# yellow-binary-tree/MMDuet

Measured on AMD Instinct MI355X. Metric: video frames/sec (stream decode, 1fps 336px), higher is better.
Workload: dtype bf16

## Files before the change

include/mmduet.h:

```cpp
#ifndef MMDUET_H
#define MMDUET_H
#include <stdint.h>
#ifdef __cplusplus
extern "C" {
#endif

#define MMD_OK 0
#define MMD_EINVAL (-22)
#define MMD_ENOMEM (-12)
#define MMD_ENOENT (-2)
#define MMD_ERANGE (-34)
#define MMD_EHIP (-5)

typedef enum { MMD_F32 = 0, MMD_BF16 = 1 } mmd_dtype;
typedef enum { MMD_W_DTYPE = 0, MMD_W_FP8_E4M3 = 1 } mmd_weight_dtype;
typedef enum { MMD_POOL_BILINEAR = 0, MMD_POOL_AVERAGE = 1, MMD_POOL_MAX = 2, MMD_POOL_ADAPTIVE_AVG = 3 } mmd_pool_mode;

typedef struct mmd_config {
    int32_t struct_size;
    int32_t dtype;
    int32_t vocab_size, hidden_size, intermediate_size, num_layers, num_heads, num_kv_heads, head_dim;
    float rope_theta, rms_norm_eps;
    int32_t vit_hidden, vit_intermediate, vit_layers, vit_heads, vit_image, vit_patch;
    float vit_ln_eps;
// ... 32 lines not shown
int mmd_vit_encode_frames(mmd_ctx* ctx, const uint8_t* frames, int B, int R, void* out);
int mmd_connector_pool(mmd_ctx* ctx, const void* tower_features, int B, void* out);
int mmd_normalize_frames(mmd_ctx* ctx, const void* frames, int src_kind, int B, int R, const float* mean3_host, const float* std3_host, float rescale, void* out);
int mmd_vision_tower(mmd_ctx* ctx, const void* pixel_values, int B, void* out);
int mmd_vision_pool_tokens(mmd_ctx* ctx, const void* feats, int B, int out_h, int out_w, void* out);
int mmd_vision_pool_head(mmd_ctx* ctx, const void* feats, int B, void* out);
int mmd_vit_set_full_tower(mmd_ctx* ctx, int on);
int mmd_vit_get_full_tower(const mmd_ctx* ctx);
int mmd_vit_debug_tap(mmd_ctx* ctx, int stage, void* out, int64_t out_elems);
int mmd_preprocess_frames(mmd_ctx* ctx, const uint8_t* frames, int T, int R, void* pixel_values);
int mmd_letterbox_geometry(int W, int H, int R, int* new_w, int* new_h, int* top, int* bottom, int* left, int* right);
int mmd_letterbox_frames(mmd_ctx* ctx, const uint8_t* frames, int T, int H, int W, int R, const uint8_t* pad_color,
                         int flip_channels, uint8_t* out);

int mmd_embed_tokens(mmd_ctx* ctx, const int64_t* ids, int k, void* out);

int mmd_stream_create(mmd_ctx* ctx, int64_t initial_tokens, mmd_stream** out);
void mmd_stream_destroy(mmd_stream* s);
int64_t mmd_kv_len(const mmd_stream* s);
int64_t mmd_kv_capacity(const mmd_stream* s);
int64_t mmd_kv_stride(const mmd_stream* s);
int mmd_kv_truncate(mmd_stream* s, int64_t new_len);
int mmd_kv_stash(mmd_stream* s, int64_t from, int64_t to);
int mmd_kv_unstash(mmd_stream* s);
int mmd_stream_reset(mmd_stream* s);
int mmd_kv_debug_set_len(mmd_stream* s, int64_t n);

int mmd_llm_step(mmd_ctx* ctx, mmd_stream* s, const void* embeds, int S, void* hidden_out);
int mmd_video_heads(mmd_ctx* ctx, const void* hidden, int M, float* out);
int mmd_lm_head(mmd_ctx* ctx, const void* hidden, int M, float* logits);
int mmd_frame_step(mmd_ctx* ctx, mmd_stream* s, const void* embeds, int S, const int32_t* head_rows_host, int n_rows,
                   float* head_logits_host);

int mmd_llm_step_multi(mmd_ctx* ctx, mmd_stream* const* streams, const int32_t* seg_rows, int n_segs, const void* embeds, void* hidden_out);
int mmd_frame_step_multi(mmd_ctx* ctx, mmd_stream* const* streams, const int32_t* seg_rows, int n_segs, const void* embeds,
                         const int32_t* head_rows, int n_head_rows, float* heads_out_host,
                         const int32_t* hidden_rows, int n_hidden_rows, void* hidden_rows_out, float* logits_out);

typedef struct mmd_sampler mmd_sampler;
#define MMD_SEG_FEED 1
#define MMD_SEG_SAMPLE 2
int mmd_sampler_create(mmd_ctx* ctx, mmd_sampler** out);
void mmd_sampler_destroy(mmd_sampler* sp);
int mmd_sampler_begin(mmd_sampler* sp, int64_t eos_id, float rep_penalty, const int64_t* prev_ids_host, int n_prev, int max_new);
int mmd_sampler_prev_len(const mmd_sampler* sp);
int mmd_round_multi(mmd_ctx* ctx, mmd_stream* const* streams, const int32_t* seg_rows, int n_segs, const void* const* seg_embeds, mmd_sampler* const* samplers,
                    const int32_t* seg_flags, const int32_t* head_rows, int n_head_rows, float* heads_out_host, int64_t* tokens_out_host);

int mmd_greedy_generate(mmd_ctx* ctx, mmd_stream* s, const void* prompt_embeds, int S, int64_t eos_id, float rep_penalty,
                        int64_t* prev_ids_host, int* n_prev, int prev_cap, int64_t* out_ids_host, int max_new, int* n_out);

#define MMD_COMM_ID_BYTES 128
typedef struct mmd_comm mmd_comm;
int mmd_comm_unique_id(uint8_t* id_out_host);
int mmd_comm_create(const uint8_t* id_host, int rank, int world, int device, void* hip_stream, mmd_comm** out);
void mmd_comm_destroy(mmd_comm* comm);
int mmd_comm_world(const mmd_comm* comm);
const char* mmd_comm_last_error(const mmd_comm* comm);
int mmd_gather_scores(mmd_comm* comm, const float* local, int T, int t_max, float* all);
int mmd_comm_probe(void);
int mmd_comm_set_stream(mmd_comm* comm, void* hip_stream);
int mmd_gather_block(mmd_comm* comm, const float* block, int64_t n_floats, float* all);

enum { MMD_K_GEMM_SKINNY = 0, MMD_K_GEMM_TILE = 1, MMD_K_ATTN_LLM = 2, MMD_K_ATTN_VIT = 3, MMD_K_NORM_ROPE = 4,
       MMD_K_OTHER = 5, MMD_K_COUNT = 6 };
int mmd_prof_enable(mmd_ctx* ctx, int class_mask);
int mmd_prof_set_stride(mmd_ctx* ctx, int stride);
int mmd_prof_read(mmd_ctx* ctx, double* ms_out , int64_t* launches_out ,
                  double* bytes_out , double* flops_out );
int mmd_prof_reset(mmd_ctx* ctx);

int mmd_op_gemm(mmd_ctx* ctx, const void* X, const void* W, const void* bias, const void* R, void* Y, int M, int N, int K,
                int epi, int out_f32, int variant);
int mmd_op_gemm_last_plan(mmd_ctx* ctx, int* out4);
int mmd_op_gemm_pair(mmd_ctx* ctx, const void* X, const void* W1, const void* b1, int epi1, const void* W2, const void* R, void* Y, int M, int N1, int K1, int N2,
                     int piece_major, int* used_pm_out);
int mmd_op_gemm_slabs(mmd_ctx* ctx, const void* X, const void* W, int M, int N, int K, int variant, float* slabs_out, int max_splits, int* splits_out);
int mmd_op_quantize_fp8(mmd_ctx* ctx, void* W, int N, int K, uint8_t* q8_out, float* scale_out);
int mmd_op_gemm_w8(mmd_ctx* ctx, const void* X, const void* Wq, const uint8_t* q8, const float* scale, const void* bias, const void* R, void* Y,
                   int M, int N, int K, int epi, int out_f32, int variant);
int mmd_op_gemm_bench(mmd_ctx* ctx, int M, int N, int K, int epi, int variant, int iters, float* avg_ms_out, const void* X, const void* W);
int mmd_op_rmsnorm(mmd_ctx* ctx, const void* x, const void* w, void* y, int M, int H, float eps);
int mmd_op_layernorm(mmd_ctx* ctx, const void* x, const void* w, const void* b, void* y, int M, int H, float eps);
int mmd_op_resid32_layernorm(mmd_ctx* ctx, const void* y16, float* h32, const void* pos16, int period, const void* w16, const void* b16, void* out16, void* outbf,
                             int M, int H, float eps);
int mmd_op_rope_append(mmd_ctx* ctx, void* qkv, int S, int nh, int nkv, int d, float theta, int64_t pos0, void* q_out,
                       void* Kc, void* Vc, int64_t cap);
int mmd_op_attention(mmd_ctx* ctx, const void* q, const void* Kc, const void* Vc, void* out, int S, int nh, int nkv, int d,
                     int64_t n_ctx, int64_t cap, int causal, int variant);
int mmd_op_attention_bench(mmd_ctx* ctx, int S, int nh, int nkv, int d, int64_t n_ctx, int variant, int iters, float* avg_ms_out);
int mmd_op_attention_last_form(mmd_ctx* ctx, int* out2);
int mmd_op_pool(mmd_ctx* ctx, const void* x, void* y, int B, int grid, int H, int mode, int stride);

#ifdef __cplusplus
}
#endif
#endif
```

mmduet_amd/_lib.py:

```python
import ctypes as C
import os

_HERE = os.path.dirname(os.path.abspath(__file__))
LIB_PATH = os.path.join(_HERE, 'csrc', 'libmmduet_hip.so')

MMD_F32, MMD_BF16 = 0, 1
POOL_MODES = {'bilinear': 0, 'average': 1, 'max': 2, 'adaptive_avg': 3}
K_NAMES = ('gemm_skinny', 'gemm_tile', 'attn_llm', 'attn_vit', 'norm_rope', 'other')
EPI = {'none': 0, 'gelu_tanh': 1, 'gelu_erf': 2, 'resid': 3, 'swiglu': 4}


class MmdConfig(C.Structure):
    _fields_ = [('struct_size', C.c_int32), ('dtype', C.c_int32),
                ('vocab_size', C.c_int32), ('hidden_size', C.c_int32), ('intermediate_size', C.c_int32),
                ('num_layers', C.c_int32), ('num_heads', C.c_int32), ('num_kv_heads', C.c_int32), ('head_dim', C.c_int32),
                ('rope_theta', C.c_float), ('rms_norm_eps', C.c_float),
                ('vit_hidden', C.c_int32), ('vit_intermediate', C.c_int32), ('vit_layers', C.c_int32), ('vit_heads', C.c_int32),
                ('vit_image', C.c_int32), ('vit_patch', C.c_int32), ('vit_ln_eps', C.c_float), ('vit_post_layernorm', C.c_int32),
                ('pool_mode', C.c_int32), ('pool_stride', C.c_int32), ('frame_num_tokens', C.c_int32),
                ('max_vit_batch', C.c_int32), ('max_step_tokens', C.c_int32), ('weight_dtype', C.c_int32),
                ('vision_only', C.c_int32), ('vit_class_token', C.c_int32), ('vit_pre_layernorm', C.c_int32), ('vit_act', C.c_int32), ('vit_pool_head', C.c_int32), ('tower_f16', C.c_int32)]


class MmduetError(RuntimeError):
    pass


_lib = None

_VP, _I, _I64, _F = C.c_void_p, C.c_int, C.c_int64, C.c_float
_SIGS = {
    'mmd_create': (_I, [C.POINTER(MmdConfig), _I, C.POINTER(_VP)]),
    'mmd_destroy': (None, [_VP]),
    'mmd_last_error': (C.c_char_p, [_VP]),
    'mmd_set_stream': (_I, [_VP, _VP]),
    'mmd_get_stream': (_VP, [_VP]),
    'mmd_synchronize': (_I, [_VP]),
    'mmd_load_tensor': (_I, [_VP, C.c_char_p, _VP, _I, C.POINTER(_I64), _I, _I]),
    'mmd_merge_lora': (_I, [_VP, C.c_char_p, _VP, _VP, _I, _F]),
    'mmd_set_rope_inv_freq': (_I, [_VP, _VP, _I]),
    'mmd_set_tower_share': (_I, [_VP, _I]),
    'mmd_finalize_weights': (_I, [_VP]),
    'mmd_weight_bytes': (_I64, [_VP]),
    'mmd_vit_encode': (_I, [_VP, _VP, _I, _VP]),
    'mmd_vit_set_full_tower': (_I, [_VP, _I]),
    'mmd_vit_get_full_tower': (_I, [_VP]),
    'mmd_vit_debug_tap': (_I, [_VP, _I, _VP, _I64]),
    'mmd_connector_pool': (_I, [_VP, _VP, _I, _VP]),
    'mmd_vit_encode_frames': (_I, [_VP, _VP, _I, _I, _VP]),
    'mmd_normalize_frames': (_I, [_VP, _VP, _I, _I, _I, C.POINTER(_F), C.POINTER(_F), _F, _VP]),
    'mmd_vision_tower': (_I, [_VP, _VP, _I, _VP]),
    'mmd_vision_pool_tokens': (_I, [_VP, _VP, _I, _I, _I, _VP]),
    'mmd_vision_pool_head': (_I, [_VP, _VP, _I, _VP]),
    'mmd_preprocess_frames': (_I, [_VP, _VP, _I, _I, _VP]),
    'mmd_letterbox_geometry': (_I, [_I, _I, _I] + [C.POINTER(_I)] * 6),
    'mmd_letterbox_frames': (_I, [_VP, _VP, _I, _I, _I, _I, _VP, _I, _VP]),
    'mmd_embed_tokens': (_I, [_VP, _VP, _I, _VP]),
    'mmd_stream_create': (_I, [_VP, _I64, C.POINTER(_VP)]),
    'mmd_stream_destroy': (None, [_VP]),
    'mmd_kv_len': (_I64, [_VP]),
    'mmd_kv_capacity': (_I64, [_VP]),
    'mmd_kv_stride': (_I64, [_VP]),
    'mmd_kv_truncate': (_I, [_VP, _I64]),
    'mmd_kv_debug_set_len': (_I, [_VP, _I64]),
    'mmd_stream_reset': (_I, [_VP]),
    'mmd_kv_stash': (_I, [_VP, _I64, _I64]),
    'mmd_kv_unstash': (_I, [_VP]),
    'mmd_comm_unique_id': (_I, [_VP]),
    'mmd_comm_create': (_I, [_VP, _I, _I, _I, _VP, C.POINTER(_VP)]),
    'mmd_comm_destroy': (None, [_VP]),
    'mmd_comm_world': (_I, [_VP]),
    'mmd_comm_last_error': (C.c_char_p, [_VP]),
    'mmd_gather_scores': (_I, [_VP, _VP, _I, _I, _VP]),
    'mmd_comm_probe': (_I, []),
    'mmd_comm_set_stream': (_I, [_VP, _VP]),
    'mmd_gather_block': (_I, [_VP, _VP, C.c_int64, _VP]),
    'mmd_llm_step': (_I, [_VP, _VP, _VP, _I, _VP]),
    'mmd_video_heads': (_I, [_VP, _VP, _I, _VP]),
    'mmd_lm_head': (_I, [_VP, _VP, _I, _VP]),
    'mmd_frame_step': (_I, [_VP, _VP, _VP, _I, _VP, _I, _VP]),
    'mmd_llm_step_multi': (_I, [_VP, C.POINTER(_VP), C.POINTER(C.c_int32), _I, _VP, _VP]),
    'mmd_frame_step_multi': (_I, [_VP, C.POINTER(_VP), C.POINTER(C.c_int32), _I, _VP, C.POINTER(C.c_int32), _I, C.POINTER(_F), C.POINTER(C.c_int32), _I, _VP, _VP]),
    'mmd_sampler_create': (_I, [_VP, C.POINTER(_VP)]),
    'mmd_sampler_destroy': (None, [_VP]),
    'mmd_sampler_begin': (_I, [_VP, _I64, _F, _VP, _I, _I]),
    'mmd_sampler_prev_len': (_I, [_VP]),
    'mmd_round_multi': (_I, [_VP, C.POINTER(_VP), C.POINTER(C.c_int32), _I, C.POINTER(_VP), C.POINTER(_VP), C.POINTER(C.c_int32), C.POINTER(C.c_int32), _I, C.POINTER(_F), C.POINTER(_I64)]),
    'mmd_greedy_generate': (_I, [_VP, _VP, _VP, _I, _I64, _F, _VP, C.POINTER(_I), _I, _VP, _I, C.POINTER(_I)]),
    'mmd_prof_enable': (_I, [_VP, _I]),
    'mmd_prof_set_stride': (_I, [_VP, _I]),
    'mmd_prof_read': (_I, [_VP, _VP, _VP, _VP, _VP]),
    'mmd_prof_reset': (_I, [_VP]),
    'mmd_op_gemm': (_I, [_VP, _VP, _VP, _VP, _VP, _VP, _I, _I, _I, _I, _I, _I]),
    'mmd_op_gemm_bench': (_I, [_VP, _I, _I, _I, _I, _I, _I, C.POINTER(_F), _VP, _VP]),
    'mmd_op_gemm_last_plan': (_I, [_VP, C.POINTER(_I)]),
    'mmd_op_gemm_pair': (_I, [_VP, _VP, _VP, _VP, _I, _VP, _VP, _VP, _I, _I, _I, _I, _I, C.POINTER(_I)]),
    'mmd_op_gemm_slabs': (_I, [_VP, _VP, _VP, _I, _I, _I, _I, _VP, _I, C.POINTER(_I)]),
    'mmd_op_quantize_fp8': (_I, [_VP, _VP, _I, _I, _VP, _VP]),
    'mmd_op_gemm_w8': (_I, [_VP, _VP, _VP, _VP, _VP, _VP, _VP, _VP, _I, _I, _I, _I, _I, _I]),
    'mmd_op_rmsnorm': (_I, [_VP, _VP, _VP, _VP, _I, _I, _F]),
    'mmd_op_layernorm': (_I, [_VP, _VP, _VP, _VP, _VP, _I, _I, _F]),
    'mmd_op_resid32_layernorm': (_I, [_VP, _VP, _VP, _VP, _I, _VP, _VP, _VP, _VP, _I, _I, _F]),
    'mmd_op_rope_append': (_I, [_VP, _VP, _I, _I, _I, _I, _F, _I64, _VP, _VP, _VP, _I64]),
    'mmd_op_attention': (_I, [_VP, _VP, _VP, _VP, _VP, _I, _I, _I, _I, _I64, _I64, _I, _I]),
    'mmd_op_attention_bench': (_I, [_VP, _I, _I, _I, _I, _I64, _I, _I, C.POINTER(_F)]),
    'mmd_op_attention_last_form': (_I, [_VP, C.POINTER(_I)]),
    'mmd_op_pool': (_I, [_VP, _VP, _VP, _I, _I, _I, _I, _I]),
}
EXPORTED_SYMBOLS = tuple(_SIGS)


def lib():
    global _lib
    if _lib is not None:
        return _lib
    if not os.path.exists(LIB_PATH):
        raise MmduetError(f'{LIB_PATH} not found: the MI355X HIP library is required (no CPU fallback). '
                          f'Build it with `make -C {os.path.dirname(LIB_PATH)}` or __graft_entry__.build().')
    try:
        L = C.CDLL(LIB_PATH, mode=C.RTLD_GLOBAL)
    except OSError as e:
        raise MmduetError(f'cannot load {LIB_PATH}: {e}') from e
    for name, (res, args) in _SIGS.items():
        try:
            fn = getattr(L, name)
        except AttributeError as e:
            raise MmduetError(f'{LIB_PATH} does not export {name}') from e
        fn.restype, fn.argtypes = res, args
    _lib = L
    return L


def check(rc, ctx=None, what=''):
    if rc == 0:
        return
    msg = lib().mmd_last_error(ctx)
    raise MmduetError(f'{what or "libmmduet_hip"} failed ({rc}): {msg.decode() if msg else "?"}')
```

mmduet_amd/csrc/gemm.hip:

```cpp
#include "common.h"
#include <type_traits>

#include "gemm_ring.h"

template <typename T> struct Frag;
template <> struct Frag<bf16_t> { using type = bf16x8_t; static constexpr int KSTEP = 32; };
template <> struct Frag<float> { using type = float; static constexpr int KSTEP = 4; };

template <typename T, int BM, int BN> struct TileCfg {
    static constexpr int BK = 32;
    static constexpr int PAD = sizeof(T) == 2 ? 8 : 1;
    static constexpr int LD = BK + PAD;
    static constexpr int WM = BM / 2, WN = BN / 2;
    static constexpr int TM = WM / 16, TN = WN / 16;
};

template <typename T, int ROWS, int LD>
__device__ __forceinline__ void stage_tile(T* __restrict__ lds, const T* __restrict__ g, long long ld, int r0, int nrows, int k0, int kend,
                                           int vec, int tid) {
    if constexpr (sizeof(T) == 2) {
        for (int i = tid; i < ROWS * 4; i += 256) {
            int r = i >> 2, c = (i & 3) * 8;
            s16x8_t v = {0, 0, 0, 0, 0, 0, 0, 0};
            int gr = r0 + r, gk = k0 + c;
// ... 841 lines not shown
        const int k0 = step * BK;
#pragma unroll
        for (int j = 0; j < BM / 32; ++j) {
            const int pi = wave + 4 * j;
            int row = m0 + pi * 8 + (lane >> 3);
            row = row < p.M ? row : p.M - 1;
            const int chunk = (lane & 7) ^ (lane >> 3);
            const bf16_t* src = X + (long long)row * p.ldx + k0 + chunk * 8;
            __builtin_amdgcn_global_load_lds((const __attribute__((address_space(1))) void*)src,
                                             (__attribute__((address_space(3))) void*)(xs + pi * 512), 16, 0, 0);
        }
#pragma unroll
        for (int j = 0; j < BN / 32; ++j) {
            const int wi = wave + 4 * j;
            const bf16_t* src = Wp + (((long long)(n0 / 16 + (wi >> 1)) * KT + (k0 >> 5) + (wi & 1)) * 64 + lane) * 8;
            __builtin_amdgcn_global_load_lds((const __attribute__((address_space(1))) void*)src,
                                             (__attribute__((address_space(3))) void*)(ws + wi * 512), 16, 0, 0);
        }
    };

    f32x4_t acc[TM][TN];
#pragma unroll
    for (int i = 0; i < TM; ++i)
#pragma unroll
        for (int j = 0; j < TN; ++j) acc[i][j] = f32x4_t{0, 0, 0, 0};

    const int zsteps = (nsteps + gridDim.z - 1) / gridDim.z;
    const int t0 = blockIdx.z * zsteps, t1 = min(nsteps, t0 + zsteps);
    if (t0 < t1) stage(0, t0);
    int cur = 0;
    for (int t = t0; t < t1; ++t) {
        __syncthreads();
        if (t + 1 < t1) stage(cur ^ 1, t + 1);
        const bf16_t* xs = lds + cur * (XE + WE);
        const bf16_t* ws = xs + XE;
#pragma unroll
        for (int kt = 0; kt < 2; ++kt) {
            bf16x8_t xf[TM], wf[TN];
#pragma unroll
            for (int i = 0; i < TM; ++i) {
                const int mt = (wm >> 4) + i;
                const int c = kt * 4 + lq;
                xf[i] = *reinterpret_cast<const bf16x8_t*>(xs + (mt * 2 + (lr >> 3)) * 512 + (lr & 7) * 64 + ((c ^ (lr & 7)) * 8));
            }
#pragma unroll
            for (int j = 0; j < TN; ++j) wf[j] = *reinterpret_cast<const bf16x8_t*>(ws + (((wn >> 4) + j) * 2 + kt) * 512 + lane * 8);
#pragma unroll
            for (int i = 0; i < TM; ++i)
#pragma unroll
                for (int j = 0; j < TN; ++j) acc[i][j] = mfma16<F16>(wf[j], xf[i], acc[i][j]);
        }
        cur ^= 1;
    }

    if (gridDim.z > 1) {
        float* ws = p.ws + (long long)blockIdx.z * p.M * p.N;
#pragma unroll
        for (int i = 0; i < TM; ++i) {
            const int m = m0 + wm + i * 16 + lr;
            if (m < p.M) {
#pragma unroll
                for (int j = 0; j < TN; ++j) *reinterpret_cast<f32x4_t*>(ws + (long long)m * p.N + n0 + wn + j * 16 + lq * 4) = acc[i][j];
            }
        }
        return;
    }
    [[maybe_unused]] f32x4_t scq[TN]; [[maybe_unused]] s16x4_t biq[TN]; [[maybe_unused]] s16x4_t rq[TM][TN];
    const bool has_sc = p.wscale != nullptr, has_bi = p.bias != nullptr;
    if constexpr (EPI != EPI_SWIGLU) {
#pragma unroll
        for (int j = 0; j < TN; ++j) {
            const int n = n0 + wn + j * 16 + lq * 4;
            scq[j] = has_sc ? *reinterpret_cast<const f32x4_t*>(p.wscale + n) : f32x4_t{1, 1, 1, 1};
            biq[j] = has_bi ? *reinterpret_cast<const s16x4_t*>((const bf16_t*)p.bias + n) : s16x4_t{0, 0, 0, 0};
        }
#pragma unroll
        for (int i = 0; i < TM; ++i)
#pragma unroll
            for (int j = 0; j < TN; ++j) {
                rq[i][j] = s16x4_t{0, 0, 0, 0};
                if constexpr (EPI == EPI_RESID) rq[i][j] = *reinterpret_cast<const s16x4_t*>((const bf16_t*)p.R + (long long)min(m0 + wm + i * 16 + lr, p.M - 1) * p.ldr + n0 + wn + j * 16 + lq * 4);
            }
    }
#pragma unroll
    for (int i = 0; i < TM; ++i) {
        const int m = m0 + wm + i * 16 + lr;
        [[maybe_unused]] const int mc = m < p.M ? m : p.M - 1;
        if constexpr (EPI == EPI_SWIGLU) {
            if constexpr (TN == 4) {
                const int nb = n0 + wn, ob = (nb >> 5) * 16;
                const s16x8_t v = pair_to_row8(big_value_swiglu(acc[i][0], acc[i][1], p.wscale, nb + lq * 4), big_value_swiglu(acc[i][2], acc[i][3], p.wscale, nb + 32 + lq * 4));
                if (m < p.M) *reinterpret_cast<s16x8_t*>((bf16_t*)p.Y + (long long)m * p.ldy + ob + (lq & 1) * 16 + (lq >> 1) * 8) = v;
            } else {
#pragma unroll
                for (int j = 0; j < TN; j += 2) big_store_swiglu(p, m, n0 + wn + j * 16 + lq * 4, acc[i][j], acc[i][j + 1]);
            }
        } else {
#pragma unroll
            for (int j = 0; j < TN; j += 2) {
                const int nb = n0 + wn + j * 16;
                const s16x8_t v = pair_to_row8(big_value_pre<EPI, F16>(acc[i][j], has_sc, scq[j], has_bi, biq[j], rq[i][j]), big_value_pre<EPI, F16>(acc[i][j + 1], has_sc, scq[j + 1], has_bi, biq[j + 1], rq[i][j + 1]));
                if (m < p.M) *reinterpret_cast<s16x8_t*>((bf16_t*)p.Y + (long long)m * p.ldy + nb + (lq & 1) * 16 + (lq >> 1) * 8) = v;
            }
        }
    }
}

template <int BN>
static void launch_big(const GemmP& p, const GemmPlan& pl, hipStream_t st) {
    const int KT = p.K >> 5;
    const dim3 grid(pl.gx, pl.gy, pl.splits);
    if (pl.bm == 160) {
        if constexpr (BN == 64) {
            if (p.epi == EPI_RESID) hipLaunchKernelGGL((gemm_big_kernel<64, EPI_RESID, false, 160>), grid, dim3(256), 0, st, p, KT);
            else hipLaunchKernelGGL((gemm_big_kernel<64, EPI_NONE, false, 160>), grid, dim3(256), 0, st, p, KT);
        }
        return;
    }
    if (pl.f16) {
        switch (p.epi) {
            case EPI_GELU_TANH: hipLaunchKernelGGL((gemm_big_kernel<BN, EPI_GELU_TANH, true>), grid, dim3(256), 0, st, p, KT); break;
            case EPI_RESID: hipLaunchKernelGGL((gemm_big_kernel<BN, EPI_RESID, true>), grid, dim3(256), 0, st, p, KT); break;
            default: hipLaunchKernelGGL((gemm_big_kernel<BN, EPI_NONE, true>), grid, dim3(256), 0, st, p, KT); break;
        }
        return;
    }
    switch (p.epi) {
        case EPI_GELU_TANH: hipLaunchKernelGGL((gemm_big_kernel<BN, EPI_GELU_TANH>), grid, dim3(256), 0, st, p, KT); break;
        case EPI_GELU_ERF: hipLaunchKernelGGL((gemm_big_kernel<BN, EPI_GELU_ERF>), grid, dim3(256), 0, st, p, KT); break;
        case EPI_RESID: hipLaunchKernelGGL((gemm_big_kernel<BN, EPI_RESID>), grid, dim3(256), 0, st, p, KT); break;
        case EPI_SWIGLU: hipLaunchKernelGGL((gemm_big_kernel<BN, EPI_SWIGLU>), grid, dim3(256), 0, st, p, KT); break;
        default: hipLaunchKernelGGL((gemm_big_kernel<BN, EPI_NONE>), grid, dim3(256), 0, st, p, KT); break;
    }
    if (pl.reduce) launch_reduce(splitk_reduce_kernel<bf16_t>, p, pl.splits, st);
}


static void* ring_dump_slot() {
    static void* dump_slot[64] = {};
    int dev = 0; hipGetDevice(&dev);
    if (dev < 0 || dev >= 64) return nullptr;
    if (!dump_slot[dev] && hipMalloc(&dump_slot[dev], 8192) != hipSuccess) return nullptr;
    return dump_slot[dev];
}

template <int WN, bool M32, int NS, bool EARLY, bool F16 = false>
static hipError_t launch_ringx_t(const GemmP& p, const GemmPlan& pl, hipStream_t st) {
    constexpr int BN = 64 * WN;
    const dim3 grid(pl.gx, 1, pl.splits);
    const int KT = p.K >> 5;
    const size_t smem = NS * (256 * 32 + BN * 32) * sizeof(bf16_t);
    static bool attr_set[64] = {};
    int adev = 0; hipGetDevice(&adev);
    if (adev >= 0 && adev < 64 && !attr_set[adev]) {
#define RX_ATTR(E) hipFuncSetAttribute((const void*)gemm_ringx_kernel<E, WN, M32, NS, EARLY, 0, F16>, hipFuncAttributeMaxDynamicSharedMemorySize, (int)smem);
        RX_ATTR(EPI_NONE) RX_ATTR(EPI_GELU_TANH) RX_ATTR(EPI_RESID)
        if constexpr (!F16) { RX_ATTR(EPI_GELU_ERF) RX_ATTR(EPI_SWIGLU) }
#undef RX_ATTR
        attr_set[adev] = true;
    }
    const dim3 block(WN * 128);
    GemmP q = p;
    q.dump = ring_dump_slot();
    if (!q.dump) return hipErrorOutOfMemory;
#define RX_GO(E) hipLaunchKernelGGL((gemm_ringx_kernel<E, WN, M32, NS, EARLY, 0, F16>), grid, block, smem, st, q, KT)
    switch (p.epi) {
        case EPI_GELU_TANH: RX_GO(EPI_GELU_TANH); break;
        case EPI_GELU_ERF: if constexpr (!F16) RX_GO(EPI_GELU_ERF); break;
        case EPI_RESID: RX_GO(EPI_RESID); break;
        case EPI_SWIGLU: if constexpr (!F16) RX_GO(EPI_SWIGLU); break;
        default: RX_GO(EPI_NONE); break;
    }
#undef RX_GO
    if (pl.reduce) launch_reduce(splitk_reduce_kernel<bf16_t>, p, pl.splits, st);
    return hipSuccess;
}
static hipError_t launch_ringx(const GemmP& p, const GemmPlan& pl, hipStream_t st) {
    if (pl.f16) return launch_ringx_t<4, false, 3, true, true>(p, pl, st);
    return pl.wn == 4 ? launch_ringx_t<4, false, 3, true>(p, pl, st) : launch_ringx_t<2, false, 3, true>(p, pl, st);
}

static inline void set_plan(const GemmArgs& a, const GemmPlan& pl) {
    if (a.plan_out) { a.plan_out[0] = pl.kernel; a.plan_out[1] = pl.tiles; a.plan_out[2] = pl.splits; a.plan_out[3] = pl.blocks; }
}

#ifdef MMDUET_DEBUG_VARIANTS
template <int DBG, int NS = 3>
static hipError_t launch_ringx_dbg(const GemmP& p, const GemmArgs& a, hipStream_t st) {
    GemmPlan pl;
    pl.kernel = GEMM_K_RING256; pl.tiles = cdiv(a.N, 256) * cdiv(a.M, 256); pl.blocks = pl.tiles <= 256 ? pl.tiles : 256;
    set_plan(a, pl);
    const size_t smem = NS * (256 * 32 + 256 * 32) * sizeof(bf16_t);
    hipFuncSetAttribute((const void*)gemm_ringx_kernel<EPI_NONE, 4, false, NS, true, DBG>, hipFuncAttributeMaxDynamicSharedMemorySize, (int)smem);
    hipLaunchKernelGGL((gemm_ringx_kernel<EPI_NONE, 4, false, NS, true, DBG>), dim3(pl.blocks), dim3(512), smem, st, p, a.K >> 5);
    return hipGetLastError();
}
static bool launch_debug_variant(GemmP p, const GemmArgs& a, hipStream_t st, hipError_t* err) {
    const int variant = a.variant;
    p.W = a.Wp;
    if (variant >= 92 && variant <= 99) {
        if (!big_packed_ok(MMD_BF16, a, 16) || (a.N % 32) != 0) { *err = hipErrorInvalidValue; return true; }
        switch (variant) {
            case 92: *err = launch_ringx_dbg<8, 4>(p, a, st); break;
            case 93: *err = launch_ringx_dbg<7>(p, a, st); break;
            case 94: *err = launch_ringx_dbg<6>(p, a, st); break;
            case 95: *err = launch_ringx_dbg<5>(p, a, st); break;
            case 99: *err = launch_ringx_dbg<4>(p, a, st); break;
            case 96: *err = launch_ringx_dbg<1>(p, a, st); break;
            case 97: *err = launch_ringx_dbg<2>(p, a, st); break;
            default: *err = launch_ringx_dbg<3>(p, a, st); break;
        }
        return true;
    }
    if (variant >= 300 && variant < 340 && a.M <= 64 && a.Wp) {
        p.slabs = a.epi == EPI_SWIGLU ? 0 : 1;
        GemmArgs b = a; int dummy = 0; if (a.epi != EPI_SWIGLU) { b.slabs_out = &dummy; b.epi = EPI_NONE; p.epi = EPI_NONE; }
        const bool two = a.epi == EPI_SWIGLU;
        GemmPlan pl;
#define SGO(NT_, WK_, KS_, NB_, DBG_, WN_, SPLIT_) (stream_geometry(pl, b, 4, NT_, WK_ * KS_, WN_, SPLIT_), set_plan(a, pl), launch_stream_t<4, NT_, WK_, KS_, NB_, DBG_, WN_>(p, pl, st))
#define SCFG(id, WK_, KS_, NB_, DBG_) case id: if (two) SGO(2, WK_, KS_, NB_, DBG_, 4, 0); else SGO(1, WK_, KS_, NB_, DBG_, 4, 0); break;
        switch (variant - 300) {
            SCFG(0, 2, 2, 4, 0) SCFG(1, 1, 4, 3, 0) SCFG(2, 4, 1, 4, 0) SCFG(3, 2, 4, 3, 0) SCFG(4, 1, 4, 4, 0) SCFG(5, 4, 2, 3, 0) SCFG(7, 2, 2, 6, 0)
            SCFG(10, 2, 2, 4, 1) SCFG(11, 1, 4, 3, 1) SCFG(12, 2, 2, 4, 2) SCFG(13, 1, 4, 3, 2)
            case 20: if (two) SGO(2, 2, 2, 4, 0, 5, 0); else SGO(1, 2, 2, 4, 0, 7, 8); break;
            case 21: if (two) SGO(2, 3, 2, 3, 0, 5, 0); else SGO(1, 2, 2, 4, 0, 7, 4); break;
            case 22: if (two) SGO(2, 2, 2, 4, 1, 5, 0); else SGO(1, 2, 2, 4, 1, 7, 8); break;
            case 23: if (two) SGO(2, 1, 4, 3, 0, 5, 0); else SGO(1, 1, 4, 3, 0, 7, 8); break;
            case 24: if (two) SGO(2, 2, 2, 4, 0, 8, 0); else SGO(1, 2, 2, 4, 0, 7, 16); break;
            default: *err = hipErrorInvalidValue; return true;
        }
#undef SCFG
#undef SGO
        *err = hipGetLastError();
        return true;
    }
    return false;
}
#endif

template <typename T>
static hipError_t launch_t(const GemmArgs& a, const GemmPlan& pl, hipStream_t st) {
    GemmP p;
    p.X = a.X; p.W = pl.w_from == GEMM_W_PACKED8 ? a.Wp8 : (pl.w_from == GEMM_W_PACKED ? a.Wp : a.W); p.bias = a.bias; p.R = a.R; p.Y = a.Y; p.ws = a.splitk_ws; p.wscale = a.wscale;
    p.ldx = a.ldx; p.ldw = a.ldw; p.ldr = a.ldr; p.ldy = a.ldy;
    p.M = a.M; p.N = a.N; p.K = a.K; p.epi = a.epi; p.out_f32 = a.out_f32; p.slabs = a.slabs_out ? 1 : 0; p.dump = nullptr; p.flags = 0; p.kper = pl.kper; p.x_pm = a.x_pm; p.y_pm = a.y_pm;
    p.vec = (sizeof(T) == 2 && (a.ldx % 8) == 0 && (a.ldw % 8) == 0 && ((uintptr_t)a.X % 16) == 0 && ((uintptr_t)a.W % 16) == 0) ? 1 : 0;
    if (a.ring_slabs_out) *a.ring_slabs_out = pl.ring_slabs;
    if (pl.kernel == GEMM_PLAN_EMPTY) return hipSuccess;
#ifdef MMDUET_DEBUG_VARIANTS
    if (hipError_t e = hipSuccess; sizeof(T) == 2 && launch_debug_variant(p, a, st, &e)) return e;
#endif
    if (!pl.valid()) return hipErrorInvalidValue;
    if (a.slabs_out && (pl.kernel == GEMM_K_GEMV16 || pl.kernel == GEMM_K_SKINNY || pl.kernel == GEMM_K_STREAM)) *a.slabs_out = pl.slabs;
    set_plan(a, pl);
    switch (pl.kernel) {
        case GEMM_K_GEMV16: launch_gemv16(p, pl, a.chain, st); break;
        case GEMM_K_STREAM: launch_stream(p, pl, st); break;
        case GEMM_K_RING256: case GEMM_K_RING128X2: if (hipError_t e = launch_ringx(p, pl, st); e != hipSuccess) return e; break;
        case GEMM_K_BIG128: launch_big<128>(p, pl, st); break;
        case GEMM_K_BIG64: launch_big<64>(p, pl, st); break;
        case GEMM_K_SKINNY: if (pl.mt == 1) launch_skinny_mt<1>(p, pl, st); else if (pl.mt == 2) launch_skinny_mt<2>(p, pl, st); else launch_skinny_mt<4>(p, pl, st); break;
        case GEMM_K_TILE128: hipLaunchKernelGGL((gemm_tile_kernel<T, 128, 128>), dim3(pl.gx, pl.gy, 1), dim3(256), 0, st, p); break;
        default:
            hipLaunchKernelGGL((gemm_tile_kernel<T, 64, 64>), dim3(pl.gx, pl.gy, pl.splits), dim3(256), 0, st, p);
            if (pl.reduce) launch_reduce(splitk_reduce_kernel<T>, p, pl.splits, st);
    }
    return hipGetLastError();
}

GemmPlan gemm_plan_for(int dtype, const GemmArgs& a) {
    static const GemmTuning tune = [] { GemmTuning t; if (const char* s = getenv("MMDUET_GEMV_KSPLIT_SHORT")) t.gemv_ksplit_short = atoi(s); return t; }();
    return gemm_plan(dtype, a, tune);
}
bool gemm_can_slab(int dtype, const GemmArgs& a) {
    int dummy = 0; GemmArgs b = a; b.slabs_out = &dummy; b.epi = EPI_NONE;
    const int k = gemm_plan_for(dtype, b).kernel;
    return k == GEMM_K_GEMV16 || k == GEMM_K_SKINNY || k == GEMM_K_STREAM;
}
bool gemm_ring_auto(int dtype, const GemmArgs& a, bool plain_only) {
    const int ring = gemm_plan_for(dtype, a).ring_auto;
    return !a.wscale && (plain_only ? ring == RING_AUTO_PLAIN : ring != RING_AUTO_NONE);
}
hipError_t launch_gemm(int dtype, const GemmArgs& a, hipStream_t st, const GemmPlan* planned) {
    const GemmPlan pl = planned ? *planned : gemm_plan_for(dtype, a);
    return dtype != MMD_F32 ? launch_t<bf16_t>(a, pl, st) : launch_t<float>(a, pl, st);
}
```

mmduet_amd/csrc/gemm_plan.h:

```cpp
#pragma once
#include <stddef.h>
#include <stdint.h>
#include "../../include/mmduet.h"

constexpr int MMD_F16 = 2;

static inline int cdiv(int64_t a, int64_t b) { return (int)((a + b - 1) / b); }
static inline int64_t round_up(int64_t a, int64_t b) { return (a + b - 1) / b * b; }

enum { EPI_NONE = 0, EPI_GELU_TANH = 1, EPI_GELU_ERF = 2, EPI_RESID = 3, EPI_SWIGLU = 4 };
enum { GEMM_AUTO = 0, GEMM_GENERIC = 1, GEMM_SKINNY = 2, GEMM_LARGE = 3, GEMM_BIG = 4, GEMM_SLAB = 5, GEMM_RING256 = 6, GEMM_RING256_SPLIT = 7,
       GEMM_RINGX = 16 ,
       GEMM_STREAM = 8  };

constexpr int GEMV_SSQ_STRIDE = 256;
constexpr int GEMV_CHAIN_ROWS = 4;
struct GemvChain {
    const void* xn_h = nullptr; const void* xn_gamma = nullptr; const float* xn_ssq = nullptr; float xn_eps = 0.f;
    void* fin_h = nullptr; float* fin_ssq = nullptr;
};
struct GemmArgs {
    const void* X; int64_t ldx;
    const void* W; int64_t ldw;
    const void* Wp = nullptr;
    const void* Wp8 = nullptr;
    const float* wscale = nullptr;
    const void* bias;
    const void* R; int64_t ldr;
    void* Y; int64_t ldy;
    int M, N, K;
    int epi; int out_f32;
    int variant;
    float* splitk_ws; size_t splitk_ws_bytes;
    int no_gemv = 0;
    int* ring_slabs_out = nullptr;
    int* slabs_out = nullptr;
    int ring_flags = 16;
    int ring_max_blocks = 0;
    const GemvChain* chain = nullptr;
    int* plan_out = nullptr;
    int x_pm = 0, y_pm = 0;
    int f16 = 0;
};
enum { GEMM_K_TILE64 = 0, GEMM_K_TILE128 = 1, GEMM_K_SKINNY = 2, GEMM_K_GEMV16 = 3, GEMM_K_BIG64 = 4, GEMM_K_BIG128 = 5, GEMM_K_RING256 = 6, GEMM_K_RING128X2 = 7, GEMM_K_STREAM = 8 };

struct GemmTuning {
    int gemv_ksplit_short = 2;
};

enum { GEMM_PLAN_INVALID = -1,
       GEMM_PLAN_EMPTY = -2 };
enum { GEMM_W_ROWMAJOR = 0, GEMM_W_PACKED = 1, GEMM_W_PACKED8 = 2 };
enum { GEMV_PLAIN = 0, GEMV_CONSUMER = 1, GEMV_PRODUCER = 2 };
enum { RING_AUTO_NONE = 0, RING_AUTO_PLAIN = 1, RING_AUTO_SPLIT = 2 };

struct GemmPlan {
    int kernel = GEMM_PLAN_INVALID;
    int tiles = 0, splits = 1, blocks = 0;
    int gx = 0, gy = 1;
    int prof_class = MMD_K_GEMM_TILE;
    int w_from = GEMM_W_ROWMAJOR;
    int mt = 0, nt = 0, wn = 0;
    int kt_per_block = 0;
    int kper = 0;
    int bn = 0, bm = 0;
    int chain = GEMV_PLAIN;
    int f16 = 0;
    int ring_auto = RING_AUTO_NONE;
    bool reduce = false;
    int slabs = 0;
    int ring_slabs = 0;
    bool valid() const { return kernel >= 0; }
};

static inline bool stream_ok(int dtype, const GemmArgs& a) {
    if (dtype != MMD_BF16 || a.f16 || !a.Wp || a.M <= 32 || a.M > 256 || (a.N % 16) != 0 || (a.ldx % 8) != 0 || ((uintptr_t)a.X % 16) != 0 || a.out_f32) return false;
    if (a.Wp8 && a.M <= 64) return false;
    if ((long long)a.M * a.ldx * 2 >= (1ll << 32)) return false;
    const int ksb = a.M <= 128 ? 4 : 2;
    if ((a.K % (ksb * 32)) != 0) return false;
    if (a.epi == EPI_SWIGLU) return (a.N % 32) == 0 && !a.slabs_out;
    if (a.slabs_out) return a.splitk_ws != nullptr && a.epi == EPI_NONE && (size_t)a.M * a.N * sizeof(float) <= a.splitk_ws_bytes;
    return a.splitk_ws != nullptr && (a.N % 4) == 0 && (a.ldy % 4) == 0 && (a.epi != EPI_RESID || (a.ldr % 4) == 0);
}
static inline void stream_geometry(GemmPlan& pl, const GemmArgs& a, int MT, int NT, int KSB, int WN, int want_split) {
    const int KT = a.K >> 5, ntiles = a.N >> 4;
    const int bx = cdiv(ntiles, WN * NT);
    int ksplit = 1;
    if (a.slabs_out || (a.epi != EPI_SWIGLU && a.splitk_ws)) {
        ksplit = want_split > 0 ? want_split : cdiv(288, bx);
        const int maxs = KT / (KSB * 6); if (ksplit > maxs) ksplit = maxs;
        if (ksplit > 16) ksplit = 16;
        if (ksplit < 1) ksplit = 1;
        while (ksplit > 1 && (size_t)ksplit * a.M * a.N * sizeof(float) > a.splitk_ws_bytes) --ksplit;
    }
    const int ktper = (int)round_up(cdiv(KT, ksplit), KSB);
    ksplit = cdiv(KT, ktper);
    pl.kernel = GEMM_K_STREAM; pl.tiles = ntiles; pl.splits = ksplit; pl.blocks = bx * ksplit; pl.gx = bx; pl.gy = 1;
    pl.w_from = GEMM_W_PACKED; pl.mt = MT; pl.nt = NT; pl.wn = WN; pl.kt_per_block = ktper;
    pl.slabs = ksplit;
    pl.reduce = !a.slabs_out && ksplit > 1;
}
struct StreamPlan { int wn, ksplit; };
static inline StreamPlan stream_plan(const GemmArgs& a, int NT, int MT, int KSB, bool can_split) {
    const int KT = a.K >> 5, ntiles = a.N >> 4;
    StreamPlan best{4, 1}; double best_cost = 1e30;
    for (int wn = 4; wn <= 8; ++wn) {
        const int bx = cdiv(ntiles, wn * NT);
        for (int ks = 1; ks <= (can_split ? 16 : 1); ++ks) {
            const int ktper = (int)round_up(cdiv(KT, ks), KSB);
            if (cdiv(KT, ktper) != ks) continue;
// ... 55 lines not shown
        if (splits > 8) splits = 8;
        while (splits > 1 && (size_t)splits * a.M * a.N * sizeof(float) > a.splitk_ws_bytes) --splits;
    }
    int ktper = (int)round_up(cdiv(KT, splits), 4);
    splits = cdiv(KT, ktper);
    GemmPlan pl;
    pl.kernel = GEMM_K_SKINNY; pl.tiles = ntiles; pl.splits = splits; pl.blocks = nblocks * splits; pl.gx = nblocks;
    pl.w_from = a.Wp8 ? GEMM_W_PACKED8 : GEMM_W_PACKED; pl.mt = MT; pl.nt = NT; pl.kt_per_block = ktper;
    pl.slabs = splits;
    pl.reduce = !a.slabs_out && splits > 1;
    return pl;
}

static inline bool big_bm160(const GemmArgs& a, int BN) {
    if (BN != 64 || a.f16 || (a.epi != EPI_NONE && a.epi != EPI_RESID) || a.M < 512) return false;
    const long long t128 = (long long)(a.N / 64) * cdiv(a.M, 128), t160 = (long long)(a.N / 64) * cdiv(a.M, 160);
    if (t160 > 512) return false;
    return (double)cdiv(t160, 256) * 160.0 < (double)cdiv(t128, 256) * 128.0 * 0.97;
}
static inline GemmPlan plan_big(const GemmArgs& a, int BN) {
    GemmPlan pl;
    pl.kernel = BN == 128 ? GEMM_K_BIG128 : GEMM_K_BIG64; pl.w_from = GEMM_W_PACKED; pl.bn = BN; pl.f16 = a.f16;
    if (big_bm160(a, BN)) {
        const int tiles = (a.N / 64) * cdiv(a.M, 160);
        pl.tiles = tiles; pl.splits = 1; pl.blocks = tiles; pl.gx = a.N / 64; pl.gy = cdiv(a.M, 160); pl.bm = 160;
        return pl;
    }
    const int tiles = (a.N / BN) * cdiv(a.M, 128);
    int splits = 1;
    if (tiles < 320 && a.K >= 8192 && a.epi != EPI_SWIGLU && a.splitk_ws && !a.f16) {
        splits = 3;
        if (tiles <= 64) splits = 4;
        while (splits > 1 && (size_t)splits * a.M * a.N * sizeof(float) > a.splitk_ws_bytes) --splits;
    } else if (tiles < 128 && a.K >= 2048 && a.epi != EPI_SWIGLU && a.splitk_ws && !a.f16) {
        splits = 256 / tiles; if (splits > 4) splits = 4; if (splits < 1) splits = 1;
        while (splits > 1 && (size_t)splits * a.M * a.N * sizeof(float) > a.splitk_ws_bytes) --splits;
    }
    pl.tiles = tiles; pl.splits = splits; pl.blocks = tiles * splits; pl.gx = a.N / BN; pl.gy = cdiv(a.M, 128); pl.bm = 128;
    if (splits > 1) {
        if (a.ring_slabs_out) pl.ring_slabs = splits;
        else pl.reduce = true;
    }
    return pl;
}

static inline bool ring_size_ok(const GemmArgs& a) { return (long long)a.M * a.ldx * 2 < (1ll << 32) && (long long)a.N * a.K * 2 < (1ll << 32); }
static inline bool ring_tiles_ok(long long t) { return t >= 400 || (t >= 192 && (double)t / (double)(cdiv((int)t, 256) * 256) >= 0.9); }
static inline bool big_packed_ok(int dtype, const GemmArgs& a, int BN) {
    return dtype == MMD_BF16 && a.Wp != nullptr && a.M > 64 && (a.N % BN) == 0 && (a.K % 64) == 0 && (a.ldx % 8) == 0 &&
           ((uintptr_t)a.X % 16) == 0 && !a.out_f32 && (a.ldy % 4) == 0 && ((uintptr_t)a.Y % 8) == 0 &&
           (a.epi != EPI_RESID || ((a.ldr % 4) == 0 && ((uintptr_t)a.R % 8) == 0)) && (a.bias == nullptr || ((uintptr_t)a.bias % 8) == 0);
}

static inline bool skinny_packed_ok(int dtype, const GemmArgs& a) {
    return dtype == MMD_BF16 && a.Wp != nullptr && a.M <= 64 && (a.N % 16) == 0 && (a.K % 32) == 0 && (a.ldx % 8) == 0 &&
           ((uintptr_t)a.X % 16) == 0 && (a.epi != EPI_SWIGLU || (a.N % 32) == 0);
}

static inline int ring_split_choice(const GemmArgs& a) {
    const int t256 = cdiv(a.M, 256) * cdiv(a.N, 256);
    int sp = 256 / t256; if (sp < 1) sp = 1;
    if (t256 > 128) {
        double best = 1e30; int bsp = 1;
        for (int s = 1; s <= 8; ++s) {
            if (s > 1 && (a.K / s < 1024 || (size_t)s * a.M * a.N * sizeof(float) > a.splitk_ws_bytes)) break;
            const double rounds = (double)cdiv(t256 * s, 256);
            const double cost = rounds * ((double)a.K / s) * 0.025 + (s > 1 ? (double)s * a.M * a.N * 8.0 / 5e6 : 0.0);
            if (cost < best * 0.97) { best = cost; bsp = s; }
        }
        return bsp;
    }
    while (sp > 1 && a.K / sp < 1024) --sp;
    while (sp > 1 && (size_t)sp * a.M * a.N * sizeof(float) > a.splitk_ws_bytes) --sp;
    return sp;
}
static inline GemmPlan plan_ring(const GemmArgs& a, int flags, int splits) {
    GemmPlan pl;
    int WN = 4;
    if (!a.f16) switch (flags & 27) {
        case 16: WN = 4; break;
        case 17: WN = 2; break;
        default: return pl;
    }
    if (a.f16 && a.epi != EPI_NONE && a.epi != EPI_GELU_TANH && a.epi != EPI_RESID) return pl;
    if (a.f16) splits = 1;
    while (splits > 1 && (a.epi == EPI_SWIGLU || !a.splitk_ws || (size_t)splits * a.M * a.N * sizeof(float) > a.splitk_ws_bytes)) --splits;
    const int BN = 64 * WN;
    const int tiles = cdiv(a.N, BN) * cdiv(a.M, 256);
    const int slots = WN == 2 ? 512 : 256;
    const int cap = a.ring_max_blocks < 0 ? tiles : (a.ring_max_blocks > 0 && a.ring_max_blocks < slots ? a.ring_max_blocks : slots);
    pl.kernel = WN == 2 ? GEMM_K_RING128X2 : GEMM_K_RING256; pl.w_from = GEMM_W_PACKED; pl.wn = WN; pl.f16 = a.f16;
    pl.gx = splits > 1 || tiles <= cap ? tiles : cap;
    pl.tiles = tiles; pl.splits = splits; pl.blocks = pl.gx * splits;
    pl.kper = splits > 1 ? 0 : ((a.K / 32) * 10) / 100 + 1;
    if (splits > 1) {
        if (a.ring_slabs_out) pl.ring_slabs = splits;
        else pl.reduce = true;
    }
    return pl;
}

static inline GemmPlan plan_tile(const GemmArgs& a, bool skinny, bool large) {
    int splits = 1;
    if (skinny) {
        int blocks = cdiv(a.N, 64) * cdiv(a.M, 64);
        int want = cdiv(512, blocks);
        int maxs = a.K / 256; if (maxs < 1) maxs = 1;
        splits = want < maxs ? want : maxs;
        if (splits > 16) splits = 16;
        if (a.splitk_ws == nullptr) splits = 1;
        while (splits > 1 && (size_t)splits * a.M * a.N * sizeof(float) > a.splitk_ws_bytes) --splits;
    }
    int kper = (int)round_up(cdiv(a.K, splits), 32);
    splits = cdiv(a.K, kper);
    GemmPlan pl;
    pl.kper = kper;
    const int B = large ? 128 : 64;
    pl.kernel = large ? GEMM_K_TILE128 : GEMM_K_TILE64; pl.gx = cdiv(a.N, B); pl.gy = cdiv(a.M, B);
    pl.tiles = pl.gx * pl.gy; pl.splits = large ? 1 : splits; pl.blocks = pl.tiles * pl.splits;
    pl.reduce = !large && splits > 1;
    return pl;
}

static inline GemmPlan plan_kernel(bool two_byte, const GemmArgs& a, const GemmTuning& tune) {
    const GemmPlan invalid;
    const int variant = a.variant;
    const bool skinny = (variant == GEMM_SKINNY) || (variant == GEMM_AUTO && a.M <= 64);
    const bool large = (variant == GEMM_LARGE) || (variant == GEMM_AUTO && a.M >= 256 && a.N >= 128);
    if (two_byte) {
        if ((variant == GEMM_AUTO || variant == GEMM_SKINNY || variant == GEMM_STREAM) && stream_ok(MMD_BF16, a)) return plan_stream(a);
        if (variant == GEMM_STREAM) return invalid;
        const bool ring_ok = big_packed_ok(MMD_BF16, a, 16) && (a.N % 32) == 0 && ring_size_ok(a);
        if (variant == GEMM_RING256 || (variant == GEMM_AUTO && a.M >= 512 && ring_ok && ring_tiles_ok((long long)cdiv(a.M, 256) * cdiv(a.N, 256)))) {
            if (!ring_ok) return invalid;
            GemmPlan pl = plan_ring(a, a.ring_flags, 1);
            if (variant == GEMM_AUTO) pl.ring_auto = RING_AUTO_PLAIN;
            return pl;
        }
        const bool ring_split_ok = ring_ok && a.epi != EPI_SWIGLU && a.splitk_ws != nullptr;
        if (!a.f16 && (variant == GEMM_RING256_SPLIT || (variant == GEMM_AUTO && a.M >= 512 && a.K >= 8192 && ring_split_ok))) {
            if (variant == GEMM_RING256_SPLIT && !ring_ok) return invalid;
            const int sp = ring_split_choice(a);
            if (variant == GEMM_RING256_SPLIT || sp >= 2) {
                GemmPlan pl = plan_ring(a, 16, sp);
                if (variant == GEMM_AUTO) pl.ring_auto = RING_AUTO_SPLIT;
                return pl;
            }
        }
        if (variant >= GEMM_RINGX && variant < GEMM_RINGX + 128) {
            if (!ring_ok) return invalid;
            const int flags = variant - GEMM_RINGX;
            int sp = 1;
            if (flags & 4) {
                const int slots = (flags & 1) ? 512 : 256, tl = cdiv(a.M, 256) * cdiv(a.N, (flags & 1) ? 128 : 256);
                sp = slots / tl; if (sp < 1) sp = 1;
                while (sp > 1 && a.K / sp < 1024) --sp;
                if (sp < 2) sp = 2;
            }
            return plan_ring(a, flags, sp);
        }
        const bool want_big = variant == GEMM_BIG || (variant == GEMM_AUTO && a.M > 64);
        if (want_big) {
            int bn = 0;
            const long long t128 = (long long)cdiv(a.M, 128) * (a.N / 128);
            if (big_packed_ok(MMD_BF16, a, 128) && (t128 >= 400 || (a.K >= 8192 && t128 >= 224))) bn = 128;
            else if (big_packed_ok(MMD_BF16, a, 64)) bn = 64;
            if (bn && variant == GEMM_AUTO && !a.f16 && a.M >= 512 && a.K >= 1024 && (a.N % 128) == 0 && big_packed_ok(MMD_BF16, a, 16) && ring_size_ok(a)) {
                const long long mt128 = cdiv(a.M, 128);
                const double nb = bn == 64 ? (double)cdiv(mt128 * (a.N / 64), 256) : (double)cdiv(t128, 256);
                const double cbig = bn == 64 ? (nb > 1.83 ? nb : 1.83) : (1.77 * nb > 2.29 ? 1.77 * nb : 2.29);
                const double cr4 = 2.95 * (double)cdiv((long long)cdiv(a.M, 256) * (a.N / 128), 256);
                if (cr4 < 0.8 * cbig)
                    return plan_ring(a, 17, 1);
            }
            if (bn) return plan_big(a, bn);
            if (variant == GEMM_BIG) return invalid;
        }
        if (a.f16) return invalid;
        if (skinny && skinny_packed_ok(MMD_BF16, a)) {
            if (a.slabs_out && !a.splitk_ws) return invalid;
            if (a.M <= 16 && !a.no_gemv) return plan_gemv16(a, tune);
            if (a.chain) return invalid;
            return plan_skinny(a, a.M <= 16 ? 1 : (a.M <= 32 ? 2 : 4));
        }
    }
    if (a.slabs_out) return invalid;
    if (a.chain) return invalid;
    if (a.W == nullptr) return invalid;
    return plan_tile(a, skinny, large);
}

static inline GemmPlan gemm_plan(int dtype, const GemmArgs& a, const GemmTuning& tune) {
    if (dtype == MMD_F16 && !a.f16) { GemmArgs h = a; h.f16 = 1; return gemm_plan(dtype, h, tune); }
    GemmPlan pl;
    if (a.M <= 0 || a.N <= 0) { pl.kernel = GEMM_PLAN_EMPTY; return pl; }
    pl = plan_kernel(dtype != MMD_F32, a, tune);
    if (!pl.valid()) return pl;
    if ((a.x_pm || a.y_pm) && (pl.ring_auto == RING_AUTO_NONE || a.wscale || (a.x_pm && (a.K % 32)) || (a.y_pm && ((a.epi == EPI_SWIGLU ? a.N / 2 : a.N) % 32)))) return GemmPlan();
    if (a.y_pm && pl.ring_auto != RING_AUTO_PLAIN) return GemmPlan();
    const bool streaming = pl.kernel == GEMM_K_GEMV16 || pl.kernel == GEMM_K_SKINNY || pl.kernel == GEMM_K_STREAM;
    pl.prof_class = streaming || (pl.kernel == GEMM_K_TILE64 && a.M <= 64) ? MMD_K_GEMM_SKINNY : MMD_K_GEMM_TILE;
    return pl;
}
```

mmduet_amd/csrc/gemm_ring.h:

```cpp
#pragma once
#include "common.h"
#include <type_traits>

#define MMD_BAR() do { asm volatile("" ::: "memory"); __builtin_amdgcn_s_barrier(); asm volatile("" ::: "memory"); } while (0)

struct GemmP {
    const void* X; const void* W; const void* bias; const void* R; void* Y; float* ws;
    const float* wscale;
    long long ldx, ldw, ldr, ldy;
    int M, N, K, epi, out_f32, kper, vec;
    int slabs;
    void* dump;
    int flags;
    int x_pm, y_pm;
};

template <int EPI>
__device__ __forceinline__ s16x4_t big_value(const GemmP& p, int m, int n, const f32x4_t& a) {
    float v[4] = {a[0], a[1], a[2], a[3]};
    if (p.wscale) {
        const f32x4_t sc = *reinterpret_cast<const f32x4_t*>(p.wscale + n);
#pragma unroll
        for (int r = 0; r < 4; ++r) v[r] *= sc[r];
    }
    if (p.bias) {
        s16x4_t b = *reinterpret_cast<const s16x4_t*>((const bf16_t*)p.bias + n);
#pragma unroll
        for (int r = 0; r < 4; ++r) v[r] += bf2f((bf16_t)b[r]);
    }
    if constexpr (EPI == EPI_GELU_TANH) {
#pragma unroll
        for (int r = 0; r < 4; ++r) v[r] = gelu_tanh_fast(bf2f(f2bf(v[r])));
    } else if constexpr (EPI == EPI_GELU_ERF) {
#pragma unroll
        for (int r = 0; r < 4; ++r) v[r] = gelu_erf_fast(bf2f(f2bf(v[r])));
    } else if constexpr (EPI == EPI_RESID) {
        s16x4_t rr = *reinterpret_cast<const s16x4_t*>((const bf16_t*)p.R + (long long)m * p.ldr + n);
#pragma unroll
        for (int r = 0; r < 4; ++r) v[r] = bf2f(f2bf(v[r])) + bf2f((bf16_t)rr[r]);
    }
    return s16x4_t{(short)f2bf(v[0]), (short)f2bf(v[1]), (short)f2bf(v[2]), (short)f2bf(v[3])};
}
template <int EPI, bool F16 = false>
__device__ __forceinline__ s16x4_t big_value_pre(const f32x4_t& a, bool has_scale, const f32x4_t& sc, bool has_bias, const s16x4_t& b, const s16x4_t& rr) {
    float v[4] = {a[0], a[1], a[2], a[3]};
    if (has_scale) {
#pragma unroll
        for (int r = 0; r < 4; ++r) v[r] *= sc[r];
    }
    if (has_bias) {
#pragma unroll
        for (int r = 0; r < 4; ++r) v[r] += raw2f<F16>((uint16_t)b[r]);
    }
    if constexpr (EPI == EPI_GELU_TANH) {
#pragma unroll
        for (int r = 0; r < 4; ++r) v[r] = gelu_tanh_fast(raw2f<F16>(f2raw<F16>(v[r])));
    } else if constexpr (EPI == EPI_GELU_ERF) {
#pragma unroll
        for (int r = 0; r < 4; ++r) v[r] = gelu_erf_fast(raw2f<F16>(f2raw<F16>(v[r])));
    } else if constexpr (EPI == EPI_RESID) {
#pragma unroll
        for (int r = 0; r < 4; ++r) v[r] = raw2f<F16>(f2raw<F16>(v[r])) + raw2f<F16>((uint16_t)rr[r]);
    }
    return s16x4_t{(short)f2raw<F16>(v[0]), (short)f2raw<F16>(v[1]), (short)f2raw<F16>(v[2]), (short)f2raw<F16>(v[3])};
}
template <int EPI>
__device__ __forceinline__ void big_store(const GemmP& p, int m, int n, const f32x4_t& a) {
    if (m >= p.M) return;
    *reinterpret_cast<s16x4_t*>((bf16_t*)p.Y + (long long)m * p.ldy + n) = big_value<EPI>(p, m, n, a);
}
__device__ __forceinline__ s16x4_t big_value_swiglu(const f32x4_t& g_in, const f32x4_t& u_in, const float* ws = nullptr, int n_gate = 0) {
    f32x4_t g = g_in, u = u_in;
    if (ws) { g *= *reinterpret_cast<const f32x4_t*>(ws + n_gate); u *= *reinterpret_cast<const f32x4_t*>(ws + n_gate + 16); }
    s16x4_t o;
#pragma unroll
    for (int r = 0; r < 4; ++r) {
        float gg = bf2f(f2bf(g[r])), uu = bf2f(f2bf(u[r]));
        float sl = bf2f(f2bf(gg * __builtin_amdgcn_rcpf(1.0f + __builtin_amdgcn_exp2f(-gg * 1.4426950408889634f))));
        o[r] = (short)f2bf(sl * uu);
    }
    return o;
}
__device__ __forceinline__ s16x8_t pair_to_row8(const s16x4_t& ta, const s16x4_t& tb) {
    const uint2 a = __builtin_bit_cast(uint2, ta), b = __builtin_bit_cast(uint2, tb);
    const auto x = __builtin_amdgcn_permlane16_swap(a.x, b.x, false, false);
    const auto y = __builtin_amdgcn_permlane16_swap(a.y, b.y, false, false);
    const uint4 o = {x[0], y[0], x[1], y[1]};
    return __builtin_bit_cast(s16x8_t, o);
}
__device__ __forceinline__ void big_store_swiglu(const GemmP& p, int m, int n_gate, const f32x4_t& g, const f32x4_t& u) {
    if (m >= p.M) return;
    const int oc = (n_gate >> 5) * 16 + (n_gate & 15);
    *reinterpret_cast<s16x4_t*>((bf16_t*)p.Y + (long long)m * p.ldy + oc) = big_value_swiglu(g, u, p.wscale, n_gate);
}


__device__ __forceinline__ f32x4_t quad_of(const f32x16_t& v, int q) { return f32x4_t{v[4 * q], v[4 * q + 1], v[4 * q + 2], v[4 * q + 3]}; }
__device__ __forceinline__ s16x8_t halves_to_row8(const s16x4_t& q0, const s16x4_t& q1) {
    const uint2 a = __builtin_bit_cast(uint2, q0), b = __builtin_bit_cast(uint2, q1);
    const auto x = __builtin_amdgcn_permlane32_swap(a.x, b.x, false, false);
    const auto y = __builtin_amdgcn_permlane32_swap(a.y, b.y, false, false);
    const uint4 o = {x[0], y[0], x[1], y[1]};
    return __builtin_bit_cast(s16x8_t, o);
}

template <int EPI, int WN, bool M32, int NS, bool EARLY, int DBG = 0, bool F16 = false>
__global__ __launch_bounds__(WN * 128, 2) void gemm_ringx_kernel(GemmP p, int KT) {
    static_assert(!F16 || (!M32 && EPI != EPI_SWIGLU), "the fp16 form exists for the 16x16x32 schedule and the tower's epilogues");
    constexpr int BM = 256, BN = 64 * WN, BK = 32, NW = 2 * WN;
    constexpr int XE = BM * BK, WE = BN * BK, SE = XE + WE;
    constexpr int XP = (BM / 16) / NW, WP = (BN / 16) / NW;
    constexpr int NDMA = DBG == 3 ? 0 : (DBG == 2 ? WP : XP + WP);
    extern __shared__ __attribute__((aligned(16))) bf16_t lds[];
    const int tid = threadIdx.x, lane = tid & 63, wave = __builtin_amdgcn_readfirstlane(tid >> 6);
    const int lr = lane & 15, lq = lane >> 4, lh = lane >> 5;
    const int wr = wave / WN, wc = wave % WN;
    const int nbx = (p.N + BN - 1) / BN, nby = (p.M + BM - 1) / BM;
    const int nblk = nbx * nby;
    int m0 = 0, n0 = 0;
    auto tile_origin = [&](int bid) {
        const int xcd = bid & 7, q = nblk >> 3, r = nblk & 7;
        bid = (xcd < r ? xcd * (q + 1) : r * (q + 1) + (xcd - r) * q) + (bid >> 3);
        const int TB = nby < 8 ? nby : 8;
        const int band = bid / (TB * nbx), rem = bid - band * (TB * nbx);
        const int tb = min(TB, nby - band * TB);
        const int nt = rem / tb, mt = band * TB + rem - nt * tb;
        m0 = mt * BM; n0 = nt * BN;
    };
    const int ntiles = p.N >> 4;
    const bf16_t* X = (const bf16_t*)p.X;
    const bf16_t* Wp = (const bf16_t*)p.W;
    const int nsteps_all = p.K / BK;
    const int zsteps = (nsteps_all + gridDim.z - 1) / gridDim.z;
    const int t0 = blockIdx.z * zsteps;
    const int nsteps = min(nsteps_all, t0 + zsteps) - t0;

    const int srow = lane >> 2, spos = lane & 3;
    const int sswz = (0x1230 >> (((srow >> 2) & 3) * 4)) & 3;
    unsigned xo[XP]; long long wo[WP];
    const unsigned wlane = lane * 16;
    const int xstep = p.x_pm ? 1024 : BK * 2;
    auto tile_sources = [&]() {
#pragma unroll
        for (int j = 0; j < XP; ++j) {
            const int pi = wave + NW * j;
            if (p.x_pm) {
                int grp = (m0 >> 4) + pi; const int gmax = (p.M - 1) >> 4; grp = grp < gmax ? grp : gmax;
                xo[j] = (unsigned)(grp * (p.K >> 5)) * 1024u + (unsigned)(srow * 64 + ((spos ^ sswz) * 16));
                continue;
            }
            int row = m0 + pi * 16 + srow; row = row < p.M ? row : p.M - 1;
            xo[j] = (unsigned)(row * (int)p.ldx + ((spos ^ sswz) * 8)) * 2u;
        }
#pragma unroll
        for (int j = 0; j < WP; ++j) {
            const int pi = wave + NW * j;
            int ntile = n0 / 16 + pi; ntile = ntile < ntiles ? ntile : ntiles - 1;
            wo[j] = ((long long)ntile * KT * 512 + (long long)t0 * 512) * 2;
        }
    };
    auto dma_x = [&](int slot, int step, int j) {
        if constexpr (DBG == 2 || DBG == 3) return;
        if constexpr (DBG == 1) {
            __builtin_amdgcn_global_load_lds((const __attribute__((address_space(1))) void*)(X + (long long)min(m0 + (wave + NW * j) * 16, p.M - 16) * p.ldx + (long long)step * 512 + lane * 8),
                                             (__attribute__((address_space(3))) void*)(lds + slot * SE + (wave + NW * j) * 512), 16, 0, 0);
            return;
        }
        const char* ub = (const char*)X + (long long)(t0 + step) * xstep;
        asm volatile("" : "+s"(ub));
        __builtin_amdgcn_global_load_lds((const __attribute__((address_space(1))) void*)(ub + xo[j]),
                                         (__attribute__((address_space(3))) void*)(lds + slot * SE + (wave + NW * j) * 512), 16, 0, 0);
    };
    auto dma_w = [&](int slot, int step, int j) {
        if constexpr (DBG == 3) return;
        const char* ub = (const char*)Wp + wo[j] + (long long)step * 1024;
        asm volatile("" : "+s"(ub));
        __builtin_amdgcn_global_load_lds((const __attribute__((address_space(1))) void*)(ub + wlane),
                                         (__attribute__((address_space(3))) void*)(lds + slot * SE + XE + (wave + NW * j) * 512), 16, 0, 0);
    };
    auto stage = [&](int slot, int step) {
#pragma unroll
        for (int j = 0; j < XP; ++j) dma_x(slot, step, j);
#pragma unroll
        for (int j = 0; j < WP; ++j) dma_w(slot, step, j);
    };
    auto dma_k = [&](int slot, int step, int k) { if (k < XP) dma_x(slot, step, k); else if (k < XP + WP) dma_w(slot, step, k - XP); };

    constexpr int VM_ONE = NDMA, VM_TWO = 2 * NDMA;
    constexpr int NST = EPI == EPI_SWIGLU ? 8 : 16;
#ifdef MMDUET_NO_PST
    constexpr bool PST = false;
#else
    constexpr bool PST = !M32 && NS == 3 && DBG == 0;
#endif
#define RINGX_WAIT(n) asm volatile("s_waitcnt vmcnt(%0) lgkmcnt(0)" :: "i"(n) : "memory")
    const int G = gridDim.x;
    const int rswz = (0x1230 >> (((lr >> 2) & 3) * 4)) & 3;
    if constexpr (WN == 2 && NS == 3) {
        if (G > 256 && (int)blockIdx.x >= 256 && p.kper > 0) {
            for (int i = 0; i < p.kper; ++i) __builtin_amdgcn_s_sleep(127);
        }
    }

    if constexpr (!M32) {
        f32x4_t acc[8][4];
#pragma unroll
        for (int i = 0; i < 8; ++i)
#pragma unroll
            for (int j = 0; j < 4; ++j) acc[i][j] = f32x4_t{0, 0, 0, 0};
        const int aoff = (wr * 8) * 512 + lr * 32 + ((lq ^ rswz) * 8);
        const int boff = XE + (wc * 4) * 512 + lane * 8;
        bf16x8_t a[8], b0[4], b1[4];
        auto step = [&](auto steady, int s, int slot, const bf16x8_t (&b)[4], bf16x8_t (&bn)[4], auto pending) {
            constexpr bool STEADY = decltype(steady)::value;
            constexpr bool PEND = decltype(pending)::value;
            if (DBG == 5 && s < 2) RINGX_WAIT((NS - 2) * NDMA + 16);
            else if (PEND) RINGX_WAIT((NS - 2) * NDMA + NST);
            else if (STEADY || s + NS - 1 < nsteps) RINGX_WAIT((NS - 2) * NDMA);
            else if (NS == 4 && s + 2 < nsteps) RINGX_WAIT(NDMA);
            else RINGX_WAIT(0);
            if (!(DBG == 8 && (s & 1))) MMD_BAR();
            const bool refill = STEADY || s + NS < nsteps;
            const bool more = STEADY || s + 1 < nsteps;
            const bf16_t* nbase = lds + (slot == NS - 1 ? 0 : slot + 1) * SE;
            bf16x8_t a6n, a7n;
            __builtin_amdgcn_s_setprio(1);
            if constexpr (DBG == 7) {
#pragma unroll
                for (int i = 0; i < 8; ++i) {
                    acc[i][0] = mfma16<F16>(b[0], a[i], acc[i][0]);
                    __builtin_amdgcn_sched_barrier(0);
                    if (more) { if (i == 0) a7n = *reinterpret_cast<const bf16x8_t*>(nbase + aoff + 7 * 512); else a[i - 1] = *reinterpret_cast<const bf16x8_t*>(nbase + aoff + (i - 1) * 512); }
                    __builtin_amdgcn_sched_barrier(0);
                    acc[i][1] = mfma16<F16>(b[1], a[i], acc[i][1]);
                    __builtin_amdgcn_sched_barrier(0);
                    if (more && i < 4) bn[i] = *reinterpret_cast<const bf16x8_t*>(nbase + boff + i * 512);
                    __builtin_amdgcn_sched_barrier(0);
                    acc[i][2] = mfma16<F16>(b[2], a[i], acc[i][2]);
                    __builtin_amdgcn_sched_barrier(0);
                    if (refill && i < XP + WP) dma_k(slot, s + NS, i);
                    __builtin_amdgcn_sched_barrier(0);
                    acc[i][3] = mfma16<F16>(b[3], a[i], acc[i][3]);
                    __builtin_amdgcn_sched_barrier(0);
                }
                if (more) a[7] = a7n;
                __builtin_amdgcn_s_setprio(0);
                return;
            }
#pragma unroll
            for (int i = 0; i < 8; ++i) {
#pragma unroll
                for (int j = 0; j < 4; ++j) acc[i][j] = mfma16<F16>(b[j], a[i], acc[i][j]);
                __builtin_amdgcn_sched_barrier(0);
                if (more) {
                    if (i < 6) a[i] = *reinterpret_cast<const bf16x8_t*>(nbase + aoff + i * 512);
                    if (i < 4) bn[i] = *reinterpret_cast<const bf16x8_t*>(nbase + boff + i * 512);
                    if (i == 0) a6n = *reinterpret_cast<const bf16x8_t*>(nbase + aoff + 6 * 512);
                    if (i == 1) a7n = *reinterpret_cast<const bf16x8_t*>(nbase + aoff + 7 * 512);
                }
                if (refill) {
                    if (EARLY ? i < XP + WP : i >= 8 - (XP + WP)) dma_k(slot, s + NS, i - (EARLY ? 0 : 8 - (XP + WP)));
                }
                __builtin_amdgcn_sched_barrier(0);
            }
            if (more) { a[6] = a6n; a[7] = a7n; }
            __builtin_amdgcn_s_setprio(0);
        };
        auto prologue = [&]() { stage(0, 0); if (nsteps > 1) stage(1, 1); if (nsteps > 2) stage(2, 2); if (NS > 3 && nsteps > 3) stage(3, 3); };
        int tile = blockIdx.x;
        tile_origin(tile); tile_sources(); prologue();
        for (; tile < nblk; tile += G) {
            const bool pend = PST && tile != (int)blockIdx.x && nsteps >= NS + 3 && gridDim.z == 1;
            if (DBG == 5) asm volatile("s_waitcnt vmcnt(%0)" :: "i"(VM_TWO + 16) : "memory");
            else if (pend) asm volatile("s_waitcnt vmcnt(%0)" :: "i"(VM_TWO + NST) : "memory");
            else if (NS > 3 && nsteps > 3) asm volatile("s_waitcnt vmcnt(%0)" :: "i"(3 * NDMA) : "memory");
            else if (nsteps > 2) asm volatile("s_waitcnt vmcnt(%0)" :: "i"(VM_TWO) : "memory");
            else if (nsteps > 1) asm volatile("s_waitcnt vmcnt(%0)" :: "i"(VM_ONE) : "memory");
            else asm volatile("s_waitcnt vmcnt(0)" ::: "memory");
            MMD_BAR();
#pragma unroll
            for (int i = 0; i < 8; ++i) a[i] = *reinterpret_cast<const bf16x8_t*>(lds + aoff + i * 512);
#pragma unroll
            for (int j = 0; j < 4; ++j) b0[j] = *reinterpret_cast<const bf16x8_t*>(lds + boff + j * 512);
            int slot = 0, s = 0;
            if (pend) {
                step(std::true_type{}, 0, 0, b0, b1, std::true_type{});
                step(std::true_type{}, 1, 1, b1, b0, std::true_type{});
                slot = 2 % NS; s = 2;
            }
            for (; s + NS + 1 < nsteps; s += 2) {
                step(std::true_type{}, s, slot, b0, b1, std::false_type{});
                slot = slot == NS - 1 ? 0 : slot + 1;
                step(std::true_type{}, s + 1, slot, b1, b0, std::false_type{});
                slot = slot == NS - 1 ? 0 : slot + 1;
            }
            for (; s < nsteps; s += 2) {
                step(std::false_type{}, s, slot, b0, b1, std::false_type{});
                slot = slot == NS - 1 ? 0 : slot + 1;
                if (s + 1 < nsteps) {
                    step(std::false_type{}, s + 1, slot, b1, b0, std::false_type{});
                    slot = slot == NS - 1 ? 0 : slot + 1;
                }
            }
            const int em0 = m0, en0 = n0;
            bf16_t* const dump = (bf16_t*)p.dump + tid * 8;
            if (tile + G < nblk) { tile_origin(tile + G); tile_sources(); prologue(); }
            __builtin_amdgcn_sched_barrier(0);
            if (gridDim.z > 1) {
                float* wsl = p.ws + (long long)blockIdx.z * p.M * p.N;
#pragma unroll
                for (int i = 0; i < 8; ++i) {
                    const int m = em0 + wr * 128 + i * 16 + lr;
                    if (m < p.M) {
#pragma unroll
                        for (int j = 0; j < 4; ++j) { const int nb = en0 + wc * 64 + j * 16; if (nb + 16 <= p.N) *reinterpret_cast<f32x4_t*>(wsl + (long long)m * p.N + nb + lq * 4) = acc[i][j]; }
                    }
                }
                return;
            }
            f32x4_t scq[4]; s16x4_t biq[4], rq[4], rnext[4];
            int ncol[4];
            const bool has_sc = p.wscale != nullptr, has_bi = p.bias != nullptr;
            if constexpr (EPI != EPI_SWIGLU) {
#pragma unroll
                for (int j = 0; j < 4; ++j) {
                    const int nb = en0 + wc * 64 + (j & ~1) * 16;
                    ncol[j] = ((j & 1) ? (nb + 32 <= p.N ? nb + 16 : p.N - 16) : (nb + 16 <= p.N ? nb : p.N - 16)) + lq * 4;
                    scq[j] = has_sc ? *reinterpret_cast<const f32x4_t*>(p.wscale + ncol[j]) : f32x4_t{1, 1, 1, 1};
                    biq[j] = has_bi ? *reinterpret_cast<const s16x4_t*>((const bf16_t*)p.bias + ncol[j]) : s16x4_t{0, 0, 0, 0};
                    rq[j] = rnext[j] = s16x4_t{0, 0, 0, 0};
                }
                if constexpr (EPI == EPI_RESID) {
                    const int m = min(em0 + wr * 128 + lr, p.M - 1);
#pragma unroll
                    for (int j = 0; j < 4; ++j) rnext[j] = *reinterpret_cast<const s16x4_t*>((const bf16_t*)p.R + (long long)m * p.ldr + ncol[j]);
                }
            }
            if constexpr (DBG == 4) {
#pragma unroll
                for (int i = 0; i < 8; ++i)
#pragma unroll
                    for (int j = 0; j < 4; ++j) asm volatile("" :: "v"(acc[i][j][0]), "v"(acc[i][j][1]), "v"(acc[i][j][2]), "v"(acc[i][j][3]));
            } else
#pragma unroll
            for (int i = 0; i < 8; ++i) {
                const int m = em0 + wr * 128 + i * 16 + lr;
                const int mc = m < p.M ? m : p.M - 1;
                if constexpr (EPI == EPI_RESID) {
#pragma unroll
                    for (int j = 0; j < 4; ++j) rq[j] = rnext[j];
                    if (i < 7) {
                        const int mn = min(m + 16, p.M - 1);
#pragma unroll
                        for (int j = 0; j < 4; ++j) rnext[j] = *reinterpret_cast<const s16x4_t*>((const bf16_t*)p.R + (long long)mn * p.ldr + ncol[j]);
                    }
                    __builtin_amdgcn_sched_barrier(0);
                }
                if constexpr (EPI == EPI_SWIGLU) {
                    const int nb = en0 + wc * 64;
                    const int ob = (nb >> 5) * 16;
                    const int ns0 = min(nb, p.N - 32) + lq * 4, ns1 = min(nb + 32, p.N - 32) + lq * 4;
                    const s16x8_t v = pair_to_row8(big_value_swiglu(acc[i][0], acc[i][1], p.wscale, ns0), big_value_swiglu(acc[i][2], acc[i][3], p.wscale, ns1));
                    const bool ok = m < p.M && nb + 32 * (lq & 1) + 32 <= p.N;
                    bf16_t* const yd = p.y_pm ? (bf16_t*)p.Y + ((long long)(m >> 4) * (p.N >> 6) + (ob >> 5)) * 512 + lr * 32 + (lq & 1) * 16 + (lq >> 1) * 8
                                              : (bf16_t*)p.Y + (long long)m * p.ldy + ob + (lq & 1) * 16 + (lq >> 1) * 8;
                    if constexpr (PST) *reinterpret_cast<s16x8_t*>(ok ? yd : dump) = v;
                    else if (ok) *reinterpret_cast<s16x8_t*>(yd) = v;
                } else {
#pragma unroll
                    for (int j = 0; j < 4; j += 2) {
                        const int nb = en0 + wc * 64 + j * 16;
                        const s16x8_t v = pair_to_row8(big_value_pre<EPI, F16>(acc[i][j], has_sc, scq[j], has_bi, biq[j], rq[j]), big_value_pre<EPI, F16>(acc[i][j + 1], has_sc, scq[j + 1], has_bi, biq[j + 1], rq[j + 1]));
                        if constexpr (DBG == 6) { const u32x4_t w = __builtin_bit_cast(u32x4_t, v); asm volatile("" :: "v"(w[0]), "v"(w[1]), "v"(w[2]), "v"(w[3])); }
                        else {
                            const bool ok = m < p.M && nb + 16 * (lq & 1) + 16 <= p.N;
                            bf16_t* const yd = p.y_pm ? (bf16_t*)p.Y + ((long long)(m >> 4) * (p.N >> 5) + (nb >> 5)) * 512 + lr * 32 + (lq & 1) * 16 + (lq >> 1) * 8
                                                      : (bf16_t*)p.Y + (long long)m * p.ldy + nb + (lq & 1) * 16 + (lq >> 1) * 8;
                            if constexpr (PST) *reinterpret_cast<s16x8_t*>(ok ? yd : dump) = v;
                            else if (ok) *reinterpret_cast<s16x8_t*>(yd) = v;
                        }
                    }
                }
            }
#pragma unroll
            for (int i = 0; i < 8; ++i)
#pragma unroll
                for (int j = 0; j < 4; ++j) acc[i][j] = f32x4_t{0, 0, 0, 0};
        }
    } else {
        f32x16_t acc[4][2];
#pragma unroll
        for (int i = 0; i < 4; ++i)
#pragma unroll
            for (int j = 0; j < 2; ++j)
#pragma unroll
                for (int r = 0; r < 16; ++r) acc[i][j][r] = 0.f;
        const int lt = (lane >> 4) & 1;
        const int xoff0 = (wr * 8 + lt) * 512 + lr * 32 + (((0 + lh) ^ rswz) * 8);
        const int xoff1 = (wr * 8 + lt) * 512 + lr * 32 + (((2 + lh) ^ rswz) * 8);
        const int woff0 = XE + (wc * 4 + lt) * 512 + ((0 + lh) * 16 + lr) * 8;
        const int woff1 = XE + (wc * 4 + lt) * 512 + ((2 + lh) * 16 + lr) * 8;
        bf16x8_t xf[4][2], w0[2][2], w1[2][2];
        auto ldx = [&](const bf16_t* base, int i, int kk) { return *reinterpret_cast<const bf16x8_t*>(base + (kk ? xoff1 : xoff0) + i * 1024); };
        auto ldw = [&](const bf16_t* base, int j, int kk) { return *reinterpret_cast<const bf16x8_t*>(base + (kk ? woff1 : woff0) + j * 1024); };
        auto step = [&](auto steady, int s, int slot, const bf16x8_t (&w)[2][2], bf16x8_t (&wn)[2][2]) {
            constexpr bool STEADY = decltype(steady)::value;
            if (STEADY || s + NS - 1 < nsteps) RINGX_WAIT((NS - 2) * NDMA);
            else if (NS == 4 && s + 2 < nsteps) RINGX_WAIT(NDMA);
            else RINGX_WAIT(0);
            MMD_BAR();
            const bool refill = STEADY || s + NS < nsteps;
            const bool more = STEADY || s + 1 < nsteps;
            const bf16_t* nbase = lds + (slot == NS - 1 ? 0 : slot + 1) * SE;
            bf16x8_t x3n0, x3n1;
            __builtin_amdgcn_s_setprio(1);
#pragma unroll
            for (int i = 0; i < 4; ++i) {
#pragma unroll
                for (int kk = 0; kk < 2; ++kk)
#pragma unroll
                    for (int j = 0; j < 2; ++j) acc[i][j] = __builtin_amdgcn_mfma_f32_32x32x16_bf16(w[j][kk], xf[i][kk], acc[i][j], 0, 0, 0);
                __builtin_amdgcn_sched_barrier(0);
                if (more) {
                    if (i < 3) { xf[i][0] = ldx(nbase, i, 0); xf[i][1] = ldx(nbase, i, 1); }
                    if (i == 0) { x3n0 = ldx(nbase, 3, 0); wn[0][0] = ldw(nbase, 0, 0); }
                    if (i == 1) { x3n1 = ldx(nbase, 3, 1); wn[0][1] = ldw(nbase, 0, 1); }
                    if (i == 2) { wn[1][0] = ldw(nbase, 1, 0); wn[1][1] = ldw(nbase, 1, 1); }
                }
                if (refill) {
                    constexpr int first = EARLY ? 0 : 4 - (XP + WP) / 2;
                    if (i >= first && i < first + (XP + WP) / 2) { dma_k(slot, s + NS, 2 * (i - first)); dma_k(slot, s + NS, 2 * (i - first) + 1); }
                }
                __builtin_amdgcn_sched_barrier(0);
            }
            if (more) { xf[3][0] = x3n0; xf[3][1] = x3n1; }
            __builtin_amdgcn_s_setprio(0);
        };
        auto prologue = [&]() { stage(0, 0); if (nsteps > 1) stage(1, 1); if (nsteps > 2) stage(2, 2); if (NS > 3 && nsteps > 3) stage(3, 3); };
        int tile = blockIdx.x;
        tile_origin(tile); tile_sources(); prologue();
        for (; tile < nblk; tile += G) {
// ... 77 lines not shown
```

mmduet_amd/csrc/model.hip:

```cpp
#include "common.h"
#include <algorithm>
#include <cfloat>
#include <cmath>
#include <cstdio>
#include <cstring>
#include <cstdlib>
#include <map>
#include <string>
#include <unordered_map>
#include <vector>

static thread_local std::string g_create_error;

struct RawTensor { void* p = nullptr; std::vector<int64_t> shape; int64_t numel = 0; };

struct Prof {
    unsigned on = 0;
    int stride = 1;
    int64_t seen[MMD_K_COUNT] = {0};
    std::vector<hipEvent_t> pool;
    struct Pending { hipEvent_t a, b; int kind; };
    std::vector<Pending> pending;
    double ms[MMD_K_COUNT] = {0}; int64_t n[MMD_K_COUNT] = {0}; double bytes[MMD_K_COUNT] = {0}; double flops[MMD_K_COUNT] = {0};
};

struct LlmLayer { void *ln1 = 0, *ln2 = 0, *wqkv = 0, *bqkv = 0, *wo = 0, *wgu = 0, *wdown = 0;
                  void *wqkv_p = 0, *wo_p = 0, *wgu_p = 0, *wdown_p = 0;
                  void *wqkv_8 = 0, *wo_8 = 0, *wgu_8 = 0, *wdown_8 = 0;
                  float *sqkv = 0, *so = 0, *sgu = 0, *sdown = 0; };
struct VitLayer { void *ln1w = 0, *ln1b = 0, *wqkv = 0, *bqkv = 0, *wo = 0, *bo = 0, *ln2w = 0, *ln2b = 0, *w1 = 0, *b1 = 0, *w2 = 0, *b2 = 0;
                  void *wqkv_p = 0, *wo_p = 0, *w1_p = 0, *w2_p = 0; };

struct mmd_ctx {
    mmd_config cfg;
    int device = 0;
    hipStream_t own_stream = nullptr, stream = nullptr;
    std::string err;
    std::unordered_map<std::string, RawTensor> raw;
    std::vector<void*> allocs;
    int64_t weight_bytes = 0;
    bool finalized = false;
    std::vector<LlmLayer> L;
    std::vector<VitLayer> VL;
    void *embed = 0, *fnorm = 0, *lm_head = 0, *heads4 = 0, *lm_head_p = 0;
    void *patch_w = 0, *patch_b = 0, *pos_emb = 0, *post_w = 0, *post_b = 0, *p0w = 0, *p0b = 0, *p2w = 0, *p2b = 0;
    void *patch_w_p = 0, *p0w_p = 0, *p2w_p = 0;
    int vit_kpad = 0, vit_ipad = 0, vit_tokens = 0, vit_grid = 0, qkv_w = 0;
    int vit_seq = 0;
    void *cls_emb = 0, *pre_w = 0, *pre_b = 0, *v_patch = 0;
    void *hd_probe = 0, *hd_wq = 0, *hd_bq = 0, *hd_wkv = 0, *hd_bkv = 0, *hd_wo = 0, *hd_bo = 0, *hd_lnw = 0, *hd_lnb = 0, *hd_w1 = 0, *hd_b1 = 0, *hd_w2 = 0, *hd_b2 = 0;
    void *hd_q = 0, *hd_kv = 0, *hd_a = 0, *hd_h = 0, *hd_n = 0, *hd_m = 0;
    float* inv_freq = nullptr; bool inv_freq_user = false;
    void *v_col = 0, *v_h = 0, *v_xn = 0, *v_qkv = 0, *v_attn = 0, *v_mlp = 0, *v_p1 = 0, *v_p2 = 0;
    float* v_h32 = 0; int64_t v_h32_rows = 0;
    void *l_h = 0, *l_xn = 0, *l_qkv = 0, *l_q = 0, *l_attn = 0, *l_act = 0, *l_hid = 0;
    float* splitk_ws = 0; size_t splitk_bytes = 0;
    float* attn_ws = 0; size_t attn_bytes = 0;
    float* v_splitk_ws = 0; size_t v_splitk_bytes = 0;
    float* v_attn_ws = 0; size_t v_attn_bytes = 0;
    float* logits_ws = 0;
    float* heads_dev = 0;
    int32_t* rows_dev = 0;
    int64_t* tok_dev = 0;
    void* argmax_scratch = 0;
    int64_t* prev_dev = 0; int prev_cap = 0;
    void* gen_embed = 0;
    float* heads_host = 0; int32_t* rows_host = 0; int64_t* tok_host = 0;
    int lb_W = 0, lb_H = 0, lb_R = 0; int32_t* lb_xtab = 0; int32_t* lb_ytab = 0;
    int pp_R = 0; int32_t* pp_coef = 0; int32_t* pp_bounds = 0; int pp_ksize = 0; uint8_t* pp_tmp = 0; size_t pp_tmp_bytes = 0;
    int last_vit_B = 0;
    StepState* step_dev = nullptr; StepState* step_host = nullptr;
    hipGraphExec_t dec_graph = nullptr; hipGraph_t dec_graph_src = nullptr;
    float dec_pen = 0.f; int64_t dec_eos = 0; bool no_graph = false;
    int last_form[2] = {0, 0};
    int last_plan[4] = {-1, 0, 0, 0};
    bool no_fuse = false;
    bool no_pm = false;
    bool gemm_half = false;
    int tower_ring_flags = -1, tower_ring_blocks = 0;
    int hid_compact = 0;
    bool full_tower = false;
    bool last_sparse = false;
    bool tower_compact = false;
    bool full_projector = false;
    bool no_slab_norm = false;
    bool full_last_layer = false;
    bool no_chain = false;
    void* rope_tab = 0;
    bool no_rope_fuse = false;
    float* chain_ssq = 0;
    StepState* seg_dev = nullptr; StepState* seg_host = nullptr; int seg_slot = 0;
    hipEvent_t seg_event[8] = {};
    float* round_logits = 0; void* round_hidden = 0; void* round_scratch = 0; int64_t* round_toks_dev = 0; int64_t* round_toks_host = 0;
    Prof prof;
};

struct mmd_stream {
    mmd_ctx* ctx;
    void* K = nullptr; void* V = nullptr;
    int64_t cap = 0, len = 0;
    bool vmm = false;
    int64_t mapped = 0, chunk_tokens = 0;
    size_t va_bytes = 0;
    std::vector<hipMemGenericAllocationHandle_t> handles;
    std::vector<std::pair<void*, size_t>> maps;
    void* stash_k = nullptr; void* stash_v = nullptr; size_t stash_bytes = 0; int64_t stash_from = -1, stash_to = -1;
};

#define FAIL(ctx, code, ...) do { char _b[512]; snprintf(_b, sizeof(_b), __VA_ARGS__); (ctx)->err = _b; return (code); } while (0)
#define HIPCHK(ctx, expr) do { hipError_t _e = (expr); if (_e != hipSuccess) { FAIL(ctx, MMD_EHIP, "%s failed: %s (%s:%d)", #expr, hipGetErrorString(_e), __FILE__, __LINE__); } } while (0)

static size_t es(const mmd_ctx* c) { return dtype_size(c->cfg.dtype); }

static int dev_alloc(mmd_ctx* c, void** out, size_t bytes, bool zero = true) {
    if (bytes == 0) bytes = 16;
    void* p = nullptr;
    hipError_t e = hipMalloc(&p, bytes);
    if (e != hipSuccess) FAIL(c, MMD_ENOMEM, "hipMalloc(%zu) failed: %s", bytes, hipGetErrorString(e));
    if (zero) { e = hipMemsetAsync(p, 0, bytes, c->stream); if (e != hipSuccess) FAIL(c, MMD_EHIP, "memset failed"); }
    c->allocs.push_back(p);
    *out = p;
    return MMD_OK;
}
static void dev_free(mmd_ctx* c, void* p) {
    if (!p) return;
    for (size_t i = 0; i < c->allocs.size(); ++i) if (c->allocs[i] == p) { c->allocs[i] = c->allocs.back(); c->allocs.pop_back(); break; }
    hipFree(p);
}

struct ProfScope {
    mmd_ctx* c; int kind; hipEvent_t a = nullptr, b = nullptr;
    ProfScope(mmd_ctx* c_, int kind_, double bytes, double flops) : c(c_), kind(kind_) {
        if (!((c->prof.on >> kind_) & 1u)) return;
        if ((c->prof.seen[kind_]++ % c->prof.stride) != 0) return;
        auto get = [&]() { hipEvent_t e; if (!c->prof.pool.empty()) { e = c->prof.pool.back(); c->prof.pool.pop_back(); } else hipEventCreate(&e); return e; };
        a = get(); b = get();
        c->prof.bytes[kind] += bytes; c->prof.flops[kind] += flops; c->prof.n[kind] += 1;
        hipEventRecord(a, c->stream);
    }
    ~ProfScope() {
        if (!a) return;
        hipEventRecord(b, c->stream);
        c->prof.pending.push_back({a, b, kind});
        if (c->prof.pending.size() >= 32) {
            size_t done = 0;
            while (done + 8 < c->prof.pending.size() && hipEventQuery(c->prof.pending[done].b) == hipSuccess) {
                Prof::Pending& p = c->prof.pending[done];
                float ms = 0; hipEventElapsedTime(&ms, p.a, p.b);
                c->prof.ms[p.kind] += ms;
                c->prof.pool.push_back(p.a); c->prof.pool.push_back(p.b);
                ++done;
            }
            if (done) c->prof.pending.erase(c->prof.pending.begin(), c->prof.pending.begin() + done);
        }
    }
};
static void prof_drain(mmd_ctx* c) {
    if (c->prof.pending.empty()) return;
    hipStreamSynchronize(c->stream);
    for (auto& p : c->prof.pending) {
        float ms = 0; hipEventElapsedTime(&ms, p.a, p.b);
        c->prof.ms[p.kind] += ms;
        c->prof.pool.push_back(p.a); c->prof.pool.push_back(p.b);
    }
    c->prof.pending.clear();
}

static GemmArgs gemm_args(mmd_ctx* c, const void* X, int64_t ldx, const void* W, int64_t ldw, const void* bias, const void* R, int64_t ldr, void* Y, int64_t ldy, int M, int N, int K,
                          int epi, int out_f32, int variant, const void* Wp, bool tower, const void* Wp8 = nullptr, const float* wscale = nullptr) {
    GemmArgs a;
    a.X = X; a.ldx = ldx; a.W = W; a.ldw = ldw; a.Wp = Wp; a.bias = bias; a.R = R; a.ldr = ldr; a.Y = Y; a.ldy = ldy;
    a.M = M; a.N = N; a.K = K; a.epi = epi; a.out_f32 = out_f32; a.variant = variant; a.Wp8 = Wp8; a.wscale = wscale;
    a.splitk_ws = tower ? c->v_splitk_ws : c->splitk_ws; a.splitk_ws_bytes = tower ? c->v_splitk_bytes : c->splitk_bytes;
    a.plan_out = c->last_plan;
    if (tower && c->tower_ring_flags >= 0) { a.ring_flags = c->tower_ring_flags; a.ring_max_blocks = c->tower_ring_blocks; }
    return a;
}
static int gemm(mmd_ctx* c, const void* X, int64_t ldx, const void* W, int64_t ldw, const void* bias, const void* R, int64_t ldr, void* Y,
                int64_t ldy, int M, int N, int K, int epi, int out_f32 = 0, int variant = GEMM_AUTO, const void* Wp = nullptr, bool tower = false,
                const void* Wp8 = nullptr, const float* wscale = nullptr, const GemvChain* chain = nullptr, int* ring_slabs_out = nullptr, int pm = 0) {
    GemmArgs a = gemm_args(c, X, ldx, W, ldw, bias, R, ldr, Y, ldy, M, N, K, epi, out_f32, variant, Wp, tower, Wp8, wscale);
    a.chain = chain; a.ring_slabs_out = ring_slabs_out; a.x_pm = pm & 1; a.y_pm = (pm >> 1) & 1;
    const int dt = c->gemm_half ? MMD_F16 : c->cfg.dtype;
    const GemmPlan pl = gemm_plan_for(dt, a);
    double e = (double)es(c);
    double bytes = (double)M * K * e + (double)N * K * ((Wp8 && M <= 64) ? 1.0 : e) + (double)M * (epi == EPI_SWIGLU ? N / 2 : N) * (out_f32 ? 4.0 : e);
    ProfScope ps(c, pl.prof_class, bytes, 2.0 * M * N * K);
    HIPCHK(c, launch_gemm(dt, a, c->stream, &pl));
    return MMD_OK;
}

static bool gemm_pair_pm(mmd_ctx* c, bool tower, const void* X1, int64_t ldx1, const void* W1p, const void* b1, int N1w, int K1, int epi1, void* T, int64_t ldt,
                         const void* W2p, int N2, const void* R2, int64_t ldr2, void* Y2, int64_t ldy2, int epi2, int M) {
    if (c->no_pm) return false;
    const int dt = c->gemm_half ? MMD_F16 : c->cfg.dtype;
    const GemmArgs a = gemm_args(c, X1, ldx1, nullptr, 0, b1, nullptr, 0, T, ldt, M, N1w, K1, epi1, 0, GEMM_AUTO, W1p, tower);
    const GemmArgs b = gemm_args(c, T, ldt, nullptr, 0, nullptr, R2, ldr2, Y2, ldy2, M, N2, (int)ldt, epi2, 0, GEMM_AUTO, W2p, tower);
    return gemm_ring_auto(dt, a, true) && gemm_ring_auto(dt, b);
}

extern "C" int mmd_create(const mmd_config* cfg, int device, mmd_ctx** out) {
    if (!cfg || !out) { g_create_error = "null argument"; return MMD_EINVAL; }
    if (cfg->struct_size != (int32_t)sizeof(mmd_config)) { g_create_error = "mmd_config size mismatch (ABI)"; return MMD_EINVAL; }
    if (cfg->dtype != MMD_F32 && cfg->dtype != MMD_BF16) { g_create_error = "unsupported dtype"; return MMD_EINVAL; }
    if (cfg->weight_dtype != MMD_W_DTYPE && (cfg->weight_dtype != MMD_W_FP8_E4M3 || cfg->dtype != MMD_BF16)) { g_create_error = "weight_dtype fp8_e4m3 needs a bf16 context"; return MMD_EINVAL; }
    if (!cfg->vision_only && (cfg->num_heads % cfg->num_kv_heads != 0 || cfg->head_dim % 2 != 0 || cfg->head_dim > 128)) { g_create_error = "unsupported head configuration"; return MMD_EINVAL; }
    if (cfg->vit_hidden % cfg->vit_heads != 0 || cfg->vit_hidden / cfg->vit_heads > 128) { g_create_error = "unsupported ViT head configuration"; return MMD_EINVAL; }
    if (cfg->tower_f16 && (cfg->dtype != MMD_BF16 || cfg->vision_only || cfg->vit_class_token || cfg->vit_pre_layernorm || cfg->vit_act != 0 || cfg->vit_pool_head ||
                           (cfg->vit_hidden % 64) != 0 || ((cfg->vit_hidden / cfg->vit_heads) % 8) != 0)) {
        g_create_error = "tower_f16 needs a bf16 context and the LLaVA SigLIP tower form (no class token / pre-LN / pooling head, hidden % 64 == 0, head_dim % 8 == 0)"; return MMD_EINVAL; }
    if (cfg->tower_f16 < 0 || cfg->tower_f16 > 2 || (cfg->tower_f16 == 1 && (cfg->vit_post_layernorm || cfg->vit_hidden > 2048))) {
        g_create_error = "tower_f16: 0 | 1 (autocast: fp32 residual stream; no post_layernorm, hidden <= 2048) | 2 (fp16 residual stream)"; return MMD_EINVAL; }
    hipError_t e = hipSetDevice(device);
    if (e != hipSuccess) { g_create_error = std::string("hipSetDevice: ") + hipGetErrorString(e); return MMD_EHIP; }
    mmd_ctx* c = new mmd_ctx();
    c->cfg = *cfg; c->device = device;
    e = hipStreamCreateWithFlags(&c->own_stream, hipStreamNonBlocking);
    if (e != hipSuccess) { g_create_error = std::string("hipStreamCreate: ") + hipGetErrorString(e); delete c; return MMD_EHIP; }
    c->stream = c->own_stream;
    c->vit_grid = cfg->vit_image / cfg->vit_patch;
    c->vit_tokens = c->vit_grid * c->vit_grid;
    c->vit_seq = c->vit_tokens + (cfg->vit_class_token ? 1 : 0);
    c->vit_kpad = (int)round_up(3 * cfg->vit_patch * cfg->vit_patch, 64);
    c->vit_ipad = (int)round_up(cfg->vit_intermediate, 64);
    c->qkv_w = cfg->vision_only ? 0 : (cfg->num_heads + 2 * cfg->num_kv_heads) * cfg->head_dim;
    { const char* nf = getenv("MMDUET_NO_FUSE"); c->no_fuse = nf && nf[0] == '1'; c->no_pm = nf && (nf[0] == '1' || nf[0] == '2'); }
    { const char* nf = getenv("MMDUET_NO_CHAIN"); c->no_chain = nf && nf[0] == '1'; }
    { const char* nf = getenv("MMDUET_NO_SLAB_NORM"); c->no_slab_norm = nf && nf[0] == '1'; }
    { const char* nf = getenv("MMDUET_FULL_LAST_LAYER"); c->full_last_layer = nf && nf[0] == '1'; }
    { const char* nf = getenv("MMDUET_NO_ROPE_FUSE"); c->no_rope_fuse = nf && nf[0] == '1'; }
    { const char* ng = getenv("MMDUET_GRAPH"); c->no_graph = !(ng && ng[0] == '1'); }
    *out = c;
    return MMD_OK;
}

extern "C" void mmd_destroy(mmd_ctx* c) {
    if (!c) return;
    hipSetDevice(c->device);
    hipStreamSynchronize(c->stream);
    prof_drain(c);
    for (auto e : c->prof.pool) hipEventDestroy(e);
    for (void* p : c->allocs) hipFree(p);
    if (c->heads_host) hipHostFree(c->heads_host);
    if (c->rows_host) hipHostFree(c->rows_host);
    if (c->tok_host) hipHostFree(c->tok_host);
    if (c->step_host) hipHostFree(c->step_host);
    if (c->seg_host) hipHostFree(c->seg_host);
    if (c->round_toks_host) hipHostFree(c->round_toks_host);
    for (auto& ev : c->seg_event) if (ev) hipEventDestroy(ev);
    if (c->dec_graph) hipGraphExecDestroy(c->dec_graph);
    if (c->dec_graph_src) hipGraphDestroy(c->dec_graph_src);
    hipStreamDestroy(c->own_stream);
    delete c;
}

extern "C" const char* mmd_last_error(const mmd_ctx* c) { return c ? c->err.c_str() : g_create_error.c_str(); }
extern "C" int mmd_set_tower_share(mmd_ctx* c, int max_blocks) {
    if (!c || max_blocks < 0) return MMD_EINVAL;
    c->tower_ring_blocks = max_blocks; if (c->tower_ring_flags < 0) c->tower_ring_flags = 16;
    return MMD_OK;
}
extern "C" int mmd_set_stream(mmd_ctx* c, void* s) { if (!c) return MMD_EINVAL; c->stream = (hipStream_t)s; return MMD_OK; }
extern "C" void* mmd_get_stream(mmd_ctx* c) { return c ? (void*)c->stream : nullptr; }
extern "C" int mmd_synchronize(mmd_ctx* c) { if (!c) return MMD_EINVAL; HIPCHK(c, hipStreamSynchronize(c->stream)); return MMD_OK; }
extern "C" int64_t mmd_weight_bytes(const mmd_ctx* c) { return c ? c->weight_bytes : 0; }

static std::string canon_name(const char* name) {
    std::string n(name);
    const std::string a = "model.vision_tower.vision_tower.vision_model.", b = "model.vision_tower.vision_tower.";
    if (n.compare(0, a.size(), a) == 0) return "vit." + n.substr(a.size());
    if (n.compare(0, b.size(), b) == 0) return "vit." + n.substr(b.size());
    return n;
}

extern "C" int mmd_load_tensor(mmd_ctx* c, const char* name, const void* data, int src_dtype, const int64_t* shape, int rank, int on_device) {
    if (!c || !name || !data || rank < 1 || rank > 4) return MMD_EINVAL;
    if (c->finalized) FAIL(c, MMD_EINVAL, "weights already finalized");
    if (src_dtype != MMD_F32 && src_dtype != MMD_BF16) FAIL(c, MMD_EINVAL, "unsupported source dtype %d for %s", src_dtype, name);
    hipSetDevice(c->device);
    RawTensor t;
    t.numel = 1;
    for (int i = 0; i < rank; ++i) { t.shape.push_back(shape[i]); t.numel *= shape[i]; }
    int rc = dev_alloc(c, &t.p, (size_t)t.numel * es(c), false);
    if (rc) return rc;
    const void* src = data;
    void* staging = nullptr;
    if (!on_device) {
        size_t sb = (size_t)t.numel * dtype_size(src_dtype);
        if (src_dtype == c->cfg.dtype) {
            HIPCHK(c, hipMemcpyAsync(t.p, data, sb, hipMemcpyHostToDevice, c->stream));
            HIPCHK(c, hipStreamSynchronize(c->stream));
            src = nullptr;
        } else {
            HIPCHK(c, hipMalloc(&staging, sb));
            HIPCHK(c, hipMemcpyAsync(staging, data, sb, hipMemcpyHostToDevice, c->stream));
            src = staging;
        }
    }
    if (src) {
        HIPCHK(c, launch_convert(src, src_dtype, t.p, c->cfg.dtype, t.numel, c->stream));
        if (staging) { HIPCHK(c, hipStreamSynchronize(c->stream)); hipFree(staging); }
    }
    std::string key = canon_name(name);
    auto it = c->raw.find(key);
    if (it != c->raw.end()) dev_free(c, it->second.p);
    c->raw[key] = t;
    return MMD_OK;
}

// ... 195 lines not shown
        { TAKE(t, "vit.head.mlp.fc1.weight", {CI, C}); c->hd_w1 = t.p; } { TAKE(t, "vit.head.mlp.fc1.bias", {CI}); c->hd_b1 = t.p; }
        { TAKE(t, "vit.head.mlp.fc2.weight", {C, CI}); c->hd_w2 = t.p; } { TAKE(t, "vit.head.mlp.fc2.bias", {C}); c->hd_b2 = t.p; }
    }
    for (auto& kv : c->raw) dev_free(c, kv.second.p);
    c->raw.clear();
    if (!c->inv_freq_user && !g.vision_only) {
        int n = d / 2;
        std::vector<float> t(n);
        for (int i = 0; i < n; ++i) t[i] = (float)(1.0 / std::pow((double)g.rope_theta, (double)(2 * i) / (double)d));
        if (!c->inv_freq) { int rc = dev_alloc(c, (void**)&c->inv_freq, sizeof(float) * n); if (rc) return rc; }
        HIPCHK(c, hipMemcpyAsync(c->inv_freq, t.data(), sizeof(float) * n, hipMemcpyHostToDevice, st));
        HIPCHK(c, hipStreamSynchronize(st));
    }
    size_t wb = 0; { size_t fr = 0, tot = 0; (void)fr; (void)tot; }
    wb = ((size_t)2 * V * H + (size_t)g.num_layers * ((size_t)c->qkv_w * H + (size_t)H * nh * d + (size_t)3 * I * H) +
          (size_t)g.vit_layers * ((size_t)4 * C * C + (size_t)2 * c->vit_ipad * C) + (size_t)C * c->vit_kpad + (size_t)H * C + (size_t)H * H) * e;
    if (g.weight_dtype == MMD_W_FP8_E4M3) wb += (size_t)g.num_layers * ((size_t)c->qkv_w * H + (size_t)H * nh * d + (size_t)3 * I * H);
    c->weight_bytes = (int64_t)wb;
    int rc = alloc_workspaces(c);
    if (rc) return rc;
    HIPCHK(c, hipStreamSynchronize(st));
    c->finalized = true;
    return MMD_OK;
}

static size_t splitk_ws_size(const mmd_config& g) { return (size_t)(g.max_step_tokens > 2048 ? 192 : 64) << 20; }

static int alloc_workspaces(mmd_ctx* c) {
    const mmd_config& g = c->cfg; const size_t e = es(c);
    const int C = g.vit_hidden, H = g.hidden_size;
    int64_t Mv = round_up((int64_t)g.max_vit_batch * c->vit_seq, 128);
    int rc;
#define WS(ptr, bytes) rc = dev_alloc(c, (void**)&(ptr), (bytes)); if (rc) return rc;
    WS(c->v_col, (size_t)Mv * c->vit_kpad * e); WS(c->v_h, (size_t)Mv * C * e); WS(c->v_xn, (size_t)Mv * C * e);
    if (g.tower_f16 == 1) {
        const int pout_ = (c->vit_grid + g.pool_stride - 1) / g.pool_stride;
        c->v_h32_rows = Mv; WS(c->v_h32, (size_t)(Mv + (int64_t)g.max_vit_batch * 4 * pout_ * pout_) * C * sizeof(float));
    }
    WS(c->v_qkv, (size_t)Mv * 3 * C * e); WS(c->v_attn, (size_t)Mv * C * e); WS(c->v_mlp, (size_t)round_up(Mv, 16) * c->vit_ipad * e);
    if (g.vit_class_token) { WS(c->v_patch, (size_t)Mv * C * e); }
    c->v_splitk_bytes = (size_t)32 << 20; WS(c->v_splitk_ws, c->v_splitk_bytes);
    c->v_attn_bytes = (size_t)32 << 20; WS(c->v_attn_ws, c->v_attn_bytes);
    if (g.vit_pool_head) {
        const size_t Bm = (size_t)g.max_vit_batch;
        WS(c->hd_q, (size_t)C * e); WS(c->hd_kv, (size_t)Mv * 2 * C * e); WS(c->hd_a, Bm * C * e); WS(c->hd_h, Bm * C * e); WS(c->hd_n, Bm * C * e);
        WS(c->hd_m, Bm * g.vit_intermediate * e);
    }
    if (g.vision_only) return MMD_OK;
    WS(c->v_p1, (size_t)Mv * H * e); WS(c->v_p2, (size_t)Mv * H * e);
    int64_t S = round_up(g.max_step_tokens, 128);
    WS(c->l_h, (size_t)S * H * e); WS(c->l_xn, (size_t)S * H * e); WS(c->l_qkv, (size_t)S * c->qkv_w * e);
    WS(c->l_q, (size_t)S * g.num_heads * g.head_dim * e); WS(c->l_attn, (size_t)S * g.num_heads * g.head_dim * e);
    WS(c->l_act, (size_t)round_up(S, 16) * g.intermediate_size * e); WS(c->l_hid, (size_t)S * H * e);
    c->splitk_bytes = splitk_ws_size(g); WS(c->splitk_ws, c->splitk_bytes);
    WS(c->chain_ssq, (size_t)GEMV_CHAIN_ROWS * GEMV_SSQ_STRIDE * sizeof(float)); WS(c->rope_tab, (size_t)S * 64 * 2 * sizeof(float));
    c->attn_bytes = (size_t)128 << 20; WS(c->attn_ws, c->attn_bytes);
    WS(c->logits_ws, (size_t)g.vocab_size * sizeof(float));
    WS(c->heads_dev, (size_t)S * 4 * sizeof(float)); WS(c->rows_dev, (size_t)S * sizeof(int32_t));
    WS(c->tok_dev, 64); WS(c->argmax_scratch, 1024); c->prev_cap = 16384; WS(c->prev_dev, (size_t)c->prev_cap * sizeof(int64_t));
    WS(c->gen_embed, (size_t)H * e);
#undef WS
    HIPCHK(c, hipHostMalloc((void**)&c->heads_host, (size_t)S * 4 * sizeof(float)));
    HIPCHK(c, hipHostMalloc((void**)&c->rows_host, (size_t)S * sizeof(int32_t)));
    HIPCHK(c, hipHostMalloc((void**)&c->tok_host, 64));
    HIPCHK(c, hipHostMalloc((void**)&c->step_host, sizeof(StepState)));
    HIPCHK(c, hipHostMalloc((void**)&c->seg_host, 8 * 64 * sizeof(StepState)));
    rc = dev_alloc(c, (void**)&c->seg_dev, 8 * 64 * sizeof(StepState)); if (rc) return rc;
    rc = dev_alloc(c, (void**)&c->step_dev, sizeof(StepState)); if (rc) return rc;
    return MMD_OK;
}

#define NEED_FINAL(c) do { if (!(c)) return MMD_EINVAL; if (!(c)->finalized) FAIL(c, MMD_EINVAL, "weights not finalized"); hipSetDevice((c)->device); } while (0)

static int connector_pool(mmd_ctx* c, const void* feats, int B, void* out);
static int ensure_preprocess_tables(mmd_ctx* c, int T, int R);
static int vit_tower(mmd_ctx* c, const void* px, int B, bool col_ready = false, bool for_pool = false) {
    const mmd_config& g = c->cfg; hipStream_t st = c->stream;
    const int dt = g.tower_f16 ? MMD_F16 : g.dtype;
    struct HalfScope { mmd_ctx* c; HalfScope(mmd_ctx* c_, bool on) : c(c_) { c->gemm_half = on; } ~HalfScope() { c->gemm_half = false; } } half_scope(c, g.tower_f16 != 0);
    if (B > g.max_vit_batch) FAIL(c, MMD_ERANGE, "vit batch %d exceeds max_vit_batch %d", B, g.max_vit_batch);
    const int C = g.vit_hidden, T = c->vit_tokens, TS = c->vit_seq, M = B * TS, hd = C / g.vit_heads;
    if (!col_ready) { ProfScope ps(c, MMD_K_OTHER, 0, 0); HIPCHK(c, launch_im2col(g.tower_f16 ? MMD_F16 + 1 : dt, px, B, g.vit_image, g.vit_patch, c->vit_grid, c->vit_kpad, c->v_col, st)); }
    const bool r32 = g.tower_f16 == 1;
    void* patch_out = g.vit_class_token ? c->v_patch : (r32 ? c->v_xn : c->v_h);
    int rc = gemm(c, c->v_col, c->vit_kpad, c->patch_w, c->vit_kpad, c->patch_b, nullptr, 0, patch_out, C, B * T, C, c->vit_kpad, EPI_NONE, 0, GEMM_AUTO, c->patch_w_p, true); if (rc) return rc;
    if (r32) {
        ProfScope ps(c, MMD_K_NORM_ROPE, 12.0 * M * C, 0);
        if (g.vit_layers > 0) { HIPCHK(c, launch_resid32_layernorm(c->v_xn, c->v_h32, c->pos_emb, T, c->VL[0].ln1w, c->VL[0].ln1b, c->v_xn, nullptr, M, C, g.vit_ln_eps, st)); }
        else { HIPCHK(c, launch_resid32_layernorm(c->v_xn, c->v_h32, c->pos_emb, T, nullptr, nullptr, nullptr, c->v_h, M, C, g.vit_ln_eps, st)); }
    } else if (g.vit_class_token) {
        ProfScope ps(c, MMD_K_OTHER, 0, 0); HIPCHK(c, launch_assemble_cls(dt, c->v_patch, c->cls_emb, c->pos_emb, B, T, C, c->v_h, st));
    } else {
        ProfScope ps(c, MMD_K_OTHER, 0, 0); HIPCHK(c, launch_add_rows(dt, c->v_h, c->pos_emb, M, C, T, st));
    }
    if (g.vit_pre_layernorm) { HIPCHK(c, launch_layernorm(dt, c->v_h, c->pre_w, c->pre_b, c->v_h, M, C, g.vit_ln_eps, st)); }
    const int pout = (c->vit_grid + g.pool_stride - 1) / g.pool_stride, U = 4 * pout * pout;
    const bool sparse_last = for_pool && !c->full_tower && !c->full_projector && g.pool_mode == MMD_POOL_BILINEAR && U < T && TS == T && !g.vit_post_layernorm &&
                             g.vit_act != 1 && g.vit_layers > 0 && !g.vision_only && (!g.tower_f16 || (U >= 64 && B * U > 64));
    c->last_sparse = sparse_last;
    c->tower_compact = false;
    for (int i = 0; i < g.vit_layers; ++i) {
        VitLayer& L = c->VL[i];
        if (!r32) { ProfScope ps(c, MMD_K_NORM_ROPE, 2.0 * M * C * es(c), 0); HIPCHK(c, launch_layernorm(dt, c->v_h, L.ln1w, L.ln1b, c->v_xn, M, C, g.vit_ln_eps, st)); }
        rc = gemm(c, c->v_xn, C, L.wqkv, C, L.bqkv, nullptr, 0, c->v_qkv, 3 * C, M, 3 * C, C, EPI_NONE, 0, GEMM_AUTO, L.wqkv_p, true); if (rc) return rc;
        if (sparse_last && i + 1 == g.vit_layers) {
            const int Mc = B * U;
            void* qc = c->v_mlp; void* hc = c->v_col;
            { ProfScope ps(c, MMD_K_OTHER, 0, 0);
              HIPCHK(c, launch_gather_pool_rows(dt == MMD_F32 ? MMD_F32 : MMD_BF16, c->v_qkv, qc, B, c->vit_grid, C, pout, st, 3 * C));
              if (r32) { HIPCHK(c, launch_gather_pool_rows(MMD_F32, c->v_h32, c->v_h32 + c->v_h32_rows * C, B, c->vit_grid, C, pout, st, C)); }
              else { HIPCHK(c, launch_gather_pool_rows(dt == MMD_F32 ? MMD_F32 : MMD_BF16, c->v_h, hc, B, c->vit_grid, C, pout, st, C)); } }
            {
                AttnArgs a; memset(&a, 0, sizeof(a));
                a.q = qc; a.ldq = C; a.K = (char*)c->v_qkv + (size_t)C * es(c); a.V = (char*)c->v_qkv + (size_t)2 * C * es(c);
                a.k_hs = hd; a.k_ts = 3 * C; a.v_hs = hd; a.v_ts = 3 * C; a.out = c->v_attn; a.ldo = C;
                a.S = U; a.nh = g.vit_heads; a.nkv = g.vit_heads; a.d = hd; a.n_ctx = TS - U; a.causal = 0;
                a.batch = B; a.q_bstride = (int64_t)U * C; a.kv_bstride = (int64_t)TS * 3 * C; a.o_bstride = (int64_t)U * C;
                a.ws = c->v_attn_ws; a.ws_bytes = c->v_attn_bytes; a.variant = 0;
                ProfScope ps(c, MMD_K_ATTN_VIT, 2.0 * (M + Mc) * C * es(c), 4.0 * B * (double)U * TS * C);
                HIPCHK(c, launch_attention(dt, a, st));
            }
            if (r32) {
                float* hc32 = c->v_h32 + c->v_h32_rows * C;
                rc = gemm(c, c->v_attn, C, L.wo, C, L.bo, nullptr, 0, c->v_xn, C, Mc, C, C, EPI_NONE, 0, GEMM_AUTO, L.wo_p, true); if (rc) return rc;
                { ProfScope ps(c, MMD_K_NORM_ROPE, 12.0 * Mc * C, 0); HIPCHK(c, launch_resid32_layernorm(c->v_xn, hc32, nullptr, 1, L.ln2w, L.ln2b, c->v_xn, nullptr, Mc, C, g.vit_ln_eps, st)); }
                const bool pm = gemm_pair_pm(c, true, c->v_xn, C, L.w1_p, L.b1, c->vit_ipad, C, EPI_GELU_TANH, c->v_mlp, c->vit_ipad, L.w2_p, C, nullptr, 0, c->v_xn, C, EPI_NONE, Mc);
                rc = gemm(c, c->v_xn, C, L.w1, C, L.b1, nullptr, 0, c->v_mlp, c->vit_ipad, Mc, c->vit_ipad, C, EPI_GELU_TANH, 0, GEMM_AUTO, L.w1_p, true, nullptr, nullptr, nullptr, nullptr, pm ? 2 : 0); if (rc) return rc;
                rc = gemm(c, c->v_mlp, c->vit_ipad, L.w2, c->vit_ipad, L.b2, nullptr, 0, c->v_xn, C, Mc, C, c->vit_ipad, EPI_NONE, 0, GEMM_AUTO, L.w2_p, true, nullptr, nullptr, nullptr, nullptr, pm ? 1 : 0); if (rc) return rc;
                { ProfScope ps(c, MMD_K_NORM_ROPE, 8.0 * Mc * C, 0); HIPCHK(c, launch_resid32_layernorm(c->v_xn, hc32, nullptr, 1, nullptr, nullptr, nullptr, hc, Mc, C, g.vit_ln_eps, st)); }
                c->tower_compact = true;
                c->last_vit_B = B;
                return MMD_OK;
            }
            rc = gemm(c, c->v_attn, C, L.wo, C, L.bo, hc, C, hc, C, Mc, C, C, EPI_RESID, 0, GEMM_AUTO, L.wo_p, true); if (rc) return rc;
            { ProfScope ps(c, MMD_K_NORM_ROPE, 2.0 * Mc * C * es(c), 0); HIPCHK(c, launch_layernorm(dt, hc, L.ln2w, L.ln2b, c->v_xn, Mc, C, g.vit_ln_eps, st)); }
            const bool pm = gemm_pair_pm(c, true, c->v_xn, C, L.w1_p, L.b1, c->vit_ipad, C, EPI_GELU_TANH, c->v_mlp, c->vit_ipad, L.w2_p, C, hc, C, hc, C, EPI_RESID, Mc);
            rc = gemm(c, c->v_xn, C, L.w1, C, L.b1, nullptr, 0, c->v_mlp, c->vit_ipad, Mc, c->vit_ipad, C, EPI_GELU_TANH, 0, GEMM_AUTO, L.w1_p, true, nullptr, nullptr, nullptr, nullptr, pm ? 2 : 0); if (rc) return rc;
            rc = gemm(c, c->v_mlp, c->vit_ipad, L.w2, c->vit_ipad, L.b2, hc, C, hc, C, Mc, C, c->vit_ipad, EPI_RESID, 0, GEMM_AUTO, L.w2_p, true, nullptr, nullptr, nullptr, nullptr, pm ? 1 : 0); if (rc) return rc;
            if (g.tower_f16) { ProfScope ps(c, MMD_K_OTHER, 0, 0); HIPCHK(c, launch_convert(hc, MMD_F16, hc, MMD_BF16, (int64_t)Mc * C, st)); }
            c->tower_compact = true;
            c->last_vit_B = B;
            return MMD_OK;
        }
        {
            AttnArgs a; memset(&a, 0, sizeof(a));
            a.q = c->v_qkv; a.ldq = 3 * C; a.K = (char*)c->v_qkv + (size_t)C * es(c); a.V = (char*)c->v_qkv + (size_t)2 * C * es(c);
            a.k_hs = hd; a.k_ts = 3 * C; a.v_hs = hd; a.v_ts = 3 * C; a.out = c->v_attn; a.ldo = C;
            a.S = TS; a.nh = g.vit_heads; a.nkv = g.vit_heads; a.d = hd; a.n_ctx = 0; a.causal = 0;
            a.batch = B; a.q_bstride = (int64_t)TS * 3 * C; a.kv_bstride = (int64_t)TS * 3 * C; a.o_bstride = (int64_t)TS * C;
            a.ws = c->v_attn_ws; a.ws_bytes = c->v_attn_bytes; a.variant = 0;
            ProfScope ps(c, MMD_K_ATTN_VIT, 4.0 * M * C * es(c), 4.0 * B * (double)TS * TS * C);
            HIPCHK(c, launch_attention(dt, a, st));
        }
        if (r32) {
            rc = gemm(c, c->v_attn, C, L.wo, C, L.bo, nullptr, 0, c->v_xn, C, M, C, C, EPI_NONE, 0, GEMM_AUTO, L.wo_p, true); if (rc) return rc;
            { ProfScope ps(c, MMD_K_NORM_ROPE, 12.0 * M * C, 0); HIPCHK(c, launch_resid32_layernorm(c->v_xn, c->v_h32, nullptr, 1, L.ln2w, L.ln2b, c->v_xn, nullptr, M, C, g.vit_ln_eps, st)); }
            const bool pm = gemm_pair_pm(c, true, c->v_xn, C, L.w1_p, L.b1, c->vit_ipad, C, EPI_GELU_TANH, c->v_mlp, c->vit_ipad, L.w2_p, C, nullptr, 0, c->v_xn, C, EPI_NONE, M);
            rc = gemm(c, c->v_xn, C, L.w1, C, L.b1, nullptr, 0, c->v_mlp, c->vit_ipad, M, c->vit_ipad, C, EPI_GELU_TANH, 0, GEMM_AUTO, L.w1_p, true, nullptr, nullptr, nullptr, nullptr, pm ? 2 : 0); if (rc) return rc;
            rc = gemm(c, c->v_mlp, c->vit_ipad, L.w2, c->vit_ipad, L.b2, nullptr, 0, c->v_xn, C, M, C, c->vit_ipad, EPI_NONE, 0, GEMM_AUTO, L.w2_p, true, nullptr, nullptr, nullptr, nullptr, pm ? 1 : 0); if (rc) return rc;
            ProfScope ps(c, MMD_K_NORM_ROPE, 12.0 * M * C, 0);
            if (i + 1 < g.vit_layers) { HIPCHK(c, launch_resid32_layernorm(c->v_xn, c->v_h32, nullptr, 1, c->VL[i + 1].ln1w, c->VL[i + 1].ln1b, c->v_xn, nullptr, M, C, g.vit_ln_eps, st)); }
            else { HIPCHK(c, launch_resid32_layernorm(c->v_xn, c->v_h32, nullptr, 1, nullptr, nullptr, nullptr, c->v_h, M, C, g.vit_ln_eps, st)); }
            continue;
        }
        rc = gemm(c, c->v_attn, C, L.wo, C, L.bo, c->v_h, C, c->v_h, C, M, C, C, EPI_RESID, 0, GEMM_AUTO, L.wo_p, true); if (rc) return rc;
        { ProfScope ps(c, MMD_K_NORM_ROPE, 2.0 * M * C * es(c), 0); HIPCHK(c, launch_layernorm(dt, c->v_h, L.ln2w, L.ln2b, c->v_xn, M, C, g.vit_ln_eps, st)); }
        bool pm = false;
        if (g.vit_act == 1) {
            rc = gemm(c, c->v_xn, C, L.w1, C, L.b1, nullptr, 0, c->v_mlp, c->vit_ipad, M, c->vit_ipad, C, EPI_NONE, 0, GEMM_AUTO, L.w1_p, true); if (rc) return rc;
            HIPCHK(c, launch_quick_gelu(dt, c->v_mlp, (int64_t)M * c->vit_ipad, st));
        } else {
            pm = gemm_pair_pm(c, true, c->v_xn, C, L.w1_p, L.b1, c->vit_ipad, C, EPI_GELU_TANH, c->v_mlp, c->vit_ipad, L.w2_p, C, c->v_h, C, c->v_h, C, EPI_RESID, M);
            rc = gemm(c, c->v_xn, C, L.w1, C, L.b1, nullptr, 0, c->v_mlp, c->vit_ipad, M, c->vit_ipad, C, EPI_GELU_TANH, 0, GEMM_AUTO, L.w1_p, true, nullptr, nullptr, nullptr, nullptr, pm ? 2 : 0); if (rc) return rc;
        }
        rc = gemm(c, c->v_mlp, c->vit_ipad, L.w2, c->vit_ipad, L.b2, c->v_h, C, c->v_h, C, M, C, c->vit_ipad, EPI_RESID, 0, GEMM_AUTO, L.w2_p, true, nullptr, nullptr, nullptr, nullptr, pm ? 1 : 0); if (rc) return rc;
    }
    if (g.vit_post_layernorm) { HIPCHK(c, launch_layernorm(dt, c->v_h, c->post_w, c->post_b, c->v_h, M, C, g.vit_ln_eps, st)); }
    if (g.tower_f16 && !r32) { ProfScope ps(c, MMD_K_OTHER, 0, 0); HIPCHK(c, launch_convert(c->v_h, MMD_F16, c->v_h, MMD_BF16, (int64_t)M * C, st)); }
    c->last_vit_B = B;
    return MMD_OK;
}

extern "C" int mmd_vit_encode(mmd_ctx* c, const void* px, int B, void* out) {
    NEED_FINAL(c);
    if (B <= 0) return MMD_OK;
    if (c->cfg.vision_only) FAIL(c, MMD_EINVAL, "vision-only context: use mmd_vision_tower");
    int rc = vit_tower(c, px, B, false, true); if (rc) return rc;
    return connector_pool(c, c->tower_compact ? c->v_col : c->v_h, B, out);
}

extern "C" int mmd_vit_encode_frames(mmd_ctx* c, const uint8_t* frames, int B, int R, void* out) {
    NEED_FINAL(c);
    if (B <= 0) return MMD_OK;
    if (!frames || !out) return MMD_EINVAL;
    if (c->cfg.vision_only) FAIL(c, MMD_EINVAL, "vision-only context: use mmd_vision_tower");
    if (B > c->cfg.max_vit_batch) FAIL(c, MMD_ERANGE, "vit batch %d exceeds max_vit_batch %d", B, c->cfg.max_vit_batch);
    int rc = ensure_preprocess_tables(c, B, R); if (rc) return rc;
    { ProfScope ps(c, MMD_K_OTHER, 0, 0);
      HIPCHK(c, launch_preprocess_im2col(c->cfg.tower_f16 ? MMD_F16 : c->cfg.dtype, frames, B, R, c->cfg.vit_image, c->pp_coef, c->pp_bounds, c->pp_ksize, c->pp_tmp, c->cfg.vit_patch, c->vit_grid,
                                         c->vit_kpad, c->v_col, c->stream)); }
    rc = vit_tower(c, nullptr, B, true, true); if (rc) return rc;
    return connector_pool(c, c->tower_compact ? c->v_col : c->v_h, B, out);
}

extern "C" int mmd_normalize_frames(mmd_ctx* c, const void* frames, int src_kind, int B, int R, const float* mean, const float* sd, float rescale, void* out) {
    if (!c || !frames || !out || !mean || !sd || (src_kind != 0 && src_kind != 1)) return MMD_EINVAL;
    hipSetDevice(c->device);
    HIPCHK(c, launch_normalize_frames(c->cfg.dtype, frames, src_kind, B, R, rescale, mean, sd, out, c->stream));
    return MMD_OK;
}
extern "C" int mmd_vision_tower(mmd_ctx* c, const void* px, int B, void* out) {
    NEED_FINAL(c);
    if (B <= 0) return MMD_OK;
    if (!px || !out) return MMD_EINVAL;
    int rc = vit_tower(c, px, B); if (rc) return rc;
    HIPCHK(c, hipMemcpyAsync(out, c->v_h, (size_t)B * c->vit_seq * c->cfg.vit_hidden * es(c), hipMemcpyDeviceToDevice, c->stream));
    return MMD_OK;
}
extern "C" int mmd_vision_pool_tokens(mmd_ctx* c, const void* feats, int B, int out_h, int out_w, void* out) {
    NEED_FINAL(c);
    if (B <= 0) return MMD_OK;
    if (!feats || !out || out_h <= 0 || out_h != out_w) FAIL(c, MMD_EINVAL, "pool target must be square (frame_token_pooled = [%d, %d])", out_h, out_w);
    const int C = c->cfg.vit_hidden, T = c->vit_tokens, TS = c->vit_seq; const size_t e = es(c);
    for (int b = 0; b < B; ++b) {
        const char* src = (const char*)feats + ((size_t)b * TS + (TS - T)) * C * e;
        HIPCHK(c, launch_pool(c->cfg.dtype, src, (char*)out + (size_t)b * out_h * out_w * C * e, 1, c->vit_grid, C, MMD_POOL_ADAPTIVE_AVG, out_h, c->stream));
    }
    return MMD_OK;
}
extern "C" int mmd_vision_pool_head(mmd_ctx* c, const void* feats, int B, void* out) {
    NEED_FINAL(c);
    if (B <= 0) return MMD_OK;
    const mmd_config& g = c->cfg; const int dt = g.dtype; hipStream_t st = c->stream; const size_t e = es(c);
    if (!g.vit_pool_head) FAIL(c, MMD_EINVAL, "this tower has no pooling head");
    if (B > g.max_vit_batch) FAIL(c, MMD_ERANGE, "batch %d exceeds max_vit_batch %d", B, g.max_vit_batch);
    const int C = g.vit_hidden, CI = g.vit_intermediate, TS = c->vit_seq, hd = C / g.vit_heads;
    int rc = gemm(c, c->hd_probe, C, c->hd_wq, C, c->hd_bq, nullptr, 0, c->hd_q, C, 1, C, C, EPI_NONE, 0, GEMM_AUTO, nullptr, true); if (rc) return rc;
    rc = gemm(c, feats, C, c->hd_wkv, C, c->hd_bkv, nullptr, 0, c->hd_kv, 2 * C, B * TS, 2 * C, C, EPI_NONE, 0, GEMM_AUTO, nullptr, true); if (rc) return rc;
    {
        AttnArgs a; memset(&a, 0, sizeof(a));
        a.q = c->hd_q; a.ldq = C; a.K = c->hd_kv; a.V = (char*)c->hd_kv + (size_t)C * e;
        a.k_hs = hd; a.k_ts = 2 * C; a.v_hs = hd; a.v_ts = 2 * C; a.out = c->hd_a; a.ldo = C;
        a.S = 1; a.nh = g.vit_heads; a.nkv = g.vit_heads; a.d = hd; a.n_ctx = TS - 1; a.causal = 0;
        a.batch = B; a.q_bstride = 0; a.kv_bstride = (int64_t)TS * 2 * C; a.o_bstride = C;
        a.ws = c->v_attn_ws; a.ws_bytes = c->v_attn_bytes; a.variant = 1;
// ... 905 lines not shown
extern "C" int mmd_prof_reset(mmd_ctx* c) {
    if (!c) return MMD_EINVAL;
    prof_drain(c);
    for (int i = 0; i < MMD_K_COUNT; ++i) { c->prof.ms[i] = 0; c->prof.n[i] = 0; c->prof.bytes[i] = 0; c->prof.flops[i] = 0; c->prof.seen[i] = 0; }
    return MMD_OK;
}
extern "C" int mmd_prof_read(mmd_ctx* c, double* ms, int64_t* n, double* bytes, double* flops) {
    if (!c) return MMD_EINVAL;
    prof_drain(c);
    for (int i = 0; i < MMD_K_COUNT; ++i) { if (ms) ms[i] = c->prof.ms[i]; if (n) n[i] = c->prof.n[i]; if (bytes) bytes[i] = c->prof.bytes[i]; if (flops) flops[i] = c->prof.flops[i]; }
    return MMD_OK;
}

extern "C" int mmd_op_gemm(mmd_ctx* c, const void* X, const void* W, const void* bias, const void* R, void* Y, int M, int N, int K, int epi,
                           int out_f32, int variant) {
    if (!c) return MMD_EINVAL;
    hipSetDevice(c->device);
    if (!c->splitk_ws) { c->splitk_bytes = splitk_ws_size(c->cfg); int rc = dev_alloc(c, (void**)&c->splitk_ws, c->splitk_bytes); if (rc) return rc; }
    int NO = epi == EPI_SWIGLU ? N / 2 : N;
    void* Wp = nullptr;
    if (variant == GEMM_AUTO || variant == GEMM_SKINNY || variant == GEMM_BIG || variant == GEMM_RING256 || variant == GEMM_RING256_SPLIT || variant == GEMM_STREAM || variant >= GEMM_RINGX) { int rc = make_packed(c, W, N, K, &Wp); if (rc) return rc; }
    int rc = gemm(c, X, K, W, K, bias, R, NO, Y, NO, M, N, K, epi, out_f32, variant, Wp);
    if (Wp) { hipStreamSynchronize(c->stream); dev_free(c, Wp); }
    return rc;
}
extern "C" int mmd_op_gemm_slabs(mmd_ctx* c, const void* X, const void* W, int M, int N, int K, int variant, float* slabs_out, int max_splits, int* splits_out) {
    if (!c || !X || !W || !slabs_out || !splits_out || max_splits < 1) return MMD_EINVAL;
    if (M <= 0 || N <= 0 || K <= 0 || M > 256 || (N % 16) != 0 || (K % 32) != 0 || (variant != GEMM_SKINNY && variant != GEMM_STREAM)) FAIL(c, MMD_EINVAL, "gemm_slabs: 1 <= M <= 256, N %% 16 == 0, K %% 32 == 0, variant 2 or 8");
    hipSetDevice(c->device);
    void* Wp = nullptr;
    int rc = make_packed(c, W, N, K, &Wp); if (rc) return rc;
    GemmArgs g; memset(&g, 0, sizeof(g));
    int splits = 0;
    g.X = X; g.ldx = K; g.Wp = Wp; g.M = M; g.N = N; g.K = K; g.epi = EPI_NONE; g.variant = variant;
    g.splitk_ws = slabs_out; g.splitk_ws_bytes = (size_t)max_splits * M * N * sizeof(float); g.slabs_out = &splits; g.plan_out = c->last_plan;
    if (!Wp || !gemm_can_slab(c->cfg.dtype, g)) { if (Wp) dev_free(c, Wp); FAIL(c, MMD_EINVAL, "gemm_slabs: no slab kernel takes M = %d, N = %d, K = %d in this context's dtype", M, N, K); }
    hipError_t e = launch_gemm(c->cfg.dtype, g, c->stream);
    hipStreamSynchronize(c->stream);
    dev_free(c, Wp);
    if (e != hipSuccess) FAIL(c, MMD_EHIP, "slab GEMM launch failed: %s", hipGetErrorString(e));
    *splits_out = splits;
    return MMD_OK;
}
extern "C" int mmd_op_quantize_fp8(mmd_ctx* c, void* W, int N, int K, uint8_t* q8_out, float* scale_out) {
    if (!c || !W || !q8_out || !scale_out) return MMD_EINVAL;
    if (c->cfg.dtype != MMD_BF16) FAIL(c, MMD_EINVAL, "fp8 weights need a bf16 context");
    hipSetDevice(c->device);
    HIPCHK(c, launch_quantize_fp8_rows(W, N, K, q8_out, scale_out, c->stream));
    return MMD_OK;
}
extern "C" int mmd_op_gemm_w8(mmd_ctx* c, const void* X, const void* Wq, const uint8_t* q8, const float* scale, const void* bias, const void* R, void* Y,
                              int M, int N, int K, int epi, int out_f32, int variant) {
    if (!c || !X || !Wq || !q8 || !scale || !Y) return MMD_EINVAL;
    if (c->cfg.dtype != MMD_BF16 || (N % 16) != 0 || (K % 64) != 0) FAIL(c, MMD_EINVAL, "mmd_op_gemm_w8: bf16 context, N %% 16 == 0, K %% 64 == 0");
    hipSetDevice(c->device);
    if (!c->splitk_ws) { c->splitk_bytes = splitk_ws_size(c->cfg); int rc = dev_alloc(c, (void**)&c->splitk_ws, c->splitk_bytes); if (rc) return rc; }
    void *Wp = nullptr, *Wp8 = nullptr;
    int rc = make_packed(c, Wq, N, K, &Wp); if (rc) return rc;
    rc = dev_alloc(c, &Wp8, (size_t)N * K, false); if (rc) return rc;
    HIPCHK(c, launch_pack_w8(q8, N, K, Wp8, c->stream));
    const int NO = epi == EPI_SWIGLU ? N / 2 : N;
    rc = gemm(c, X, K, Wq, K, bias, R, NO, Y, NO, M, N, K, epi, out_f32, variant, Wp, false, Wp8, scale);
    hipStreamSynchronize(c->stream);
    dev_free(c, Wp); dev_free(c, Wp8);
    return rc;
}
extern "C" int mmd_op_gemm_pair(mmd_ctx* c, const void* X, const void* W1, const void* b1, int epi1, const void* W2, const void* R, void* Y, int M, int N1, int K1, int N2,
                                int piece_major, int* used_pm_out) {
    if (!c || !X || !W1 || !W2 || !Y) return MMD_EINVAL;
    hipSetDevice(c->device);
    if (!c->splitk_ws) { c->splitk_bytes = splitk_ws_size(c->cfg); int rc = dev_alloc(c, (void**)&c->splitk_ws, c->splitk_bytes); if (rc) return rc; }
    const int T = epi1 == EPI_SWIGLU ? N1 / 2 : N1;
    void *W1p = nullptr, *W2p = nullptr, *mid = nullptr; int rc;
    if ((rc = make_packed(c, W1, N1, K1, &W1p)) || (rc = make_packed(c, W2, N2, T, &W2p)) || (rc = dev_alloc(c, &mid, (size_t)round_up(M, 16) * T * es(c)))) return rc;
    const int epi2 = R ? EPI_RESID : EPI_NONE;
    const bool pm = piece_major && gemm_pair_pm(c, false, X, K1, W1p, b1, N1, K1, epi1, mid, T, W2p, N2, R, N2, Y, N2, epi2, M);
    if (used_pm_out) *used_pm_out = pm ? 1 : 0;
    rc = gemm(c, X, K1, W1, K1, b1, nullptr, 0, mid, T, M, N1, K1, epi1, 0, GEMM_AUTO, W1p, false, nullptr, nullptr, nullptr, nullptr, pm ? 2 : 0);
    if (!rc) rc = gemm(c, mid, T, W2, T, nullptr, R, N2, Y, N2, M, N2, T, epi2, 0, GEMM_AUTO, W2p, false, nullptr, nullptr, nullptr, nullptr, pm ? 1 : 0);
    hipStreamSynchronize(c->stream);
    dev_free(c, W1p); dev_free(c, W2p); dev_free(c, mid);
    return rc;
}
extern "C" int mmd_op_attention_last_form(mmd_ctx* c, int* out2) { if (!c || !out2) return MMD_EINVAL; out2[0] = c->last_form[0]; out2[1] = c->last_form[1]; return MMD_OK; }
extern "C" int mmd_op_gemm_last_plan(mmd_ctx* c, int* out4) {
    if (!c || !out4) return MMD_EINVAL;
    for (int i = 0; i < 4; ++i) out4[i] = c->last_plan[i];
    return MMD_OK;
}
extern "C" int mmd_op_gemm_bench(mmd_ctx* c, int M, int N, int K, int epi, int variant, int iters, float* avg_ms_out, const void* Xin, const void* Win) {
    if (!c || !avg_ms_out || iters <= 0) return MMD_EINVAL;
    hipSetDevice(c->device);
    if (!c->splitk_ws) { c->splitk_bytes = splitk_ws_size(c->cfg); int rc = dev_alloc(c, (void**)&c->splitk_ws, c->splitk_bytes); if (rc) return rc; }
    const size_t e = es(c);
    int NO = epi == EPI_SWIGLU ? N / 2 : N;
    void *X = nullptr, *W = nullptr, *Y = nullptr, *R = nullptr, *Wp = nullptr;
    int rc;
    if ((rc = dev_alloc(c, &X, (size_t)M * K * e)) || (rc = dev_alloc(c, &W, (size_t)N * K * e)) || (rc = dev_alloc(c, &Y, (size_t)M * NO * e)) ||
        (rc = dev_alloc(c, &R, (size_t)M * NO * e))) return rc;
    if (Xin) HIPCHK(c, hipMemcpyAsync(X, Xin, (size_t)M * K * e, hipMemcpyDeviceToDevice, c->stream)); else HIPCHK(c, hipMemsetAsync(X, 0x3c, (size_t)M * K * e, c->stream));
    if (Win) HIPCHK(c, hipMemcpyAsync(W, Win, (size_t)N * K * e, hipMemcpyDeviceToDevice, c->stream)); else HIPCHK(c, hipMemsetAsync(W, 0x3b, (size_t)N * K * e, c->stream));
    if (Xin) HIPCHK(c, hipMemcpyAsync(R, Xin, std::min((size_t)M * K, (size_t)M * NO) * e, hipMemcpyDeviceToDevice, c->stream));
    void* Wp8 = nullptr; float* wsc = nullptr;
    if (variant >= 1000) { variant -= 1000; rc = quantize_fp8(c, W, N, K, &Wp8, &wsc); if (rc) return rc; }
    if (variant != GEMM_GENERIC && variant != GEMM_LARGE) { rc = make_packed(c, W, N, K, &Wp); if (rc) return rc; }
    if (variant == 5 && !Wp) FAIL(c, MMD_EINVAL, "slab mode needs a packable shape");
    hipEvent_t a, b; hipEventCreate(&a); hipEventCreate(&b);
    unsigned was = c->prof.on; c->prof.on = 0;
    int slabs = 0;
    auto run = [&]() -> int {
        if (variant == 5) {
            GemmArgs g; memset(&g, 0, sizeof(g));
            g.X = X; g.ldx = K; g.Wp = Wp; g.Wp8 = Wp8; g.wscale = wsc; g.M = M; g.N = N; g.K = K; g.epi = EPI_NONE; g.variant = GEMM_SKINNY;
            g.splitk_ws = c->splitk_ws; g.splitk_ws_bytes = c->splitk_bytes; g.slabs_out = &slabs;
            return launch_gemm(c->cfg.dtype, g, c->stream) == hipSuccess ? MMD_OK : MMD_EHIP;
        }
        return gemm(c, X, K, W, K, nullptr, epi == EPI_RESID ? R : nullptr, NO, Y, NO, M, N, K, epi, 0, variant, Wp, false, Wp8, wsc);
    };
    for (int i = 0; i < 3; ++i) { rc = run(); if (rc) return rc; }
    hipEventRecord(a, c->stream);
    for (int i = 0; i < iters; ++i) run();
    hipEventRecord(b, c->stream);
    hipEventSynchronize(b);
    float ms = 0; hipEventElapsedTime(&ms, a, b);
    *avg_ms_out = ms / iters;
    c->prof.on = was;
    hipEventDestroy(a); hipEventDestroy(b);
    dev_free(c, X); dev_free(c, W); dev_free(c, Y); dev_free(c, R); if (Wp) dev_free(c, Wp); if (Wp8) dev_free(c, Wp8); if (wsc) dev_free(c, wsc);
    return MMD_OK;
}
extern "C" int mmd_op_rmsnorm(mmd_ctx* c, const void* x, const void* w, void* y, int M, int H, float eps) {
    if (!c) return MMD_EINVAL; hipSetDevice(c->device);
    HIPCHK(c, launch_rmsnorm(c->cfg.dtype, x, w, y, M, H, eps, c->stream)); return MMD_OK;
}
extern "C" int mmd_op_layernorm(mmd_ctx* c, const void* x, const void* w, const void* b, void* y, int M, int H, float eps) {
    if (!c) return MMD_EINVAL; hipSetDevice(c->device);
    HIPCHK(c, launch_layernorm(c->cfg.dtype, x, w, b, y, M, H, eps, c->stream)); return MMD_OK;
}
extern "C" int mmd_op_resid32_layernorm(mmd_ctx* c, const void* y16, float* h32, const void* pos16, int period, const void* w16, const void* b16, void* out16, void* outbf,
                                        int M, int H, float eps) {
    if (!c) return MMD_EINVAL; hipSetDevice(c->device);
    if (!y16 || !h32 || (w16 && (!b16 || !out16)) || (pos16 && period <= 0)) FAIL(c, MMD_EINVAL, "resid32_layernorm: missing operand");
    if (outbf && w16) FAIL(c, MMD_EINVAL, "resid32_layernorm: outbf (the tower's final bf16 result: h32 is not rewritten) and a LayerNorm output are exclusive");
    HIPCHK(c, launch_resid32_layernorm(y16, h32, pos16, period, w16, b16, out16, outbf, M, H, eps, c->stream)); return MMD_OK;
}
extern "C" int mmd_op_rope_append(mmd_ctx* c, void* qkv, int S, int nh, int nkv, int d, float theta, int64_t pos0, void* q_out, void* Kc, void* Vc, int64_t cap) {
    if (!c) return MMD_EINVAL; hipSetDevice(c->device);
    std::vector<float> t(d / 2);
    for (int i = 0; i < d / 2; ++i) t[i] = (float)(1.0 / std::pow((double)theta, (double)(2 * i) / (double)d));
    float* dev = nullptr;
    HIPCHK(c, hipMalloc((void**)&dev, sizeof(float) * (d / 2)));
    HIPCHK(c, hipMemcpyAsync(dev, t.data(), sizeof(float) * (d / 2), hipMemcpyHostToDevice, c->stream));
    HIPCHK(c, launch_rope_append(c->cfg.dtype, qkv, S, nh, nkv, d, dev, pos0, q_out, Kc, Vc, cap, 0, c->stream));
    HIPCHK(c, hipStreamSynchronize(c->stream));
    hipFree(dev);
    return MMD_OK;
}
extern "C" int mmd_op_attention(mmd_ctx* c, const void* q, const void* Kc, const void* Vc, void* out, int S, int nh, int nkv, int d, int64_t n_ctx,
                                int64_t cap, int causal, int variant) {
    if (!c) return MMD_EINVAL; hipSetDevice(c->device);
    if (!c->attn_ws) { c->attn_bytes = (size_t)128 << 20; int rc = dev_alloc(c, (void**)&c->attn_ws, c->attn_bytes); if (rc) return rc; }
    AttnArgs a; memset(&a, 0, sizeof(a));
    a.q = q; a.ldq = (int64_t)nh * d; a.K = Kc; a.V = Vc; a.k_hs = cap * d; a.k_ts = d; a.v_hs = cap * d; a.v_ts = d; a.out = out; a.ldo = (int64_t)nh * d;
    a.S = S; a.nh = nh; a.nkv = nkv; a.d = d; a.n_ctx = n_ctx; a.causal = causal; a.batch = 1; a.ws = c->attn_ws; a.ws_bytes = c->attn_bytes; a.variant = variant;
    void* vt = nullptr;
    if (variant == 3 || variant == 5 || variant == 6) {
        if (cap % 64 != 0) FAIL(c, MMD_EINVAL, "variant 3 needs cap %% 64 == 0");
        int rc = dev_alloc(c, &vt, (size_t)nkv * cap * d * es(c)); if (rc) return rc;
        HIPCHK(c, launch_transpose_v(c->cfg.dtype, Vc, vt, nkv, cap, d, c->stream));
        a.V = vt; a.v_transposed = 1;
    }
    hipError_t le = launch_attention(c->cfg.dtype, a, c->stream);
    attn_last_form(c->last_form);
    if (vt) { hipStreamSynchronize(c->stream); dev_free(c, vt); }
    HIPCHK(c, le);
    return MMD_OK;
}
extern "C" int mmd_op_attention_bench(mmd_ctx* c, int S, int nh, int nkv, int d, int64_t n_ctx, int variant, int iters, float* avg_ms_out) {
    if (!c || !avg_ms_out || iters <= 0) return MMD_EINVAL;
    hipSetDevice(c->device);
    if (!c->attn_ws) { c->attn_bytes = (size_t)128 << 20; int rc = dev_alloc(c, (void**)&c->attn_ws, c->attn_bytes); if (rc) return rc; }
    const size_t e = es(c);
    int64_t cap = round_up(n_ctx + S, 64);
    void *q = nullptr, *K = nullptr, *V = nullptr, *o = nullptr; int rc;
    if ((rc = dev_alloc(c, &q, (size_t)S * nh * d * e)) || (rc = dev_alloc(c, &K, (size_t)nkv * cap * d * e)) || (rc = dev_alloc(c, &V, (size_t)nkv * cap * d * e)) ||
        (rc = dev_alloc(c, &o, (size_t)S * nh * d * e))) return rc;
    HIPCHK(c, hipMemsetAsync(q, 0x3c, (size_t)S * nh * d * e, c->stream));
    HIPCHK(c, hipMemsetAsync(K, 0x3b, (size_t)nkv * cap * d * e, c->stream));
    HIPCHK(c, hipMemsetAsync(V, 0x3c, (size_t)nkv * cap * d * e, c->stream));
    AttnArgs a; memset(&a, 0, sizeof(a));
    a.q = q; a.ldq = (int64_t)nh * d; a.K = K; a.V = V; a.k_hs = cap * d; a.k_ts = d; a.v_hs = cap * d; a.v_ts = d; a.out = o; a.ldo = (int64_t)nh * d;
    a.S = S; a.nh = nh; a.nkv = nkv; a.d = d; a.n_ctx = n_ctx; a.causal = 1; a.batch = 1; a.ws = c->attn_ws; a.ws_bytes = c->attn_bytes; a.variant = variant;
    a.v_transposed = 1;
    hipEvent_t ea, eb; hipEventCreate(&ea); hipEventCreate(&eb);
    for (int i = 0; i < 3; ++i) HIPCHK(c, launch_attention(c->cfg.dtype, a, c->stream));
    hipEventRecord(ea, c->stream);
    for (int i = 0; i < iters; ++i) launch_attention(c->cfg.dtype, a, c->stream);
    hipEventRecord(eb, c->stream);
    hipEventSynchronize(eb);
    float ms = 0; hipEventElapsedTime(&ms, ea, eb);
    *avg_ms_out = ms / iters;
    hipEventDestroy(ea); hipEventDestroy(eb);
    dev_free(c, q); dev_free(c, K); dev_free(c, V); dev_free(c, o);
    return MMD_OK;
}
extern "C" int mmd_op_pool(mmd_ctx* c, const void* x, void* y, int B, int grid, int H, int mode, int stride) {
    if (!c) return MMD_EINVAL; hipSetDevice(c->device);
    HIPCHK(c, launch_pool(c->cfg.dtype, x, y, B, grid, H, mode, stride, c->stream)); return MMD_OK;
}
```

mmduet_amd/csrc/ops.hip:

```cpp
#include "common.h"
#include <type_traits>

template <typename T>
__global__ void rmsnorm_kernel(const T* __restrict__ x, const T* __restrict__ w, T* __restrict__ y, int M, int H, float eps) {
    int row = blockIdx.x * (blockDim.x >> 6) + (threadIdx.x >> 6);
    int lane = threadIdx.x & 63;
    if (row >= M) return;
    const T* xr = x + (long long)row * H;
    T* yr = y + (long long)row * H;
    float ss = 0.f;
    if constexpr (sizeof(T) == 2) {
        if ((H & 7) == 0) {
            for (int c = lane * 8; c < H; c += 512) {
                s16x8_t v = *reinterpret_cast<const s16x8_t*>(xr + c);
#pragma unroll
                for (int e = 0; e < 8; ++e) { float f = bf2f((bf16_t)v[e]); ss += f * f; }
            }
        } else for (int c = lane; c < H; c += 64) { float f = to_f<T>(xr[c]); ss += f * f; }
    } else for (int c = lane; c < H; c += 64) { float f = to_f<T>(xr[c]); ss += f * f; }
    ss = wave_sum(ss);
    float inv = rsqrtf(ss / (float)H + eps);
    if constexpr (sizeof(T) == 2) {
        if ((H & 7) == 0) {
            for (int c = lane * 8; c < H; c += 512) {
// ... 49 lines not shown
    dim3 grid(cdiv(M, 4)), block(256);
    if (dtype == MMD_F32) hipLaunchKernelGGL(rmsnorm_kernel<float>, grid, block, 0, st, (const float*)x, (const float*)w, (float*)y, M, H, eps);
    else hipLaunchKernelGGL(rmsnorm_kernel<bf16_t>, grid, block, 0, st, (const bf16_t*)x, (const bf16_t*)w, (bf16_t*)y, M, H, eps);
    return hipGetLastError();
}

template <typename T>
__global__ void layernorm_kernel(const T* __restrict__ x, const T* __restrict__ w, const T* __restrict__ b, T* __restrict__ y, int M, int H, float eps) {
    int row = blockIdx.x * (blockDim.x >> 6) + (threadIdx.x >> 6);
    int lane = threadIdx.x & 63;
    if (row >= M) return;
    const T* xr = x + (long long)row * H;
    T* yr = y + (long long)row * H;
    [[maybe_unused]] constexpr bool F16 = std::is_same<T, f16_t>::value;
    if constexpr (sizeof(T) == 2) {
        if ((H & 7) == 0 && H <= 2048) {
            float v[4][8];
            float s = 0.f;
#pragma unroll
            for (int j = 0; j < 4; ++j) {
                const int c = lane * 8 + j * 512;
                if (c < H) {
                    s16x8_t raw = *reinterpret_cast<const s16x8_t*>(xr + c);
#pragma unroll
                    for (int e = 0; e < 8; ++e) { v[j][e] = raw2f<F16>((uint16_t)raw[e]); s += v[j][e]; }
                }
            }
            const float mu = wave_sum(s) / (float)H;
            float q = 0.f;
#pragma unroll
            for (int j = 0; j < 4; ++j) {
                const int c = lane * 8 + j * 512;
                if (c < H) {
#pragma unroll
                    for (int e = 0; e < 8; ++e) { const float dlt = v[j][e] - mu; q += dlt * dlt; }
                }
            }
            const float inv = rsqrtf(wave_sum(q) / (float)H + eps);
#pragma unroll
            for (int j = 0; j < 4; ++j) {
                const int c = lane * 8 + j * 512;
                if (c < H) {
                    s16x8_t g = *reinterpret_cast<const s16x8_t*>(w + c), bb = *reinterpret_cast<const s16x8_t*>(b + c), o;
#pragma unroll
                    for (int e = 0; e < 8; ++e) o[e] = (short)f2raw<F16>((v[j][e] - mu) * inv * raw2f<F16>((uint16_t)g[e]) + raw2f<F16>((uint16_t)bb[e]));
                    *reinterpret_cast<s16x8_t*>(yr + c) = o;
                }
            }
            return;
        }
    }
    float s = 0.f;
    for (int c = lane; c < H; c += 64) s += to_f<T>(xr[c]);
    float mu = wave_sum(s) / (float)H;
    float v = 0.f;
    for (int c = lane; c < H; c += 64) { float d = to_f<T>(xr[c]) - mu; v += d * d; }
    float inv = rsqrtf(wave_sum(v) / (float)H + eps);
    for (int c = lane; c < H; c += 64) yr[c] = from_f<T>((to_f<T>(xr[c]) - mu) * inv * to_f<T>(w[c]) + to_f<T>(b[c]));
}

hipError_t launch_layernorm(int dtype, const void* x, const void* w, const void* b, void* y, int M, int H, float eps, hipStream_t st) {
    if (M <= 0) return hipSuccess;
    dim3 grid(cdiv(M, 4)), block(256);
    if (dtype == MMD_F32) hipLaunchKernelGGL(layernorm_kernel<float>, grid, block, 0, st, (const float*)x, (const float*)w, (const float*)b, (float*)y, M, H, eps);
    else if (dtype == MMD_F16) hipLaunchKernelGGL(layernorm_kernel<f16_t>, grid, block, 0, st, (const f16_t*)x, (const f16_t*)w, (const f16_t*)b, (f16_t*)y, M, H, eps);
    else hipLaunchKernelGGL(layernorm_kernel<bf16_t>, grid, block, 0, st, (const bf16_t*)x, (const bf16_t*)w, (const bf16_t*)b, (bf16_t*)y, M, H, eps);
    return hipGetLastError();
}

__global__ __launch_bounds__(256) void resid32_layernorm_kernel(const f16_t* y , float* __restrict__ h, const f16_t* __restrict__ pos, int period,
                                                                const f16_t* __restrict__ w, const f16_t* __restrict__ b, f16_t* out16, bf16_t* __restrict__ outbf,
                                                                int M, int H, float eps) {
    const int row = blockIdx.x * 4 + (threadIdx.x >> 6), lane = threadIdx.x & 63;
    if (row >= M) return;
    const f16_t* yr = y + (long long)row * H;
    float* hr = h + (long long)row * H;
    const f16_t* pr = pos ? pos + (long long)(row % period) * H : nullptr;
    float v[4][8];
    float s = 0.f;
#pragma unroll
    for (int j = 0; j < 4; ++j) {
        const int c = lane * 8 + j * 512;
        if (c < H) {
            const s16x8_t raw = *reinterpret_cast<const s16x8_t*>(yr + c);
            if (pr) {
                const s16x8_t pw = *reinterpret_cast<const s16x8_t*>(pr + c);
#pragma unroll
                for (int e = 0; e < 8; ++e) v[j][e] = h2f((uint16_t)pw[e]) + h2f((uint16_t)raw[e]);
            } else {
                const f32x4_t a0 = *reinterpret_cast<const f32x4_t*>(hr + c), a1 = *reinterpret_cast<const f32x4_t*>(hr + c + 4);
#pragma unroll
                for (int e = 0; e < 4; ++e) { v[j][e] = a0[e] + h2f((uint16_t)raw[e]); v[j][e + 4] = a1[e] + h2f((uint16_t)raw[e + 4]); }
            }
            if (!outbf) {
                *reinterpret_cast<f32x4_t*>(hr + c) = f32x4_t{v[j][0], v[j][1], v[j][2], v[j][3]};
                *reinterpret_cast<f32x4_t*>(hr + c + 4) = f32x4_t{v[j][4], v[j][5], v[j][6], v[j][7]};
            } else {
                s16x8_t o;
#pragma unroll
                for (int e = 0; e < 8; ++e) o[e] = (short)f2bf(v[j][e]);
                *reinterpret_cast<s16x8_t*>(outbf + (long long)row * H + c) = o;
            }
#pragma unroll
            for (int e = 0; e < 8; ++e) s += v[j][e];
        }
    }
    if (!w) return;
    const float mu = wave_sum(s) / (float)H;
    float q = 0.f;
#pragma unroll
    for (int j = 0; j < 4; ++j) {
        const int c = lane * 8 + j * 512;
        if (c < H) {
#pragma unroll
            for (int e = 0; e < 8; ++e) { const float dlt = v[j][e] - mu; q += dlt * dlt; }
        }
    }
    const float inv = rsqrtf(wave_sum(q) / (float)H + eps);
#pragma unroll
    for (int j = 0; j < 4; ++j) {
        const int c = lane * 8 + j * 512;
        if (c < H) {
            const s16x8_t g = *reinterpret_cast<const s16x8_t*>(w + c), bb = *reinterpret_cast<const s16x8_t*>(b + c);
            s16x8_t o;
#pragma unroll
            for (int e = 0; e < 8; ++e) o[e] = (short)f2h((v[j][e] - mu) * inv * h2f((uint16_t)g[e]) + h2f((uint16_t)bb[e]));
            *reinterpret_cast<s16x8_t*>(out16 + (long long)row * H + c) = o;
        }
    }
}

hipError_t launch_resid32_layernorm(const void* y16, float* h32, const void* pos16, int period, const void* ln_w, const void* ln_b, void* out16, void* outbf,
                                    int M, int H, float eps, hipStream_t st) {
    if (M <= 0) return hipSuccess;
    if ((H & 7) || H > 2048) return hipErrorInvalidValue;
    hipLaunchKernelGGL(resid32_layernorm_kernel, dim3(cdiv(M, 4)), dim3(256), 0, st, (const f16_t*)y16, h32, (const f16_t*)pos16, period, (const f16_t*)ln_w, (const f16_t*)ln_b,
                       (f16_t*)out16, (bf16_t*)outbf, M, H, eps);
    return hipGetLastError();
}

template <int MAXS>
__global__ __launch_bounds__(256) void slab_resid_rmsnorm_kernel(const float* __restrict__ slabs, int splits, int M, int H, const bf16_t* __restrict__ resid,
                                                                 bf16_t* __restrict__ h_out, const bf16_t* __restrict__ w, float eps, bf16_t* __restrict__ xn,
                                                                 const float* __restrict__ wscale = nullptr) {
    __shared__ float red[4];
    const int m = blockIdx.x, tid = threadIdx.x;
    const long long MN = (long long)M * H;
    float hv[4][4];
    float ss = 0.f;
#pragma unroll
    for (int j = 0; j < 4; ++j) {
        const int c = tid * 4 + j * 1024;
        if (c < H) {
            const float* sp = slabs + (long long)m * H + c;
            f32x4_t part[MAXS];
#pragma unroll
            for (int s = 0; s < MAXS; ++s) part[s] = s < splits ? *reinterpret_cast<const f32x4_t*>(sp + s * MN) : f32x4_t{0, 0, 0, 0};
            s16x4_t r = *reinterpret_cast<const s16x4_t*>(resid + (long long)m * H + c);
            f32x4_t acc = part[0];
#pragma unroll
            for (int s = 1; s < MAXS; ++s) acc += part[s];
            if (wscale) acc *= *reinterpret_cast<const f32x4_t*>(wscale + c);
            s16x4_t o;
#pragma unroll
            for (int e = 0; e < 4; ++e) {
                float v = bf2f(f2bf(bf2f(f2bf(acc[e])) + bf2f((bf16_t)r[e])));
// ... 805 lines not shown
```

Baseline: 363.8.

## Fuse fp32 residual add into tower GEMM epilogues for out-proj and fc2

Adds an EPI_RESID32 GEMM epilogue that reads the fp32 residual stream, adds the fp16 GEMM output, and writes fp32 back in place. The vision tower's out-projection and fc2 GEMMs use it by default, and the following resid32_layernorm then just reads h32 instead of also reading an fp16 intermediate and rewriting h32. This removes one fp16 write/read round trip per fused GEMM and the layernorm's h32 write. The cost is heavier epilogue traffic (fp32 read+write inside the GEMM) and more restrictive plan eligibility, which falls back to an invalid plan for unsupported kernels. A microbenchmark entry point and a test op are also added.

```diff
diff --git a/include/mmduet.h b/include/mmduet.h
--- a/include/mmduet.h
+++ b/include/mmduet.h
@@ -138,6 +138,8 @@
 int mmd_op_gemm_bench(mmd_ctx* ctx, int M, int N, int K, int epi, int variant, int iters, float* avg_ms_out, const void* X, const void* W);
 int mmd_op_rmsnorm(mmd_ctx* ctx, const void* x, const void* w, void* y, int M, int H, float eps);
 int mmd_op_layernorm(mmd_ctx* ctx, const void* x, const void* w, const void* b, void* y, int M, int H, float eps);
+int mmd_op_gemm_f16(mmd_ctx* ctx, const void* X, const void* W, const void* bias, void* Y, float* h32, int64_t ldh, int M, int N, int K, int variant);
+int mmd_op_tower_resid_bench(mmd_ctx* ctx, int M, int N, int K, int fused, int iters, float* out3, const void* X, const void* W);
 int mmd_op_resid32_layernorm(mmd_ctx* ctx, const void* y16, float* h32, const void* pos16, int period, const void* w16, const void* b16, void* out16, void* outbf,
                              int M, int H, float eps);
 int mmd_op_rope_append(mmd_ctx* ctx, void* qkv, int S, int nh, int nkv, int d, float theta, int64_t pos0, void* q_out,
diff --git a/mmduet_amd/_lib.py b/mmduet_amd/_lib.py
--- a/mmduet_amd/_lib.py
+++ b/mmduet_amd/_lib.py
@@ -92,6 +92,8 @@
     'mmd_prof_read': (_I, [_VP, _VP, _VP, _VP, _VP]),
     'mmd_prof_reset': (_I, [_VP]),
     'mmd_op_gemm': (_I, [_VP, _VP, _VP, _VP, _VP, _VP, _I, _I, _I, _I, _I, _I]),
+    'mmd_op_gemm_f16': (_I, [_VP, _VP, _VP, _VP, _VP, _VP, C.c_int64, _I, _I, _I, _I]),
+    'mmd_op_tower_resid_bench': (_I, [_VP, _I, _I, _I, _I, _I, C.POINTER(_F), _VP, _VP]),
     'mmd_op_gemm_bench': (_I, [_VP, _I, _I, _I, _I, _I, _I, C.POINTER(_F), _VP, _VP]),
     'mmd_op_gemm_last_plan': (_I, [_VP, C.POINTER(_I)]),
     'mmd_op_gemm_pair': (_I, [_VP, _VP, _VP, _VP, _I, _VP, _VP, _VP, _I, _I, _I, _I, _I, C.POINTER(_I)]),
diff --git a/mmduet_amd/csrc/gemm.hip b/mmduet_amd/csrc/gemm.hip
--- a/mmduet_amd/csrc/gemm.hip
+++ b/mmduet_amd/csrc/gemm.hip
@@ -947,6 +947,28 @@
                 if constexpr (EPI == EPI_RESID) rq[i][j] = *reinterpret_cast<const s16x4_t*>((const bf16_t*)p.R + (long long)min(m0 + wm + i * 16 + lr, p.M - 1) * p.ldr + n0 + wn + j * 16 + lq * 4);
             }
     }
+    if constexpr (EPI == EPI_RESID32) {
+        f32x4_t hq[TM][TN];
+#pragma unroll
+        for (int i = 0; i < TM; ++i) {
+            const int m = m0 + wm + i * 16 + lr;
+#pragma unroll
+            for (int j = 0; j < TN; ++j) hq[i][j] = m < p.M ? *reinterpret_cast<const f32x4_t*>(p.R32 + (long long)m * p.ldr32 + n0 + wn + j * 16 + lq * 4) : f32x4_t{0, 0, 0, 0};
+        }
+#pragma unroll
+        for (int i = 0; i < TM; ++i) {
+            const int m = m0 + wm + i * 16 + lr;
+#pragma unroll
+            for (int j = 0; j < TN; ++j) {
+                const s16x4_t y = big_value_pre<EPI_NONE, F16>(acc[i][j], has_sc, scq[j], has_bi, biq[j], rq[i][j]);
+                f32x4_t o;
+#pragma unroll
+                for (int r = 0; r < 4; ++r) o[r] = hq[i][j][r] + raw2f<F16>((uint16_t)y[r]);
+                if (m < p.M) *reinterpret_cast<f32x4_t*>(p.R32 + (long long)m * p.ldr32 + n0 + wn + j * 16 + lq * 4) = o;
+            }
+        }
+        return;
+    }
 #pragma unroll
     for (int i = 0; i < TM; ++i) {
         const int m = m0 + wm + i * 16 + lr;
@@ -986,6 +1008,7 @@
         switch (p.epi) {
             case EPI_GELU_TANH: hipLaunchKernelGGL((gemm_big_kernel<BN, EPI_GELU_TANH, true>), grid, dim3(256), 0, st, p, KT); break;
             case EPI_RESID: hipLaunchKernelGGL((gemm_big_kernel<BN, EPI_RESID, true>), grid, dim3(256), 0, st, p, KT); break;
+            case EPI_RESID32: hipLaunchKernelGGL((gemm_big_kernel<BN, EPI_RESID32, true>), grid, dim3(256), 0, st, p, KT); break;
             default: hipLaunchKernelGGL((gemm_big_kernel<BN, EPI_NONE, true>), grid, dim3(256), 0, st, p, KT); break;
         }
         return;
@@ -1020,7 +1043,7 @@
     if (adev >= 0 && adev < 64 && !attr_set[adev]) {
 #define RX_ATTR(E) hipFuncSetAttribute((const void*)gemm_ringx_kernel<E, WN, M32, NS, EARLY, 0, F16>, hipFuncAttributeMaxDynamicSharedMemorySize, (int)smem);
         RX_ATTR(EPI_NONE) RX_ATTR(EPI_GELU_TANH) RX_ATTR(EPI_RESID)
-        if constexpr (!F16) { RX_ATTR(EPI_GELU_ERF) RX_ATTR(EPI_SWIGLU) }
+        if constexpr (!F16) { RX_ATTR(EPI_GELU_ERF) RX_ATTR(EPI_SWIGLU) } else { RX_ATTR(EPI_RESID32) }
 #undef RX_ATTR
         attr_set[adev] = true;
     }
@@ -1034,6 +1057,7 @@
         case EPI_GELU_ERF: if constexpr (!F16) RX_GO(EPI_GELU_ERF); break;
         case EPI_RESID: RX_GO(EPI_RESID); break;
         case EPI_SWIGLU: if constexpr (!F16) RX_GO(EPI_SWIGLU); break;
+        case EPI_RESID32: if constexpr (F16) RX_GO(EPI_RESID32); break;
         default: RX_GO(EPI_NONE); break;
     }
 #undef RX_GO
@@ -1108,7 +1132,7 @@
     GemmP p;
     p.X = a.X; p.W = pl.w_from == GEMM_W_PACKED8 ? a.Wp8 : (pl.w_from == GEMM_W_PACKED ? a.Wp : a.W); p.bias = a.bias; p.R = a.R; p.Y = a.Y; p.ws = a.splitk_ws; p.wscale = a.wscale;
     p.ldx = a.ldx; p.ldw = a.ldw; p.ldr = a.ldr; p.ldy = a.ldy;
-    p.M = a.M; p.N = a.N; p.K = a.K; p.epi = a.epi; p.out_f32 = a.out_f32; p.slabs = a.slabs_out ? 1 : 0; p.dump = nullptr; p.flags = 0; p.kper = pl.kper; p.x_pm = a.x_pm; p.y_pm = a.y_pm;
+    p.M = a.M; p.N = a.N; p.K = a.K; p.epi = a.epi; p.out_f32 = a.out_f32; p.slabs = a.slabs_out ? 1 : 0; p.dump = nullptr; p.flags = 0; p.kper = pl.kper; p.x_pm = a.x_pm; p.y_pm = a.y_pm; p.R32 = a.R32; p.ldr32 = a.ldr32;
     p.vec = (sizeof(T) == 2 && (a.ldx % 8) == 0 && (a.ldw % 8) == 0 && ((uintptr_t)a.X % 16) == 0 && ((uintptr_t)a.W % 16) == 0) ? 1 : 0;
     if (a.ring_slabs_out) *a.ring_slabs_out = pl.ring_slabs;
     if (pl.kernel == GEMM_PLAN_EMPTY) return hipSuccess;
diff --git a/mmduet_amd/csrc/gemm_plan.h b/mmduet_amd/csrc/gemm_plan.h
--- a/mmduet_amd/csrc/gemm_plan.h
+++ b/mmduet_amd/csrc/gemm_plan.h
@@ -8,7 +8,8 @@
 static inline int cdiv(int64_t a, int64_t b) { return (int)((a + b - 1) / b); }
 static inline int64_t round_up(int64_t a, int64_t b) { return (a + b - 1) / b * b; }
 
-enum { EPI_NONE = 0, EPI_GELU_TANH = 1, EPI_GELU_ERF = 2, EPI_RESID = 3, EPI_SWIGLU = 4 };
+enum { EPI_NONE = 0, EPI_GELU_TANH = 1, EPI_GELU_ERF = 2, EPI_RESID = 3, EPI_SWIGLU = 4,
+       EPI_RESID32 = 5  };
 enum { GEMM_AUTO = 0, GEMM_GENERIC = 1, GEMM_SKINNY = 2, GEMM_LARGE = 3, GEMM_BIG = 4, GEMM_SLAB = 5, GEMM_RING256 = 6, GEMM_RING256_SPLIT = 7,
        GEMM_RINGX = 16 ,
        GEMM_STREAM = 8  };
@@ -27,6 +28,7 @@
     const float* wscale = nullptr;
     const void* bias;
     const void* R; int64_t ldr;
+    float* R32 = nullptr; int64_t ldr32 = 0;
     void* Y; int64_t ldy;
     int M, N, K;
     int epi; int out_f32;
@@ -248,7 +250,7 @@
         case 17: WN = 2; break;
         default: return pl;
     }
-    if (a.f16 && a.epi != EPI_NONE && a.epi != EPI_GELU_TANH && a.epi != EPI_RESID) return pl;
+    if (a.f16 && a.epi != EPI_NONE && a.epi != EPI_GELU_TANH && a.epi != EPI_RESID && a.epi != EPI_RESID32) return pl;
     if (a.f16) splits = 1;
     while (splits > 1 && (a.epi == EPI_SWIGLU || !a.splitk_ws || (size_t)splits * a.M * a.N * sizeof(float) > a.splitk_ws_bytes)) --splits;
     const int BN = 64 * WN;
@@ -360,8 +362,11 @@
     if (dtype == MMD_F16 && !a.f16) { GemmArgs h = a; h.f16 = 1; return gemm_plan(dtype, h, tune); }
     GemmPlan pl;
     if (a.M <= 0 || a.N <= 0) { pl.kernel = GEMM_PLAN_EMPTY; return pl; }
+    if (a.epi == EPI_RESID32 && (!a.f16 || !a.R32 || ((uintptr_t)a.R32 % 16) != 0 || (a.ldr32 % 4) != 0 || a.ldr32 < a.N || a.y_pm || a.out_f32 || a.slabs_out || a.ring_slabs_out ||
+                                 a.variant == GEMM_RING256_SPLIT || (a.variant >= GEMM_RINGX && ((a.variant - GEMM_RINGX) & 4)))) return GemmPlan();
     pl = plan_kernel(dtype != MMD_F32, a, tune);
     if (!pl.valid()) return pl;
+    if (a.epi == EPI_RESID32 && ((pl.kernel != GEMM_K_RING256 && pl.kernel != GEMM_K_BIG64 && pl.kernel != GEMM_K_BIG128) || pl.splits != 1 || !pl.f16 || pl.bm == 160)) return GemmPlan();
     if ((a.x_pm || a.y_pm) && (pl.ring_auto == RING_AUTO_NONE || a.wscale || (a.x_pm && (a.K % 32)) || (a.y_pm && ((a.epi == EPI_SWIGLU ? a.N / 2 : a.N) % 32)))) return GemmPlan();
     if (a.y_pm && pl.ring_auto != RING_AUTO_PLAIN) return GemmPlan();
     const bool streaming = pl.kernel == GEMM_K_GEMV16 || pl.kernel == GEMM_K_SKINNY || pl.kernel == GEMM_K_STREAM;
diff --git a/mmduet_amd/csrc/gemm_ring.h b/mmduet_amd/csrc/gemm_ring.h
--- a/mmduet_amd/csrc/gemm_ring.h
+++ b/mmduet_amd/csrc/gemm_ring.h
@@ -13,6 +13,7 @@
     void* dump;
     int flags;
     int x_pm, y_pm;
+    float* R32; long long ldr32;
 };
 
 template <int EPI>
@@ -107,6 +108,7 @@
 template <int EPI, int WN, bool M32, int NS, bool EARLY, int DBG = 0, bool F16 = false>
 __global__ __launch_bounds__(WN * 128, 2) void gemm_ringx_kernel(GemmP p, int KT) {
     static_assert(!F16 || (!M32 && EPI != EPI_SWIGLU), "the fp16 form exists for the 16x16x32 schedule and the tower's epilogues");
+    static_assert(EPI != EPI_RESID32 || F16, "the fp32-residual epilogue belongs to the fp16 (autocast) tower");
     constexpr int BM = 256, BN = 64 * WN, BK = 32, NW = 2 * WN;
     constexpr int XE = BM * BK, WE = BN * BK, SE = XE + WE;
     constexpr int XP = (BM / 16) / NW, WP = (BN / 16) / NW;
@@ -187,7 +189,7 @@
     auto dma_k = [&](int slot, int step, int k) { if (k < XP) dma_x(slot, step, k); else if (k < XP + WP) dma_w(slot, step, k - XP); };
 
     constexpr int VM_ONE = NDMA, VM_TWO = 2 * NDMA;
-    constexpr int NST = EPI == EPI_SWIGLU ? 8 : 16;
+    constexpr int NST = EPI == EPI_SWIGLU ? 8 : (EPI == EPI_RESID32 ? 32 : 16);
 #ifdef MMDUET_NO_PST
     constexpr bool PST = false;
 #else
@@ -336,6 +338,15 @@
                     for (int j = 0; j < 4; ++j) rnext[j] = *reinterpret_cast<const s16x4_t*>((const bf16_t*)p.R + (long long)m * p.ldr + ncol[j]);
                 }
             }
+            [[maybe_unused]] f32x4_t hq[4], hnext[4];
+            [[maybe_unused]] auto h32_at = [&](int m, int j) -> float* {
+                const int nb = en0 + wc * 64 + j * 16;
+                return (m < p.M && nb + 16 <= p.N) ? p.R32 + (long long)m * p.ldr32 + nb + lq * 4 : (float*)p.dump + tid * 4;
+            };
+            if constexpr (EPI == EPI_RESID32) {
+#pragma unroll
+                for (int j = 0; j < 4; ++j) hnext[j] = *reinterpret_cast<const f32x4_t*>(h32_at(em0 + wr * 128 + lr, j));
+            }
             if constexpr (DBG == 4) {
 #pragma unroll
                 for (int i = 0; i < 8; ++i)
@@ -356,7 +367,23 @@
                     }
                     __builtin_amdgcn_sched_barrier(0);
                 }
-                if constexpr (EPI == EPI_SWIGLU) {
+                if constexpr (EPI == EPI_RESID32) {
+#pragma unroll
+                    for (int j = 0; j < 4; ++j) hq[j] = hnext[j];
+                    if (i < 7) {
+#pragma unroll
+                        for (int j = 0; j < 4; ++j) hnext[j] = *reinterpret_cast<const f32x4_t*>(h32_at(m + 16, j));
+                    }
+                    __builtin_amdgcn_sched_barrier(0);
+#pragma unroll
+                    for (int j = 0; j < 4; ++j) {
+                        const s16x4_t y = big_value_pre<EPI_NONE, F16>(acc[i][j], has_sc, scq[j], has_bi, biq[j], rq[j]);
+                        f32x4_t o;
+#pragma unroll
+                        for (int r = 0; r < 4; ++r) o[r] = hq[j][r] + raw2f<F16>((uint16_t)y[r]);
+                        *reinterpret_cast<f32x4_t*>(h32_at(m, j)) = o;
+                    }
+                } else if constexpr (EPI == EPI_SWIGLU) {
                     const int nb = en0 + wc * 64;
                     const int ob = (nb >> 5) * 16;
                     const int ns0 = min(nb, p.N - 32) + lq * 4, ns1 = min(nb + 32, p.N - 32) + lq * 4;
diff --git a/mmduet_amd/csrc/model.hip b/mmduet_amd/csrc/model.hip
--- a/mmduet_amd/csrc/model.hip
+++ b/mmduet_amd/csrc/model.hip
@@ -76,6 +76,7 @@
     int last_plan[4] = {-1, 0, 0, 0};
     bool no_fuse = false;
     bool no_pm = false;
+    int r32_epi = 3;
     bool gemm_half = false;
     int tower_ring_flags = -1, tower_ring_blocks = 0;
     int hid_compact = 0;
@@ -178,24 +179,27 @@
 }
 static int gemm(mmd_ctx* c, const void* X, int64_t ldx, const void* W, int64_t ldw, const void* bias, const void* R, int64_t ldr, void* Y,
                 int64_t ldy, int M, int N, int K, int epi, int out_f32 = 0, int variant = GEMM_AUTO, const void* Wp = nullptr, bool tower = false,
-                const void* Wp8 = nullptr, const float* wscale = nullptr, const GemvChain* chain = nullptr, int* ring_slabs_out = nullptr, int pm = 0) {
+                const void* Wp8 = nullptr, const float* wscale = nullptr, const GemvChain* chain = nullptr, int* ring_slabs_out = nullptr, int pm = 0,
+                float* R32 = nullptr, int64_t ldr32 = 0) {
     GemmArgs a = gemm_args(c, X, ldx, W, ldw, bias, R, ldr, Y, ldy, M, N, K, epi, out_f32, variant, Wp, tower, Wp8, wscale);
     a.chain = chain; a.ring_slabs_out = ring_slabs_out; a.x_pm = pm & 1; a.y_pm = (pm >> 1) & 1;
+    a.R32 = R32; a.ldr32 = ldr32;
     const int dt = c->gemm_half ? MMD_F16 : c->cfg.dtype;
     const GemmPlan pl = gemm_plan_for(dt, a);
     double e = (double)es(c);
-    double bytes = (double)M * K * e + (double)N * K * ((Wp8 && M <= 64) ? 1.0 : e) + (double)M * (epi == EPI_SWIGLU ? N / 2 : N) * (out_f32 ? 4.0 : e);
+    double bytes = (double)M * K * e + (double)N * K * ((Wp8 && M <= 64) ? 1.0 : e) + (double)M * (epi == EPI_SWIGLU ? N / 2 : N) * (epi == EPI_RESID32 ? 8.0 : out_f32 ? 4.0 : e);
     ProfScope ps(c, pl.prof_class, bytes, 2.0 * M * N * K);
     HIPCHK(c, launch_gemm(dt, a, c->stream, &pl));
     return MMD_OK;
 }
 
 static bool gemm_pair_pm(mmd_ctx* c, bool tower, const void* X1, int64_t ldx1, const void* W1p, const void* b1, int N1w, int K1, int epi1, void* T, int64_t ldt,
-                         const void* W2p, int N2, const void* R2, int64_t ldr2, void* Y2, int64_t ldy2, int epi2, int M) {
+                         const void* W2p, int N2, const void* R2, int64_t ldr2, void* Y2, int64_t ldy2, int epi2, int M, float* R32 = nullptr) {
     if (c->no_pm) return false;
     const int dt = c->gemm_half ? MMD_F16 : c->cfg.dtype;
     const GemmArgs a = gemm_args(c, X1, ldx1, nullptr, 0, b1, nullptr, 0, T, ldt, M, N1w, K1, epi1, 0, GEMM_AUTO, W1p, tower);
-    const GemmArgs b = gemm_args(c, T, ldt, nullptr, 0, nullptr, R2, ldr2, Y2, ldy2, M, N2, (int)ldt, epi2, 0, GEMM_AUTO, W2p, tower);
+    GemmArgs b = gemm_args(c, T, ldt, nullptr, 0, nullptr, R2, ldr2, Y2, ldy2, M, N2, (int)ldt, epi2, 0, GEMM_AUTO, W2p, tower);
+    b.R32 = R32; b.ldr32 = N2;
     return gemm_ring_auto(dt, a, true) && gemm_ring_auto(dt, b);
 }
 
@@ -225,6 +229,7 @@
     c->vit_ipad = (int)round_up(cfg->vit_intermediate, 64);
     c->qkv_w = cfg->vision_only ? 0 : (cfg->num_heads + 2 * cfg->num_kv_heads) * cfg->head_dim;
     { const char* nf = getenv("MMDUET_NO_FUSE"); c->no_fuse = nf && nf[0] == '1'; c->no_pm = nf && (nf[0] == '1' || nf[0] == '2'); }
+    { const char* re = getenv("MMDUET_R32_EPI"); if (re && re[0] >= '0' && re[0] <= '3') c->r32_epi = re[0] - '0'; if (c->no_fuse) c->r32_epi = 0; }
     { const char* nf = getenv("MMDUET_NO_CHAIN"); c->no_chain = nf && nf[0] == '1'; }
     { const char* nf = getenv("MMDUET_NO_SLAB_NORM"); c->no_slab_norm = nf && nf[0] == '1'; }
     { const char* nf = getenv("MMDUET_FULL_LAST_LAYER"); c->full_last_layer = nf && nf[0] == '1'; }
@@ -586,6 +591,8 @@
     const int C = g.vit_hidden, T = c->vit_tokens, TS = c->vit_seq, M = B * TS, hd = C / g.vit_heads;
     if (!col_ready) { ProfScope ps(c, MMD_K_OTHER, 0, 0); HIPCHK(c, launch_im2col(g.tower_f16 ? MMD_F16 + 1 : dt, px, B, g.vit_image, g.vit_patch, c->vit_grid, c->vit_kpad, c->v_col, st)); }
     const bool r32 = g.tower_f16 == 1;
+    void* const o_y = r32 && (c->r32_epi & 1) ? nullptr : c->v_xn; const int o_epi = o_y ? EPI_NONE : EPI_RESID32;
+    void* const fc2_y = r32 && (c->r32_epi & 2) ? nullptr : c->v_xn; const int fc2_epi = fc2_y ? EPI_NONE : EPI_RESID32;
     void* patch_out = g.vit_class_token ? c->v_patch : (r32 ? c->v_xn : c->v_h);
     int rc = gemm(c, c->v_col, c->vit_kpad, c->patch_w, c->vit_kpad, c->patch_b, nullptr, 0, patch_out, C, B * T, C, c->vit_kpad, EPI_NONE, 0, GEMM_AUTO, c->patch_w_p, true); if (rc) return rc;
     if (r32) {
@@ -626,12 +633,12 @@
             }
             if (r32) {
                 float* hc32 = c->v_h32 + c->v_h32_rows * C;
-                rc = gemm(c, c->v_attn, C, L.wo, C, L.bo, nullptr, 0, c->v_xn, C, Mc, C, C, EPI_NONE, 0, GEMM_AUTO, L.wo_p, true); if (rc) return rc;
-                { ProfScope ps(c, MMD_K_NORM_ROPE, 12.0 * Mc * C, 0); HIPCHK(c, launch_resid32_layernorm(c->v_xn, hc32, nullptr, 1, L.ln2w, L.ln2b, c->v_xn, nullptr, Mc, C, g.vit_ln_eps, st)); }
-                const bool pm = gemm_pair_pm(c, true, c->v_xn, C, L.w1_p, L.b1, c->vit_ipad, C, EPI_GELU_TANH, c->v_mlp, c->vit_ipad, L.w2_p, C, nullptr, 0, c->v_xn, C, EPI_NONE, Mc);
+                rc = gemm(c, c->v_attn, C, L.wo, C, L.bo, nullptr, 0, o_y, C, Mc, C, C, o_epi, 0, GEMM_AUTO, L.wo_p, true, nullptr, nullptr, nullptr, nullptr, 0, hc32, C); if (rc) return rc;
+                { ProfScope ps(c, MMD_K_NORM_ROPE, (o_y ? 12.0 : 6.0) * Mc * C, 0); HIPCHK(c, launch_resid32_layernorm(o_y, hc32, nullptr, 1, L.ln2w, L.ln2b, c->v_xn, nullptr, Mc, C, g.vit_ln_eps, st)); }
+                const bool pm = gemm_pair_pm(c, true, c->v_xn, C, L.w1_p, L.b1, c->vit_ipad, C, EPI_GELU_TANH, c->v_mlp, c->vit_ipad, L.w2_p, C, nullptr, 0, fc2_y, C, fc2_epi, Mc, hc32);
                 rc = gemm(c, c->v_xn, C, L.w1, C, L.b1, nullptr, 0, c->v_mlp, c->vit_ipad, Mc, c->vit_ipad, C, EPI_GELU_TANH, 0, GEMM_AUTO, L.w1_p, true, nullptr, nullptr, nullptr, nullptr, pm ? 2 : 0); if (rc) return rc;
-                rc = gemm(c, c->v_mlp, c->vit_ipad, L.w2, c->vit_ipad, L.b2, nullptr, 0, c->v_xn, C, Mc, C, c->vit_ipad, EPI_NONE, 0, GEMM_AUTO, L.w2_p, true, nullptr, nullptr, nullptr, nullptr, pm ? 1 : 0); if (rc) return rc;
-                { ProfScope ps(c, MMD_K_NORM_ROPE, 8.0 * Mc * C, 0); HIPCHK(c, launch_resid32_layernorm(c->v_xn, hc32, nullptr, 1, nullptr, nullptr, nullptr, hc, Mc, C, g.vit_ln_eps, st)); }
+                rc = gemm(c, c->v_mlp, c->vit_ipad, L.w2, c->vit_ipad, L.b2, nullptr, 0, fc2_y, C, Mc, C, c->vit_ipad, fc2_epi, 0, GEMM_AUTO, L.w2_p, true, nullptr, nullptr, nullptr, nullptr, pm ? 1 : 0, hc32, C); if (rc) return rc;
+                { ProfScope ps(c, MMD_K_NORM_ROPE, (fc2_y ? 8.0 : 6.0) * Mc * C, 0); HIPCHK(c, launch_resid32_layernorm(fc2_y, hc32, nullptr, 1, nullptr, nullptr, nullptr, hc, Mc, C, g.vit_ln_eps, st)); }
                 c->tower_compact = true;
                 c->last_vit_B = B;
                 return MMD_OK;
@@ -657,14 +664,14 @@
             HIPCHK(c, launch_attention(dt, a, st));
         }
         if (r32) {
-            rc = gemm(c, c->v_attn, C, L.wo, C, L.bo, nullptr, 0, c->v_xn, C, M, C, C, EPI_NONE, 0, GEMM_AUTO, L.wo_p, true); if (rc) return rc;
-            { ProfScope ps(c, MMD_K_NORM_ROPE, 12.0 * M * C, 0); HIPCHK(c, launch_resid32_layernorm(c->v_xn, c->v_h32, nullptr, 1, L.ln2w, L.ln2b, c->v_xn, nullptr, M, C, g.vit_ln_eps, st)); }
-            const bool pm = gemm_pair_pm(c, true, c->v_xn, C, L.w1_p, L.b1, c->vit_ipad, C, EPI_GELU_TANH, c->v_mlp, c->vit_ipad, L.w2_p, C, nullptr, 0, c->v_xn, C, EPI_NONE, M);
+            rc = gemm(c, c->v_attn, C, L.wo, C, L.bo, nullptr, 0, o_y, C, M, C, C, o_epi, 0, GEMM_AUTO, L.wo_p, true, nullptr, nullptr, nullptr, nullptr, 0, c->v_h32, C); if (rc) return rc;
+            { ProfScope ps(c, MMD_K_NORM_ROPE, (o_y ? 12.0 : 6.0) * M * C, 0); HIPCHK(c, launch_resid32_layernorm(o_y, c->v_h32, nullptr, 1, L.ln2w, L.ln2b, c->v_xn, nullptr, M, C, g.vit_ln_eps, st)); }
+            const bool pm = gemm_pair_pm(c, true, c->v_xn, C, L.w1_p, L.b1, c->vit_ipad, C, EPI_GELU_TANH, c->v_mlp, c->vit_ipad, L.w2_p, C, nullptr, 0, fc2_y, C, fc2_epi, M, c->v_h32);
             rc = gemm(c, c->v_xn, C, L.w1, C, L.b1, nullptr, 0, c->v_mlp, c->vit_ipad, M, c->vit_ipad, C, EPI_GELU_TANH, 0, GEMM_AUTO, L.w1_p, true, nullptr, nullptr, nullptr, nullptr, pm ? 2 : 0); if (rc) return rc;
-            rc = gemm(c, c->v_mlp, c->vit_ipad, L.w2, c->vit_ipad, L.b2, nullptr, 0, c->v_xn, C, M, C, c->vit_ipad, EPI_NONE, 0, GEMM_AUTO, L.w2_p, true, nullptr, nullptr, nullptr, nullptr, pm ? 1 : 0); if (rc) return rc;
-            ProfScope ps(c, MMD_K_NORM_ROPE, 12.0 * M * C, 0);
-            if (i + 1 < g.vit_layers) { HIPCHK(c, launch_resid32_layernorm(c->v_xn, c->v_h32, nullptr, 1, c->VL[i + 1].ln1w, c->VL[i + 1].ln1b, c->v_xn, nullptr, M, C, g.vit_ln_eps, st)); }
-            else { HIPCHK(c, launch_resid32_layernorm(c->v_xn, c->v_h32, nullptr, 1, nullptr, nullptr, nullptr, c->v_h, M, C, g.vit_ln_eps, st)); }
+            rc = gemm(c, c->v_mlp, c->vit_ipad, L.w2, c->vit_ipad, L.b2, nullptr, 0, fc2_y, C, M, C, c->vit_ipad, fc2_epi, 0, GEMM_AUTO, L.w2_p, true, nullptr, nullptr, nullptr, nullptr, pm ? 1 : 0, c->v_h32, C); if (rc) return rc;
+            ProfScope ps(c, MMD_K_NORM_ROPE, (fc2_y ? 12.0 : 6.0) * M * C, 0);
+            if (i + 1 < g.vit_layers) { HIPCHK(c, launch_resid32_layernorm(fc2_y, c->v_h32, nullptr, 1, c->VL[i + 1].ln1w, c->VL[i + 1].ln1b, c->v_xn, nullptr, M, C, g.vit_ln_eps, st)); }
+            else { HIPCHK(c, launch_resid32_layernorm(fc2_y, c->v_h32, nullptr, 1, nullptr, nullptr, nullptr, c->v_h, M, C, g.vit_ln_eps, st)); }
             continue;
         }
         rc = gemm(c, c->v_attn, C, L.wo, C, L.bo, c->v_h, C, c->v_h, C, M, C, C, EPI_RESID, 0, GEMM_AUTO, L.wo_p, true); if (rc) return rc;
@@ -1736,6 +1743,42 @@
     dev_free(c, W1p); dev_free(c, W2p); dev_free(c, mid);
     return rc;
 }
+extern "C" int mmd_op_gemm_f16(mmd_ctx* c, const void* X, const void* W, const void* bias, void* Y, float* h32, int64_t ldh, int M, int N, int K, int variant) {
+    if (!c || !X || !W || (!Y && !h32)) return MMD_EINVAL;
+    if (c->cfg.dtype != MMD_BF16 || (N % 16) != 0 || (K % 32) != 0) FAIL(c, MMD_EINVAL, "mmd_op_gemm_f16: bf16 context, N %% 16 == 0, K %% 32 == 0");
+    hipSetDevice(c->device);
+    void* Wp = nullptr;
+    int rc = make_packed(c, W, N, K, &Wp); if (rc) return rc;
+    struct HalfScope { mmd_ctx* c; HalfScope(mmd_ctx* c_) : c(c_) { c->gemm_half = true; } ~HalfScope() { c->gemm_half = false; } } half_scope(c);
+    rc = gemm(c, X, K, nullptr, K, bias, nullptr, 0, h32 ? nullptr : Y, N, M, N, K, h32 ? EPI_RESID32 : EPI_NONE, 0, variant, Wp, false, nullptr, nullptr, nullptr, nullptr, 0, h32, ldh);
+    hipStreamSynchronize(c->stream); dev_free(c, Wp);
+    return rc;
+}
+extern "C" int mmd_op_tower_resid_bench(mmd_ctx* c, int M, int N, int K, int fused, int iters, float* out3, const void* Xin, const void* Win) {
+    if (!c || !out3 || !Xin || !Win || iters <= 0) return MMD_EINVAL;
+    if (c->cfg.dtype != MMD_BF16 || (N % 16) != 0 || (K % 32) != 0 || (N & 7) || N > 2048) FAIL(c, MMD_EINVAL, "mmd_op_tower_resid_bench: bf16 context, N %% 16 == 0, N <= 2048, K %% 32 == 0");
+    hipSetDevice(c->device);
+    void *Wp = nullptr, *y = nullptr, *xn = nullptr, *h32 = nullptr, *lnw = nullptr; int rc;
+    if ((rc = make_packed(c, Win, N, K, &Wp)) || (rc = dev_alloc(c, &y, (size_t)M * N * 2)) || (rc = dev_alloc(c, &xn, (size_t)M * N * 2)) || (rc = dev_alloc(c, &h32, (size_t)M * N * 4)) ||
+        (rc = dev_alloc(c, &lnw, (size_t)N * 4))) return rc;
+    HIPCHK(c, hipMemsetAsync(h32, 0, (size_t)M * N * 4, c->stream)); HIPCHK(c, hipMemsetAsync(lnw, 0x38, (size_t)N * 4, c->stream));
+    struct HalfScope { mmd_ctx* c; HalfScope(mmd_ctx* c_) : c(c_) { c->gemm_half = true; } ~HalfScope() { c->gemm_half = false; } } half_scope(c);
+    unsigned was = c->prof.on; c->prof.on = 0;
+    auto g = [&]() -> int { return gemm(c, Xin, K, nullptr, K, nullptr, nullptr, 0, fused ? nullptr : y, N, M, N, K, fused ? EPI_RESID32 : EPI_NONE, 0, GEMM_AUTO, Wp, true, nullptr, nullptr, nullptr, nullptr, 0, (float*)h32, N); };
+    auto ln = [&]() -> int { return launch_resid32_layernorm(fused ? nullptr : y, (float*)h32, nullptr, 1, lnw, (char*)lnw + (size_t)N * 2, xn, nullptr, M, N, 1e-6f, c->stream) == hipSuccess ? MMD_OK : MMD_EHIP; };
+    hipEvent_t a, b; hipEventCreate(&a); hipEventCreate(&b);
+    for (int mode = 0; mode < 3 && !rc; ++mode) {
+        for (int i = 0; i < 3 && !rc; ++i) { if (mode != 1) rc = g(); if (!rc && mode != 0) rc = ln(); }
+        hipEventRecord(a, c->stream);
+        for (int i = 0; i < iters && !rc; ++i) { if (mode != 1) rc = g(); if (!rc && mode != 0) rc = ln(); }
+        hipEventRecord(b, c->stream); hipEventSynchronize(b);
+        float ms = 0; hipEventElapsedTime(&ms, a, b); out3[mode] = ms / iters;
+    }
+    c->prof.on = was;
+    hipEventDestroy(a); hipEventDestroy(b);
+    dev_free(c, Wp); dev_free(c, y); dev_free(c, xn); dev_free(c, h32); dev_free(c, lnw);
+    return rc;
+}
 extern "C" int mmd_op_attention_last_form(mmd_ctx* c, int* out2) { if (!c || !out2) return MMD_EINVAL; out2[0] = c->last_form[0]; out2[1] = c->last_form[1]; return MMD_OK; }
 extern "C" int mmd_op_gemm_last_plan(mmd_ctx* c, int* out4) {
     if (!c || !out4) return MMD_EINVAL;
@@ -1794,7 +1837,7 @@
 extern "C" int mmd_op_resid32_layernorm(mmd_ctx* c, const void* y16, float* h32, const void* pos16, int period, const void* w16, const void* b16, void* out16, void* outbf,
                                         int M, int H, float eps) {
     if (!c) return MMD_EINVAL; hipSetDevice(c->device);
-    if (!y16 || !h32 || (w16 && (!b16 || !out16)) || (pos16 && period <= 0)) FAIL(c, MMD_EINVAL, "resid32_layernorm: missing operand");
+    if (!h32 || (!y16 && pos16) || (w16 && (!b16 || !out16)) || (pos16 && period <= 0)) FAIL(c, MMD_EINVAL, "resid32_layernorm: missing operand");
     if (outbf && w16) FAIL(c, MMD_EINVAL, "resid32_layernorm: outbf (the tower's final bf16 result: h32 is not rewritten) and a LayerNorm output are exclusive");
     HIPCHK(c, launch_resid32_layernorm(y16, h32, pos16, period, w16, b16, out16, outbf, M, H, eps, c->stream)); return MMD_OK;
 }
diff --git a/mmduet_amd/csrc/ops.hip b/mmduet_amd/csrc/ops.hip
--- a/mmduet_amd/csrc/ops.hip
+++ b/mmduet_amd/csrc/ops.hip
@@ -155,6 +155,20 @@
     for (int j = 0; j < 4; ++j) {
         const int c = lane * 8 + j * 512;
         if (c < H) {
+            if (!y) {
+                const f32x4_t a0 = *reinterpret_cast<const f32x4_t*>(hr + c), a1 = *reinterpret_cast<const f32x4_t*>(hr + c + 4);
+#pragma unroll
+                for (int e = 0; e < 4; ++e) { v[j][e] = a0[e]; v[j][e + 4] = a1[e]; }
+                if (outbf) {
+                    s16x8_t o;
+#pragma unroll
+                    for (int e = 0; e < 8; ++e) o[e] = (short)f2bf(v[j][e]);
+                    *reinterpret_cast<s16x8_t*>(outbf + (long long)row * H + c) = o;
+                }
+#pragma unroll
+                for (int e = 0; e < 8; ++e) s += v[j][e];
+                continue;
+            }
             const s16x8_t raw = *reinterpret_cast<const s16x8_t*>(yr + c);
             if (pr) {
                 const s16x8_t pw = *reinterpret_cast<const s16x8_t*>(pr + c);
```

Result: no change. 362.9 (-0.3%).
